# feixue94/sfd2

Hardware: AMD Instinct MI355X
Metric: images/sec extract+match (1600x1200, n4096) (higher is better)
Workload: dtype f16c

## Files before the change

include/sfd2_hip.h:

```cpp
#ifndef SFD2_HIP_H
#define SFD2_HIP_H

#include <stdint.h>

#ifdef __cplusplus
extern "C" {
#endif

typedef struct sfd2_ctx sfd2_ctx;

#define SFD2_DESC_DIM 128
#define SFD2_FLAG_ASYNC 1
#define SFD2_FLAG_NO_STABILITY 2
#define SFD2_FLAG_IMG_NORMALISED 4
#define SFD2_FLAG_IMG_U8_HWC 8
#define SFD2_FLAG_IMG_BGR 16
#define SFD2_FLAG_MATCH_OUT16 64
#define SFD2_FLAG_DESC_STORE64 128
#define SFD2_FLAG_IMG_U8_X 32

typedef struct {
    const char *name;
    const float *data;
    int32_t ndim;
    int64_t shape[4];
} sfd2_tensor;

#define SFD2_MATCH_HLOC 0
#define SFD2_MATCH_ITLOC_NNM 1
#define SFD2_MATCH_ITLOC_NNR 2
#define SFD2_DT_F32 0
#define SFD2_DT_F64 1
#define SFD2_DT_F16 2
#define SFD2_LAYOUT_ND 0
#define SFD2_LAYOUT_DN 1
#define SFD2_SIM_F16 0
#define SFD2_SIM_F16X2 1

typedef struct {
    int32_t flavour;
    int32_t do_mutual_check;
    float ratio_threshold;
    float distance_threshold;
    int32_t sim_mode;
} sfd2_match_conf;

typedef struct {
    float ms_total;
    float ms_backbone;
    float ms_post;
    float ms_match;
    int64_t n_candidates;
} sfd2_timings;

int sfd2_version(void);
const char *sfd2_last_error(void);

int sfd2_ctx_create(int device, sfd2_ctx **out);
int sfd2_device_pci_bus_id(int device, char *out, int len, int *n_devices);
void sfd2_ctx_destroy(sfd2_ctx *ctx);
void *sfd2_get_stream(sfd2_ctx *ctx);

int sfd2_load_weights(sfd2_ctx *ctx, const sfd2_tensor *tensors, int n);

#define SFD2_PREC_F16 0
#define SFD2_PREC_F32 1
#define SFD2_PREC_F16X3 2
#define SFD2_PREC_F16C 3
int sfd2_set_precision(sfd2_ctx *ctx, int mode);

int sfd2_set_option(sfd2_ctx *ctx, const char *key, int value);
int sfd2_get_option(sfd2_ctx *ctx, const char *key, int *value);

int sfd2_det(sfd2_ctx *ctx, const float *x, int x_on_device, int H, int W, int flags,
             float *score, float *stability, float *desc, int out_on_device,
             int *hs, int *ws, int *hc, int *wc);

int sfd2_extract(sfd2_ctx *ctx, const void *img, int img_on_device, int H, int W,
                 float conf_th, int top_k, int flags,
                 float *kpts_xy, float *scores, float *desc, int out_on_device,
                 int64_t cap_out, int *n_out);
int sfd2_extract_multiscale(sfd2_ctx *ctx, const void *img, int img_on_device, int H, int W,
                            const double *scales, int n_scales, float conf_th, int top_k, int flags,
                            float *kpts_xy, float *scores, float *desc, int out_on_device,
                            int64_t cap_out, int *n_out);

int sfd2_preprocess(sfd2_ctx *ctx, const unsigned char *img_hwc, int on_device, int H, int W, int flags,
                    int new_h, int new_w, float *out_chw_dev);

int sfd2_extract_count(sfd2_ctx *ctx, int *n_out);

typedef struct {
    int32_t n;
    int32_t n_candidates;
    uint32_t saturated;
    uint32_t flags;
} sfd2_extract_record;
int sfd2_extract_record_async(sfd2_ctx *ctx, sfd2_extract_record *rec, int rec_on_device);

int sfd2_extract_spp(sfd2_ctx *ctx, const float *x, int x_on_device, int H, int W, float conf_th, int flags,
                     float *kpts_xy, float *scores, float *desc, int64_t cap_out, int *n_out,
                     float *heat_out, float *desc_full_out);
int sfd2_extract_spp_levels(sfd2_ctx *ctx, const float *x, int x_on_device, int H, int W, int n_levels,
                            const int32_t *nh, const int32_t *nw, const int32_t *emit, float conf_th, int flags,
                            float *kpts_xy, float *scores, float *desc, int64_t cap_out, int32_t *level_count);
int sfd2_nms_fast(sfd2_ctx *ctx, const float *heat, int H, int W, float conf_th, int dist, float *kept_out);

int sfd2_simple_nms(sfd2_ctx *ctx, const float *heat, int H, int W, int radius, float *nms_out);
int sfd2_select_keypoints(sfd2_ctx *ctx, const float *heat, int H, int W, float conf_th,
                          int radius, int border, int top_k,
                          float *kpts_xy, float *scores, int64_t cap_out, int *n_out);
int sfd2_sample_descriptors(sfd2_ctx *ctx, const float *desc_map, int hc, int wc, int nh, int nw,
                            const float *kpts_xy, int n, float *desc_out);
int sfd2_heatmap(sfd2_ctx *ctx, const float *score, int hs, int ws, const float *sta, int hc, int wc,
                 int H, int W, float *heat_out);
int sfd2_debug_activation(sfd2_ctx *ctx, const char *name, float *out, int64_t cap, int *c, int *h, int *w);

int sfd2_match(sfd2_ctx *ctx, const void *d0, int n0, const void *d1, int n1, int dim,
               int dtype, int layout, int on_device, const sfd2_match_conf *conf,
               int64_t *matches0, float *scores0, int out_on_device);

int sfd2_match_segments(sfd2_ctx *ctx, const void *d0, int n0, const void *d1, int n1, int dim,
                        int dtype, int layout, int on_device, int n_seg, const int32_t *seg0, const int32_t *seg1,
                        const sfd2_match_conf *conf, int64_t *matches0, float *scores0, int out_on_device);

typedef struct {
    const void *data;
    int32_t n;
    int32_t dtype;
    int32_t layout;
    int32_t on_device;
    const int32_t *rows;
    int32_t n_rows;
    int32_t reserved;
} sfd2_desc_set;

int sfd2_desc_pack(sfd2_ctx *ctx, const sfd2_desc_set *src, int dim, void *dst_f16_dev, int flags);

int sfd2_match_batch(sfd2_ctx *ctx, const sfd2_desc_set *q, const sfd2_desc_set *db, int k, int dim,
                     const sfd2_match_conf *conf, int64_t *matches0, float *scores0, int out_on_device,
                     int flags);

int sfd2_extract_match(sfd2_ctx *ctx, const void *img_dev, int H, int W, float conf_th, int top_k, int flags,
                       float *kpts_xy, float *scores, float *desc, const sfd2_desc_set *db, int k, int dim,
                       const sfd2_match_conf *conf, int64_t *matches0, float *scores0);

int sfd2_get_timings(sfd2_ctx *ctx, sfd2_timings *out);

#define SFD2_RANGE_TENSORS 17
#define SFD2_RANGE_GROUPS 14
typedef struct {
    int32_t n_tensors;
    float max_stored[SFD2_RANGE_TENSORS];
    float max_value[SFD2_RANGE_TENSORS];
    int32_t exponent[SFD2_RANGE_TENSORS];
    uint32_t saturated;
    uint32_t low;
    int32_t fallbacks;
} sfd2_range_status;
int sfd2_get_range_status(sfd2_ctx *ctx, sfd2_range_status *out, int reset);
const char *sfd2_range_tensor_name(int i);
int sfd2_calibrate_range(sfd2_ctx *ctx, const float *img, int img_on_device, int H, int W, int flags);
int sfd2_get_act_exponents(sfd2_ctx *ctx, int32_t *exps, float *maxima, int cap, int *n);
int sfd2_set_act_exponents(sfd2_ctx *ctx, const int32_t *exps, int n );
int sfd2_get_margin_status(sfd2_ctx *ctx, float *errs4, int *choice, float *target);
int sfd2_get_relax_status(sfd2_ctx *ctx, float *err_plain, int *c3b_plain);

int sfd2_sync(sfd2_ctx *ctx);

typedef struct {
    char name[32];
    char kernel[48];
    double flops;
    double bytes;
    double ms_total;
    int32_t launches;
} sfd2_layer_timing;
int sfd2_set_profiling(sfd2_ctx *ctx, int max_steps );
int sfd2_set_profile_filter(sfd2_ctx *ctx, const char *substr);
int sfd2_get_layer_timings(sfd2_ctx *ctx, sfd2_layer_timing *out, int cap, int *n);

#define SFD2_JPEG_OK 0
#define SFD2_JPEG_NOT_JPEG 1
#define SFD2_JPEG_TRUNCATED 2
#define SFD2_JPEG_PROGRESSIVE 3
#define SFD2_JPEG_ARITHMETIC 4
#define SFD2_JPEG_PRECISION 5
#define SFD2_JPEG_COLOUR 6
#define SFD2_JPEG_SAMPLING 7
#define SFD2_JPEG_MULTI_SCAN 8
#define SFD2_JPEG_PROCESS 9
#define SFD2_JPEG_MALFORMED 10
typedef struct {
    int32_t width, height;
    int32_t n_components;
    int32_t h_samp[3], v_samp[3];
    int32_t restart_interval;
    int32_t supported;
    int32_t reason;
    int32_t mcus_x, mcus_y;
    int32_t n_intervals;
    int32_t n_blocks;
    int64_t file_bytes;
    int64_t scan_begin, scan_end;
    int64_t prepared_cap;
    int64_t prepared_bytes;
    int32_t n_lanes;
    int32_t prepared;
} sfd2_jpeg_info;

int sfd2_jpeg_parse(const uint8_t *data, int64_t n, sfd2_jpeg_info *info);

int sfd2_jpeg_prepare(uint8_t *buf, int64_t cap, sfd2_jpeg_info *info);

int sfd2_jpeg_decode(sfd2_ctx *ctx, const uint8_t *data, int64_t n, const sfd2_jpeg_info *info, int flags,
                     uint8_t *out_rgbx_dev, int64_t out_cap, uint32_t *status, int status_on_device);

#define SFD2_CAM_SIMPLE_PINHOLE 0
#define SFD2_CAM_PINHOLE 1
#define SFD2_CAM_SIMPLE_RADIAL 2
#define SFD2_CAM_OPENCV 4
typedef struct {
    int32_t n;
    int32_t model;
    const double *points2D;
    const double *points3D;
    double params[8];
    int32_t width, height;
    double max_error_px;
} sfd2_pose_problem;
typedef struct {
    double min_inlier_ratio;
    int64_t min_num_trials, max_num_trials;
    double confidence;
    uint64_t seed;
} sfd2_pose_conf;
typedef struct {
    int32_t success;
    int32_t num_inliers;
    int32_t num_trials;
    int32_t reserved;
    double qvec[4];
    double tvec[3];
} sfd2_pose_result;

int sfd2_absolute_pose_batch(sfd2_ctx *ctx, const sfd2_pose_problem *problems, int k, const sfd2_pose_conf *conf,
                             sfd2_pose_result *results, uint8_t *inlier_mask_u8, int flags);
int sfd2_pose_refine_batch(sfd2_ctx *ctx, const sfd2_pose_problem *problems, int k, const double *qvec_tvec_in,
                           const uint8_t *inlier_mask_u8, sfd2_pose_result *results, int flags);

#ifdef __cplusplus
}
#endif
#endif
```

sfd2_amd/_lib.py:

```python
import ctypes
import os

import numpy as np

_HERE = os.path.dirname(os.path.abspath(__file__))
LIB_PATH = os.path.join(_HERE, "libsfd2hip.so")


def use_library(path):
    global LIB_PATH, _lib
    if _lib is not None:
        raise RuntimeError("use_library() must be called before the library is first loaded")
    LIB_PATH = os.path.abspath(path)

FLAG_ASYNC = 1
FLAG_NO_STABILITY = 2
FLAG_IMG_NORMALISED = 4
FLAG_IMG_U8_HWC = 8
FLAG_IMG_BGR = 16
FLAG_IMG_U8_X = 32
FLAG_MATCH_OUT16 = 64
FLAG_DESC_STORE64 = 128
MATCH_HLOC, MATCH_ITLOC_NNM, MATCH_ITLOC_NNR = 0, 1, 2
DT_F32, DT_F64, DT_F16 = 0, 1, 2
LAYOUT_ND, LAYOUT_DN = 0, 1
SIM_F16, SIM_F16X2 = 0, 1


class Sfd2Tensor(ctypes.Structure):
    _fields_ = [("name", ctypes.c_char_p), ("data", ctypes.c_void_p), ("ndim", ctypes.c_int32),
                ("shape", ctypes.c_int64 * 4)]


class MatchConf(ctypes.Structure):
    _fields_ = [("flavour", ctypes.c_int32), ("do_mutual_check", ctypes.c_int32),
                ("ratio_threshold", ctypes.c_float), ("distance_threshold", ctypes.c_float),
                ("sim_mode", ctypes.c_int32)]


class Timings(ctypes.Structure):
    _fields_ = [("ms_total", ctypes.c_float), ("ms_backbone", ctypes.c_float), ("ms_post", ctypes.c_float),
                ("ms_match", ctypes.c_float), ("n_candidates", ctypes.c_int64)]


class DescSet(ctypes.Structure):
    _fields_ = [("data", ctypes.c_void_p), ("n", ctypes.c_int32), ("dtype", ctypes.c_int32),
                ("layout", ctypes.c_int32), ("on_device", ctypes.c_int32),
                ("rows", ctypes.c_void_p), ("n_rows", ctypes.c_int32), ("reserved", ctypes.c_int32)]


class LayerTiming(ctypes.Structure):
    _fields_ = [("name", ctypes.c_char * 32), ("kernel", ctypes.c_char * 48), ("flops", ctypes.c_double),
                ("bytes", ctypes.c_double), ("ms_total", ctypes.c_double), ("launches", ctypes.c_int32)]


class ExtractRecord(ctypes.Structure):
    _fields_ = [("n", ctypes.c_int32), ("n_candidates", ctypes.c_int32), ("saturated", ctypes.c_uint32), ("flags", ctypes.c_uint32)]


RANGE_TENSORS, RANGE_GROUPS = 17, 14


class RangeStatus(ctypes.Structure):
    _fields_ = [("n_tensors", ctypes.c_int32), ("max_stored", ctypes.c_float * RANGE_TENSORS),
                ("max_value", ctypes.c_float * RANGE_TENSORS), ("exponent", ctypes.c_int32 * RANGE_TENSORS),
                ("saturated", ctypes.c_uint32), ("low", ctypes.c_uint32), ("fallbacks", ctypes.c_int32)]


class JpegInfo(ctypes.Structure):
    _fields_ = [("width", ctypes.c_int32), ("height", ctypes.c_int32), ("n_components", ctypes.c_int32),
                ("h_samp", ctypes.c_int32 * 3), ("v_samp", ctypes.c_int32 * 3), ("restart_interval", ctypes.c_int32),
                ("supported", ctypes.c_int32), ("reason", ctypes.c_int32), ("mcus_x", ctypes.c_int32), ("mcus_y", ctypes.c_int32),
                ("n_intervals", ctypes.c_int32), ("n_blocks", ctypes.c_int32), ("file_bytes", ctypes.c_int64),
                ("scan_begin", ctypes.c_int64), ("scan_end", ctypes.c_int64), ("prepared_cap", ctypes.c_int64),
                ("prepared_bytes", ctypes.c_int64), ("n_lanes", ctypes.c_int32), ("prepared", ctypes.c_int32)]


class PoseProblem(ctypes.Structure):
    _fields_ = [("n", ctypes.c_int32), ("model", ctypes.c_int32), ("points2D", ctypes.c_void_p), ("points3D", ctypes.c_void_p),
                ("params", ctypes.c_double * 8), ("width", ctypes.c_int32), ("height", ctypes.c_int32), ("max_error_px", ctypes.c_double)]


class PoseConf(ctypes.Structure):
    _fields_ = [("min_inlier_ratio", ctypes.c_double), ("min_num_trials", ctypes.c_int64), ("max_num_trials", ctypes.c_int64),
                ("confidence", ctypes.c_double), ("seed", ctypes.c_uint64)]


class PoseResult(ctypes.Structure):
    _fields_ = [("success", ctypes.c_int32), ("num_inliers", ctypes.c_int32), ("num_trials", ctypes.c_int32), ("reserved", ctypes.c_int32),
                ("qvec", ctypes.c_double * 4), ("tvec", ctypes.c_double * 3)]


EXPORTS = [
    "sfd2_version", "sfd2_last_error", "sfd2_ctx_create", "sfd2_ctx_destroy", "sfd2_get_stream",
    "sfd2_load_weights", "sfd2_det", "sfd2_extract", "sfd2_extract_count", "sfd2_simple_nms",
    "sfd2_select_keypoints", "sfd2_sample_descriptors", "sfd2_heatmap", "sfd2_debug_activation",
    "sfd2_match", "sfd2_match_batch", "sfd2_get_timings", "sfd2_sync", "sfd2_set_profiling",
    "sfd2_get_layer_timings", "sfd2_set_precision", "sfd2_extract_spp", "sfd2_nms_fast",
    "sfd2_set_profile_filter", "sfd2_extract_multiscale", "sfd2_set_option", "sfd2_extract_match", "sfd2_preprocess", "sfd2_extract_spp_levels", "sfd2_match_segments",
    "sfd2_get_range_status", "sfd2_range_tensor_name", "sfd2_calibrate_range", "sfd2_get_act_exponents", "sfd2_set_act_exponents",
    "sfd2_extract_record_async", "sfd2_desc_pack", "sfd2_get_margin_status", "sfd2_get_relax_status", "sfd2_get_option", "sfd2_device_pci_bus_id",
    "sfd2_jpeg_parse", "sfd2_jpeg_prepare", "sfd2_jpeg_decode", "sfd2_absolute_pose_batch", "sfd2_pose_refine_batch",
]

_lib = None


def load():
    global _lib
    if _lib is not None:
        return _lib
    if LIB_PATH == os.path.join(_HERE, "libsfd2hip.so"):
        from . import build as _build
        if _build.needs_build() and _build.have_hipcc():
            import fcntl
            with open(os.path.join(_HERE, ".build.lock"), "w") as lk:
                fcntl.flock(lk, fcntl.LOCK_EX)
                try:
                    if _build.needs_build():
                        _build.build_lib()
                finally:
                    fcntl.flock(lk, fcntl.LOCK_UN)
    if not os.path.exists(LIB_PATH):
        raise RuntimeError(f"{LIB_PATH} is missing and no hipcc was found to build it "
                           "(hipcc --offload-arch=gfx950; `python -c 'import __graft_entry__ as g; g.build()'`). "
                           "There is no CPU fallback.")
    lib = ctypes.CDLL(LIB_PATH)
    vp, ci, cf, i64 = ctypes.c_void_p, ctypes.c_int, ctypes.c_float, ctypes.c_int64
    pi = ctypes.POINTER(ctypes.c_int)
    lib.sfd2_version.restype = ci
    lib.sfd2_last_error.restype = ctypes.c_char_p
    lib.sfd2_ctx_create.argtypes = [ci, ctypes.POINTER(vp)]
    lib.sfd2_ctx_destroy.argtypes = [vp]
    lib.sfd2_ctx_destroy.restype = None
    lib.sfd2_get_stream.argtypes = [vp]
    lib.sfd2_get_stream.restype = vp
    lib.sfd2_load_weights.argtypes = [vp, ctypes.POINTER(Sfd2Tensor), ci]
    lib.sfd2_det.argtypes = [vp, vp, ci, ci, ci, ci, vp, vp, vp, ci, pi, pi, pi, pi]
    lib.sfd2_extract.argtypes = [vp, vp, ci, ci, ci, cf, ci, ci, vp, vp, vp, ci, i64, pi]
    lib.sfd2_extract_count.argtypes = [vp, pi]
    lib.sfd2_extract_multiscale.argtypes = [vp, vp, ci, ci, ci, vp, ci, cf, ci, ci, vp, vp, vp, ci, i64, pi]
    lib.sfd2_extract_spp.argtypes = [vp, vp, ci, ci, ci, cf, ci, vp, vp, vp, i64, pi, vp, vp]
    lib.sfd2_nms_fast.argtypes = [vp, vp, ci, ci, cf, ci, vp]
    lib.sfd2_extract_spp_levels.argtypes = [vp, vp, ci, ci, ci, ci, vp, vp, vp, cf, ci, vp, vp, vp, i64, vp]
    lib.sfd2_simple_nms.argtypes = [vp, vp, ci, ci, ci, vp]
    lib.sfd2_select_keypoints.argtypes = [vp, vp, ci, ci, cf, ci, ci, ci, vp, vp, i64, pi]
    lib.sfd2_sample_descriptors.argtypes = [vp, vp, ci, ci, ci, ci, vp, ci, vp]
    lib.sfd2_heatmap.argtypes = [vp, vp, ci, ci, vp, ci, ci, ci, ci, vp]
    lib.sfd2_debug_activation.argtypes = [vp, ctypes.c_char_p, vp, i64, pi, pi, pi]
    lib.sfd2_match.argtypes = [vp, vp, ci, vp, ci, ci, ci, ci, ci, ctypes.POINTER(MatchConf), vp, vp, ci]
    lib.sfd2_match_segments.argtypes = [vp, vp, ci, vp, ci, ci, ci, ci, ci, ci, vp, vp, ctypes.POINTER(MatchConf), vp, vp, ci]
    lib.sfd2_match_batch.argtypes = [vp, ctypes.POINTER(DescSet), ctypes.POINTER(DescSet), ci, ci,
                                     ctypes.POINTER(MatchConf), vp, vp, ci, ci]
    lib.sfd2_get_timings.argtypes = [vp, ctypes.POINTER(Timings)]
    lib.sfd2_sync.argtypes = [vp]
    lib.sfd2_set_precision.argtypes = [vp, ci]
    lib.sfd2_set_option.argtypes = [vp, ctypes.c_char_p, ci]
    lib.sfd2_get_option.argtypes = [vp, ctypes.c_char_p, pi]
    lib.sfd2_device_pci_bus_id.argtypes = [ci, ctypes.c_char_p, ci, pi]
    lib.sfd2_preprocess.argtypes = [vp, vp, ci, ci, ci, ci, ci, ci, vp]
    lib.sfd2_extract_match.argtypes = [vp, vp, ci, ci, cf, ci, ci, vp, vp, vp, ctypes.POINTER(DescSet), ci, ci,
                                       ctypes.POINTER(MatchConf), vp, vp]
    lib.sfd2_set_profiling.argtypes = [vp, ci]
    lib.sfd2_set_profile_filter.argtypes = [vp, ctypes.c_char_p]
    lib.sfd2_get_layer_timings.argtypes = [vp, ctypes.POINTER(LayerTiming), ci, pi]
    lib.sfd2_get_range_status.argtypes = [vp, ctypes.POINTER(RangeStatus), ci]
    lib.sfd2_range_tensor_name.argtypes = [ci]
    lib.sfd2_range_tensor_name.restype = ctypes.c_char_p
    lib.sfd2_calibrate_range.argtypes = [vp, vp, ci, ci, ci, ci]
    lib.sfd2_get_act_exponents.argtypes = [vp, vp, vp, ci, pi]
    lib.sfd2_get_margin_status.argtypes = [vp, vp, pi, ctypes.POINTER(ctypes.c_float)]
    lib.sfd2_get_relax_status.restype = ci
    lib.sfd2_get_relax_status.argtypes = [vp, ctypes.POINTER(ctypes.c_float), pi]
    lib.sfd2_set_act_exponents.argtypes = [vp, vp, ci]
    lib.sfd2_extract_record_async.argtypes = [vp, vp, ci]
    lib.sfd2_desc_pack.argtypes = [vp, ctypes.POINTER(DescSet), ci, vp, ci]
    lib.sfd2_jpeg_parse.argtypes = [vp, i64, ctypes.POINTER(JpegInfo)]
    lib.sfd2_jpeg_prepare.argtypes = [vp, i64, ctypes.POINTER(JpegInfo)]
    lib.sfd2_jpeg_decode.argtypes = [vp, vp, i64, ctypes.POINTER(JpegInfo), ci, vp, i64, vp, ci]
    lib.sfd2_absolute_pose_batch.argtypes = [vp, ctypes.POINTER(PoseProblem), ci, ctypes.POINTER(PoseConf), ctypes.POINTER(PoseResult), vp, ci]
    lib.sfd2_pose_refine_batch.argtypes = [vp, ctypes.POINTER(PoseProblem), ci, vp, vp, ctypes.POINTER(PoseResult), ci]
    for name in EXPORTS:
        getattr(lib, name)
    if lib.sfd2_version() < 109:
        raise RuntimeError(f"{LIB_PATH} is version {lib.sfd2_version()}, this binding needs >= 109 (rebuild: __graft_entry__.build())")
    _lib = lib
    return lib


def check(rc):
    if rc != 0:
        raise RuntimeError("libsfd2hip: " + load().sfd2_last_error().decode("utf-8", "replace"))


def ptr(a):
    if a is None:
        return None
    if isinstance(a, int):
        return a
    if isinstance(a, np.ndarray):
        return a.ctypes.data
    return a.data_ptr()


class Context:

    def __init__(self, device=0):
        self.lib = load()
        h = ctypes.c_void_p()
        check(self.lib.sfd2_ctx_create(int(device), ctypes.byref(h)))
        self.h = h
        self.device = int(device)
        self.options = {}

    def close(self):
        if getattr(self, "h", None):
            self.lib.sfd2_ctx_destroy(self.h)
            self.h = None

    def __del__(self):
        try:
            self.close()
        except Exception:
            pass

    @property
    def stream(self):
        return self.lib.sfd2_get_stream(self.h)

    def load_weights(self, sd):
        keep, arr = [], (Sfd2Tensor * len(sd))()
        n = 0
        for name, v in sd.items():
            a = v.detach().cpu().numpy() if hasattr(v, "detach") else np.asarray(v)
            if a.dtype.kind != "f":
                continue
            a = np.ascontiguousarray(a, dtype=np.float32)
            if a.ndim > 4:
                continue
            keep.append(a)
            arr[n].name = name.encode()
            arr[n].data = a.ctypes.data
            arr[n].ndim = a.ndim
            for i, s in enumerate(a.shape):
                arr[n].shape[i] = s
            n += 1
        check(self.lib.sfd2_load_weights(self.h, arr, n))

    def timings(self):
        t = Timings()
        check(self.lib.sfd2_get_timings(self.h, ctypes.byref(t)))
        return {"ms_total": t.ms_total, "ms_backbone": t.ms_backbone, "ms_post": t.ms_post,
                "ms_match": t.ms_match, "n_candidates": t.n_candidates}

    def set_precision(self, mode):
        check(self.lib.sfd2_set_precision(self.h, {'f16': 0, 'f32': 1, 'f16x3': 2, 'f16c': 3, 'f16x3d': 2}[mode]))
        check(self.lib.sfd2_set_option(self.h, b"x3_desc16", 1 if mode == 'f16x3d' else 0))

    def set_option(self, key, value):
        check(self.lib.sfd2_set_option(self.h, key.encode(), int(value)))
        self.options.pop(key, None)
        self.options[key] = int(value)

    def get_option(self, key):
        v = ctypes.c_int(0)
        check(self.lib.sfd2_get_option(self.h, key.encode(), ctypes.byref(v)))
        return int(v.value)

    def sync(self):
        check(self.lib.sfd2_sync(self.h))

    def set_profiling(self, max_steps, kernel_filter=None):
        check(self.lib.sfd2_set_profile_filter(self.h, (kernel_filter or "").encode()))
        check(self.lib.sfd2_set_profiling(self.h, int(max_steps)))

    def layer_timings(self):
        n = ctypes.c_int(0)
        arr = (LayerTiming * 64)()
        check(self.lib.sfd2_get_layer_timings(self.h, arr, 64, ctypes.byref(n)))
        return [{"name": arr[i].name.decode(), "kernel": arr[i].kernel.decode(), "flops": arr[i].flops,
                 "bytes": arr[i].bytes, "ms_total": arr[i].ms_total, "launches": arr[i].launches}
                for i in range(min(n.value, 64))]

    def range_status(self, reset=False):
        rs = RangeStatus()
        check(self.lib.sfd2_get_range_status(self.h, ctypes.byref(rs), 1 if reset else 0))
        names = [self.lib.sfd2_range_tensor_name(i).decode() for i in range(rs.n_tensors)]
        return {"tensors": {n: {"max_stored": rs.max_stored[i], "max_value": rs.max_value[i], "exponent": rs.exponent[i]}
                            for i, n in enumerate(names)},
                "saturated": [n for i, n in enumerate(names) if rs.saturated >> i & 1],
                "low": [n for i, n in enumerate(names) if rs.low >> i & 1], "fallbacks": rs.fallbacks}

    def calibrate_range(self, img, normalised=False):
        on_dev = 0 if isinstance(img, np.ndarray) else 1
        if isinstance(img, np.ndarray):
            img = np.ascontiguousarray(img, dtype=np.float32)
        check(self.lib.sfd2_calibrate_range(self.h, ptr(img), on_dev, int(img.shape[-2]), int(img.shape[-1]),
                                            FLAG_IMG_NORMALISED if normalised else 0))

    def act_exponents(self):
        e = np.zeros(RANGE_GROUPS, dtype=np.int32)
        m = np.zeros(RANGE_GROUPS, dtype=np.float32)
        n = ctypes.c_int(0)
        check(self.lib.sfd2_get_act_exponents(self.h, e.ctypes.data, m.ctypes.data, RANGE_GROUPS, ctypes.byref(n)))
        return e, m

    def margin_status(self):
        e = np.zeros(4, dtype=np.float32)
        ch, tg = ctypes.c_int(0), ctypes.c_float(0)
        check(self.lib.sfd2_get_margin_status(self.h, e.ctypes.data, ctypes.byref(ch), ctypes.byref(tg)))
        names = ["as set", "rb_inner=0", "comp_heads=1", "rb_inner=0 comp_heads=1"]
        ep, on = ctypes.c_float(0), ctypes.c_int(0)
        check(self.lib.sfd2_get_relax_status(self.h, ctypes.byref(ep), ctypes.byref(on)))
        return {"errors": {n: float(v) for n, v in zip(names, e)}, "choice": int(ch.value),
                "running": names[ch.value] if ch.value >= 0 else None, "target": float(tg.value),
                "c3b_plain": bool(on.value), "error_with_c3b_plain": float(ep.value)}

    def set_act_exponents(self, exps=None):
        if exps is None:
            check(self.lib.sfd2_set_act_exponents(self.h, None, 0))
        else:
            e = np.ascontiguousarray(exps, dtype=np.int32)
            check(self.lib.sfd2_set_act_exponents(self.h, e.ctypes.data, int(e.size)))

    def debug_activation(self, name):
        c, h, w = ctypes.c_int(), ctypes.c_int(), ctypes.c_int()
        check(self.lib.sfd2_debug_activation(self.h, name.encode(), None, 0, ctypes.byref(c), ctypes.byref(h), ctypes.byref(w)))
        out = np.empty((c.value, h.value, w.value), dtype=np.float32)
        check(self.lib.sfd2_debug_activation(self.h, name.encode(), out.ctypes.data, out.size, ctypes.byref(c),
                                             ctypes.byref(h), ctypes.byref(w)))
        return out


_default_ctx = {}


def default_context(device=0):
    d = int(device)
    if d not in _default_ctx:
        _default_ctx[d] = Context(d)
# ... 2 lines not shown
```

sfd2_amd/csrc/api_core.hip:

```cpp
#include "sfd2_ctx.h"

static thread_local std::string g_err;
int sfd2_fail(const std::string &m)
{
    g_err = m;
    return -1;
}

std::atomic<unsigned long long> g_alloc_gen{0};

thread_local int g_sfd2_cu_limit = 0;

extern "C" int sfd2_version(void) { return 110; }
extern "C" const char *sfd2_last_error(void) { return g_err.c_str(); }

extern "C" int sfd2_ctx_create(int device, sfd2_ctx **out)
{
    if (!out) return fail("sfd2_ctx_create: out is null");
    int ndev = 0;
    hipError_t e = hipGetDeviceCount(&ndev);
    if (e != hipSuccess || ndev <= 0) return fail("sfd2_ctx_create: no HIP device available (libsfd2hip has no CPU fallback)");
    if (device < 0 || device >= ndev) return fail("sfd2_ctx_create: bad device index");
    HIPCHECK(hipSetDevice(device));
    sfd2_ctx *c = new sfd2_ctx();
    c->device = device;
    HIPCHECK(hipStreamCreateWithFlags(&c->stream, hipStreamNonBlocking));
    for (int i = 0; i < 4; ++i) HIPCHECK(hipEventCreate(&c->ev[i]));
    HIPCHECK(hipEventCreateWithFlags(&c->ev_jobs, hipEventDisableTiming));
    HIPCHECK(hipStreamCreateWithFlags(&c->copy_stream, hipStreamNonBlocking));
    HIPCHECK(hipStreamCreateWithFlags(&c->side_stream, hipStreamNonBlocking));
    HIPCHECK(hipEventCreateWithFlags(&c->ev_fork, hipEventDisableTiming));
    HIPCHECK(hipEventCreateWithFlags(&c->ev_join, hipEventDisableTiming));
    c->cur_stream = c->stream;
    for (int i = 0; i < SFD2_IMG_SLOTS; ++i) {
        HIPCHECK(hipEventCreateWithFlags(&c->ev_copied[i], hipEventDisableTiming));
        HIPCHECK(hipEventCreateWithFlags(&c->ev_img_free[i], hipEventDisableTiming));
    }
    c->fuse = sfd2_env("SFD2_NO_FUSE") ? 0 : 1;
    HIPCHECK(c->zero_page.ensure(SFD2_ZERO_PAGE_BYTES + ((size_t)SFD2_RS_COUNT * (SFD2_RANGE_SUB + 1) + 4) * sizeof(unsigned int)));
    HIPCHECK(hipMemset(c->zero_page.p, 0, c->zero_page.cap));
    c->range_stat.p = c->zero_page.as<char>() + SFD2_ZERO_PAGE_BYTES;
    c->range_hist_dev.p = c->range_stat.as<unsigned int>() + SFD2_RS_COUNT * SFD2_RANGE_SUB;
    c->extract_rec.p = c->range_hist_dev.as<unsigned int>() + SFD2_RS_COUNT;
    static_assert(SFD2_RS_COUNT == SFD2_RANGE_TENSORS && AE_COUNT == SFD2_RANGE_GROUPS, "include/sfd2_hip.h and the internal tables agree");

    *out = c;
    return 0;
}

extern "C" int sfd2_device_pci_bus_id(int device, char *out, int len, int *n_devices)
{
    int ndev = 0;
    hipError_t e = hipGetDeviceCount(&ndev);
    if (e != hipSuccess || ndev <= 0) return fail("sfd2_device_pci_bus_id: no HIP device available");
    if (n_devices) *n_devices = ndev;
    if (device < 0 || device >= ndev) return fail("sfd2_device_pci_bus_id: bad device index");
    if (!out || len < 13) return fail("sfd2_device_pci_bus_id: buffer of at least 13 bytes needed");
    HIPCHECK(hipDeviceGetPCIBusId(out, len, device));
    return 0;
}

extern "C" void sfd2_ctx_destroy(sfd2_ctx *c)
{
    if (!c) return;
    (void)hipSetDevice(c->device);
    (void)hipStreamSynchronize(c->stream);
    graphs_release(c);
    for (int i = 0; i < 4; ++i) if (c->ev[i]) (void)hipEventDestroy(c->ev[i]);
    if (c->ev_jobs) (void)hipEventDestroy(c->ev_jobs);
    for (int i = 0; i < SFD2_IMG_SLOTS; ++i) {
        if (c->ev_copied[i]) (void)hipEventDestroy(c->ev_copied[i]);
        if (c->ev_img_free[i]) (void)hipEventDestroy(c->ev_img_free[i]);
    }
    if (c->copy_stream) (void)hipStreamDestroy(c->copy_stream);
    if (c->side_stream) (void)hipStreamDestroy(c->side_stream);
    if (c->ev_fork) (void)hipEventDestroy(c->ev_fork);
    if (c->ev_join) (void)hipEventDestroy(c->ev_join);
    for (hipEvent_t e : c->prof_ev) (void)hipEventDestroy(e);
    if (c->pin_jobs) (void)hipHostFree(c->pin_jobs);
    if (c->stream) (void)hipStreamDestroy(c->stream);
    delete c;
}

extern "C" void *sfd2_get_stream(sfd2_ctx *c) { return c ? (void *)c->stream : nullptr; }

extern "C" int sfd2_set_precision(sfd2_ctx *c, int mode)
{
    if (!c) return fail("sfd2_set_precision: null ctx");
    if (mode != SFD2_PREC_F16 && mode != SFD2_PREC_F32 && mode != SFD2_PREC_F16X3 && mode != SFD2_PREC_F16C)
        return fail("sfd2_set_precision: unknown mode");
    HIPCHECK(hipSetDevice(c->device));
    HIPCHECK(hipStreamSynchronize(c->stream));
    if (mode != c->precision) graphs_release(c);
    c->precision = mode;
    return sfd2_margin_selfcheck_if_pending(c);
}

extern "C" int sfd2_set_option(sfd2_ctx *c, const char *key, int value)
{
    if (!c || !key) return fail("sfd2_set_option: null argument");
    HIPCHECK(hipSetDevice(c->device));
    HIPCHECK(hipStreamSynchronize(c->stream));
    const std::string k(key);
    graphs_release(c);
    if (k == "fuse") c->fuse = value ? 1 : 0;
    else if (k == "fuse_det") c->fuse_det = value ? 1 : 0;
    else if (k == "alias") c->opt_alias = value ? 1 : 0;
    else if (k == "graphs") c->use_graphs = value ? 1 : 0;
    else if (k == "branches") c->opt_branches = value ? 1 : 0;
    else if (k == "sta_side") c->opt_sta_side = value ? 1 : 0;
    else if (k == "fuse_post") c->opt_fuse_post = value ? 1 : 0;
    else if (k == "sparse_desc") c->opt_sparse_desc = value ? 1 : 0;
    else if (k == "sparse_da3") c->opt_sparse_da3 = value ? 1 : 0;
    else if (k == "cu_limit") c->opt_cu_limit = value < 0 ? 0 : value;
    else if (k == "auto_range") c->opt_auto_range = value ? 1 : 0;
    else if (k == "range_fallback") c->opt_range_fallback = value ? 1 : 0;
    else if (k == "x3_pp") c->opt_x3_pp = value ? 1 : 0;
    else if (k == "x3_desc16") c->opt_x3_desc16 = value ? 1 : 0;
    else if (k == "auto_margin") c->opt_auto_margin = value ? 1 : 0;
    else if (k == "fp6_filters") c->opt_fp6_filters = value ? 1 : 0;
    else if (k == "fp6_acts") c->opt_fp6_acts = value ? 1 : 0;
    else if (k == "s2d") c->opt_s2d = value ? 1 : 0;
    else if (k == "trunk_r1") c->opt_trunk_r1 = value ? 1 : 0;
    else if (k == "fuse_pb") c->opt_fuse_pb = value ? 1 : 0;
    else if (k == "generic_c") c->opt_generic_c = value ? 1 : 0;
    else if (k == "comp_rb") c->opt_comp_rb = value ? 1 : 0;
    else if (k == "no_rf_c") c->opt_no_rf_c = value ? 1 : 0;
    else if (k == "comp_heads") { c->opt_comp_heads = c->user_comp_heads = value ? 1 : 0; c->user_set_comp_heads = true; }
    else if (k == "c3b_plain") { c->user_c3b_plain = value < 0 ? -1 : (value ? 1 : 0); c->opt_c3b_plain = value > 0 ? 1 : 0; }
    else if (k == "comp_det") c->opt_comp_det = value ? 1 : 0;
    else if (k == "fuse_rb23") c->opt_fuse_rb23 = value ? 1 : 0;
    else if (k == "rb_inner") { c->opt_rb_inner = c->user_rb_inner = value < 0 ? 0 : (value > 2 ? 2 : value); c->user_set_rb_inner = true; }
    else return fail("sfd2_set_option: unknown key '" + k + "'");
    return 0;
}

extern "C" int sfd2_get_option(sfd2_ctx *c, const char *key, int *value)
{
    if (!c || !key || !value) return fail("sfd2_get_option: null argument");
    const std::string k(key);
    const struct { const char *name; int v; } tab[] = {
        {"fuse", c->fuse}, {"fuse_det", c->fuse_det}, {"alias", c->opt_alias}, {"graphs", c->use_graphs}, {"branches", c->opt_branches}, {"sta_side", c->opt_sta_side},
        {"fuse_post", c->opt_fuse_post}, {"sparse_desc", c->opt_sparse_desc}, {"sparse_da3", c->opt_sparse_da3}, {"cu_limit", c->opt_cu_limit},
        {"auto_range", c->opt_auto_range}, {"range_fallback", c->opt_range_fallback}, {"x3_pp", c->opt_x3_pp}, {"x3_desc16", c->opt_x3_desc16},
        {"auto_margin", c->opt_auto_margin}, {"fp6_filters", c->opt_fp6_filters}, {"fp6_acts", c->opt_fp6_acts}, {"s2d", c->opt_s2d},
        {"trunk_r1", c->opt_trunk_r1}, {"fuse_pb", c->opt_fuse_pb}, {"generic_c", c->opt_generic_c}, {"comp_rb", c->opt_comp_rb},
        {"no_rf_c", c->opt_no_rf_c}, {"comp_heads", c->opt_comp_heads}, {"c3b_plain", c->opt_c3b_plain}, {"comp_det", c->opt_comp_det},
        {"fuse_rb23", c->opt_fuse_rb23}, {"rb_inner", c->opt_rb_inner},
    };
    for (const auto &e : tab)
        if (k == e.name) { *value = e.v; return 0; }
    return fail("sfd2_get_option: unknown key '" + k + "'");
}

extern "C" int sfd2_sync(sfd2_ctx *c)
{
    if (!c) return fail("sfd2_sync: null ctx");
    HIPCHECK(hipSetDevice(c->device));
    HIPCHECK(hipStreamSynchronize(c->stream));
    return 0;
}

extern "C" int sfd2_set_profiling(sfd2_ctx *c, int max_steps)
{
    if (!c) return fail("sfd2_set_profiling: null ctx");
    HIPCHECK(hipSetDevice(c->device));
    HIPCHECK(hipStreamSynchronize(c->stream));
    if (max_steps < 0 || max_steps > 4096) return fail("sfd2_set_profiling: max_steps out of range");
    const size_t need = (size_t)max_steps * PROF_SLOTS * 2;
    while (c->prof_ev.size() < need) {
        hipEvent_t e;
        HIPCHECK(hipEventCreate(&e));
        c->prof_ev.push_back(e);
    }
    c->prof_max_steps = max_steps;
    c->prof_step = 0;
    c->prof_slot = 0;
    c->prof_used.assign(max_steps, 0);
    c->prof_row.assign((size_t)max_steps * PROF_SLOTS, 0);
    c->prof_tab.clear();
    return 0;
}

extern "C" int sfd2_set_profile_filter(sfd2_ctx *c, const char *substr)
{
    if (!c) return fail("sfd2_set_profile_filter: null ctx");
    c->prof_filter = substr ? substr : "";
    return 0;
}

extern "C" int sfd2_get_layer_timings(sfd2_ctx *c, sfd2_layer_timing *out, int cap, int *n)
{
    if (!c || !n) return fail("sfd2_get_layer_timings: null argument");
    HIPCHECK(hipSetDevice(c->device));
    HIPCHECK(hipStreamSynchronize(c->stream));
    for (int st = 0; st < c->prof_step; ++st)
        for (int sl = 0; sl < c->prof_used[st]; ++sl) {
            float ms = 0.0f;
            const size_t e = ((size_t)st * PROF_SLOTS + sl) * 2;
            const int row = c->prof_row[(size_t)st * PROF_SLOTS + sl];
            if (hipEventElapsedTime(&ms, c->prof_ev[e], c->prof_ev[e + 1]) == hipSuccess) {
                c->prof_tab[row].ms_total += ms;
                c->prof_tab[row].launches += 1;
            }
        }
    c->prof_step = 0;
    *n = (int)c->prof_tab.size();
    if (out)
        for (int i = 0; i < *n && i < cap; ++i) out[i] = c->prof_tab[i];
    return 0;
}

extern "C" int sfd2_get_timings(sfd2_ctx *c, sfd2_timings *out)
{
    if (!c || !out) return fail("sfd2_get_timings: null argument");
    *out = c->tim;
    return 0;
}

static const int kRsGroup[SFD2_RS_COUNT] = {AE_CONV1A, AE_CONV1B, AE_CONV2A, AE_CONV2B, AE_CONV3A, AE_TRUNK, AE_T1_0, AE_T1_1, AE_T1_2,
                                            AE_T2_0, AE_T2_1, AE_T2_2, AE_TRUNK, AE_TRUNK, AE_TRUNK, AE_PA0, AE_DA0};
extern "C" const char *sfd2_range_tensor_name(int i)
{
    static const char *names[SFD2_RS_COUNT] = {"conv1a", "conv1b", "conv2a", "conv2b", "conv3a", "conv3b", "conv4.0.t1", "conv4.1.t1", "conv4.2.t1",
                                               "conv4.0.t2", "conv4.1.t2", "conv4.2.t2", "conv4.0", "conv4.1", "conv4.2", "convPa.0", "convDa.0"};
    return (i >= 0 && i < SFD2_RS_COUNT) ? names[i] : "";
}

static int fetch_range_words(sfd2_ctx *c, unsigned int *raw , bool clear)
{
    const size_t bytes = (size_t)SFD2_RS_COUNT * (SFD2_RANGE_SUB + 1) * sizeof(unsigned int);
    HIPCHECK(hipMemcpyAsync(raw, c->range_stat.p, bytes, hipMemcpyDeviceToHost, c->stream));
    if (clear) HIPCHECK(hipMemsetAsync(c->range_stat.p, 0, bytes, c->stream));
    HIPCHECK(hipStreamSynchronize(c->stream));
    return 0;
}

int read_range_status(sfd2_ctx *c, sfd2_range_status *out, int reset)
{
    unsigned int raw[SFD2_RS_COUNT * (SFD2_RANGE_SUB + 1)];
    if (fetch_range_words(c, raw, reset != 0)) return -1;
    std::memset(out, 0, sizeof(*out));
    out->n_tensors = SFD2_RS_COUNT;
    const unsigned int sat_bits = 0x44E00000u;
    for (int t = 0; t < SFD2_RS_COUNT; ++t) {
        unsigned int m = raw[SFD2_RS_COUNT * SFD2_RANGE_SUB + t];
        for (int s = 0; s < SFD2_RANGE_SUB; ++s) m = std::max(m, raw[t * SFD2_RANGE_SUB + s]);
        float f;
        std::memcpy(&f, &m, 4);
        const bool sat = m >= sat_bits || c->range_hist[t] >= SFD2_C_SAT;
        if (!(f >= c->range_hist[t])) f = c->range_hist[t];
        if (reset) c->range_hist[t] = 0.0f;
        const int e = c->act_exp[kRsGroup[t]];
        out->max_stored[t] = f;
        out->max_value[t] = std::ldexp(f, -e);
        out->exponent[t] = e;
        if (sat) out->saturated |= 1u << t;
        if (f > 0.0f && f < 0.03125f) out->low |= 1u << t;
    }
    out->fallbacks = c->range_fallbacks;
    return 0;
}

int reset_range_records(sfd2_ctx *c)
{
    if (!c->range_stat.p) return 0;
    HIPCHECK(hipMemsetAsync(c->range_stat.p, 0, (size_t)SFD2_RS_COUNT * (SFD2_RANGE_SUB + 1) * sizeof(unsigned int), c->stream));
    for (int t = 0; t < SFD2_RS_COUNT; ++t) c->range_hist[t] = 0.0f;
    return 0;
}

int range_fold_before_sync_extract(sfd2_ctx *c)
{
    if (c->precision != SFD2_PREC_F16C || !c->opt_range_fallback || c->in_fallback) return 0;
    launch_extract_record(c->stream, c->range_stat.as<unsigned int>(), c->range_hist_dev.as<unsigned int>(), nullptr, 0, 0, nullptr);
    HIPCHECK(hipGetLastError());
    return 0;
}

extern "C" int sfd2_get_range_status(sfd2_ctx *c, sfd2_range_status *out, int reset)
{
    if (!c || !out) return fail("sfd2_get_range_status: null argument");
    HIPCHECK(hipSetDevice(c->device));
    return read_range_status(c, out, reset);
}

int range_wants_fallback(sfd2_ctx *c)
{
    if (c->precision != SFD2_PREC_F16C || !c->opt_range_fallback || c->in_fallback) return 0;
    unsigned int raw[SFD2_RS_COUNT * SFD2_RANGE_SUB];
    HIPCHECK(hipMemcpyAsync(raw, c->range_stat.p, sizeof(raw), hipMemcpyDeviceToHost, c->stream));
    HIPCHECK(hipStreamSynchronize(c->stream));
    bool sat = false;
    float mx[SFD2_RS_COUNT];
    for (int t = 0; t < SFD2_RS_COUNT; ++t) {
        unsigned int m = 0;
// ... 25 lines not shown
```

sfd2_amd/csrc/api_graph.hip:

```cpp
#include "sfd2_ctx.h"

struct GraphKey {
    int H, W, top_k, flags, k, dim, n0;
    float conf_th;
    sfd2_match_conf conf;
    const void *img, *kp, *sc, *de, *m, *ms;
    unsigned long long db_hash;
    bool operator==(const GraphKey &o) const { return memcmp(this, &o, sizeof(GraphKey)) == 0; }
};
struct GraphEntry {
    GraphKey key;
    hipGraph_t graph = nullptr;
    hipGraphExec_t exec = nullptr;
    unsigned long long gen = 0, last_use = 0;
    int seen = 0;
    void *pin = nullptr;
    size_t pin_cap = 0;
    DevBuf jobs, fins;
};
#define SFD2_MAX_GRAPHS 16

static void graph_entry_release(GraphEntry &e)
{
    if (e.exec) (void)hipGraphExecDestroy(e.exec);
    if (e.graph) (void)hipGraphDestroy(e.graph);
    if (e.pin) (void)hipHostFree(e.pin);
    e.jobs.release();
    e.fins.release();
    e = GraphEntry();
}

void graphs_release(sfd2_ctx *c)
{
    if (!c->graphs) return;
    for (int i = 0; i < c->n_graphs; ++i) graph_entry_release(c->graphs[i]);
    delete[] c->graphs;
    c->graphs = nullptr;
    c->n_graphs = 0;
}

static int extract_match_eager(sfd2_ctx *c, const void *img, int H, int W, float conf_th, int top_k, int flags, float *kp,
                               float *sc, float *de, const sfd2_desc_set *db, int k, int dim, const sfd2_match_conf *conf,
                               int64_t *m, float *ms)
{
    int n_dummy = 0;
    if (sfd2_extract(c, img, 1, H, W, conf_th, top_k, flags | SFD2_FLAG_ASYNC, kp, sc, de, 1, top_k, &n_dummy)) return -1;
    if (k > 0) {
        const sfd2_desc_set q = {de, top_k, SFD2_DT_F32, SFD2_LAYOUT_ND, 1, nullptr, 0, 0};
        if (sfd2_match_batch(c, &q, db, k, dim, conf, m, ms, 1, SFD2_FLAG_ASYNC)) return -1;
    }
    return 0;
}

extern "C" int sfd2_extract_match(sfd2_ctx *c, const void *img_dev, int H, int W, float conf_th, int top_k, int flags,
                                  float *kpts_xy, float *scores, float *desc, const sfd2_desc_set *db, int k, int dim,
                                  const sfd2_match_conf *conf, int64_t *matches0, float *scores0)
{
    if (!c || !img_dev || !kpts_xy || !scores || !desc) return fail("sfd2_extract_match: null argument");
    if (top_k <= 0) return fail("sfd2_extract_match: top_k must be positive (fixed-capacity device outputs)");
    if (flags & SFD2_FLAG_DESC_STORE64) return fail("sfd2_extract_match: SFD2_FLAG_DESC_STORE64 is for stores; the matcher reads the float [n][128] descriptors");
    if (k < 0 || (k > 0 && (!db || !conf || !matches0 || !scores0))) return fail("sfd2_extract_match: null matcher argument");
    for (int i = 0; i < k; ++i)
        if (!db[i].on_device || db[i].rows) return fail("sfd2_extract_match: database sets must be device resident, without row selection");
    HIPCHECK(hipSetDevice(c->device));
    if (!c->use_graphs || c->prof_max_steps > 0)
        return extract_match_eager(c, img_dev, H, W, conf_th, top_k, flags, kpts_xy, scores, desc, db, k, dim, conf, matches0, scores0);

    GraphKey key;
    memset(&key, 0, sizeof(key));
    key.H = H; key.W = W; key.top_k = top_k; key.flags = flags; key.k = k; key.dim = dim; key.n0 = top_k; key.conf_th = conf_th;
    if (conf) key.conf = *conf;
    key.img = img_dev; key.kp = kpts_xy; key.sc = scores; key.de = desc; key.m = matches0; key.ms = scores0;
    unsigned long long h = 1469598103934665603ull;
    for (int i = 0; i < k; ++i) {
        const unsigned long long v[3] = {(unsigned long long)(uintptr_t)db[i].data, (unsigned long long)db[i].n,
                                         ((unsigned long long)db[i].dtype << 8) | (unsigned long long)db[i].layout};
        for (unsigned long long x : v) { h ^= x; h *= 1099511628211ull; }
    }
    key.db_hash = h;
    if (!c->graphs) { c->graphs = new GraphEntry[SFD2_MAX_GRAPHS]; c->n_graphs = SFD2_MAX_GRAPHS; }
    GraphEntry *e = nullptr, *lru = &c->graphs[0];
    for (int i = 0; i < c->n_graphs; ++i) {
        GraphEntry &g = c->graphs[i];
        if (g.seen && g.key == key) { e = &g; break; }
        if (g.last_use < lru->last_use) lru = &g;
    }
    if (!e) {
        graph_entry_release(*lru);
        e = lru;
        e->key = key;
    }
    e->last_use = ++c->graph_clock;
    if (e->exec && e->gen == g_alloc_gen) {
        HIPCHECK(hipGraphLaunch(e->exec, c->stream));
        return 0;
    }
    if (e->exec) {
        (void)hipGraphExecDestroy(e->exec); e->exec = nullptr;
        (void)hipGraphDestroy(e->graph); e->graph = nullptr;
        e->seen = 0;
    }
    if (e->seen == 0) {
        e->seen = 1;
        return extract_match_eager(c, img_dev, H, W, conf_th, top_k, flags, kpts_xy, scores, desc, db, k, dim, conf, matches0, scores0);
    }
    const size_t jb = 2 * (size_t)std::max(k, 1) * sizeof(MatchJob), fb = (size_t)std::max(k, 1) * sizeof(MatchFinal);
    if (!e->pin) {
        HIPCHECK(hipHostMalloc(&e->pin, jb + fb, hipHostMallocDefault));
        e->pin_cap = jb + fb;
        HIPCHECK(e->jobs.ensure(jb + fb));
    }
    HIPCHECK(hipStreamSynchronize(c->stream));
    HIPCHECK(hipEventSynchronize(c->ev_jobs));
    const unsigned long long gen0 = g_alloc_gen.load();
    std::swap(c->pin_jobs, e->pin); std::swap(c->pin_cap, e->pin_cap);
    std::swap(c->m_jobs, e->jobs); std::swap(c->m_fins, e->fins);
    hipError_t be = hipStreamBeginCapture(c->stream, hipStreamCaptureModeThreadLocal);
    int rc = -1;
    hipGraph_t g = nullptr;
    if (be == hipSuccess) {
        rc = extract_match_eager(c, img_dev, H, W, conf_th, top_k, flags, kpts_xy, scores, desc, db, k, dim, conf, matches0, scores0);
        const hipError_t ee = hipStreamEndCapture(c->stream, &g);
        if (ee != hipSuccess) rc = fail(std::string("hipStreamEndCapture: ") + hipGetErrorString(ee));
    } else {
        fail(std::string("hipStreamBeginCapture: ") + hipGetErrorString(be));
    }
    std::swap(c->pin_jobs, e->pin); std::swap(c->pin_cap, e->pin_cap);
    std::swap(c->m_jobs, e->jobs); std::swap(c->m_fins, e->fins);
    if (rc != 0 || g_alloc_gen != gen0) {
        if (g) (void)hipGraphDestroy(g);
        e->seen = 0;
        if (rc == 0) return fail("sfd2_extract_match: workspace changed during capture");
        return -1;
    }
    e->graph = g;
    HIPCHECK(hipGraphInstantiate(&e->exec, g, nullptr, nullptr, 0));
    e->gen = g_alloc_gen;
    HIPCHECK(hipGraphLaunch(e->exec, c->stream));
    return 0;
}
```

sfd2_amd/csrc/api_match.hip:

```cpp
#include "sfd2_ctx.h"

static size_t elt_size(int dtype) { return dtype == SFD2_DT_F64 ? 8 : (dtype == SFD2_DT_F16 ? 2 : 4); }

static int prep_set(sfd2_ctx *c, const void *src, int n_src, const int32_t *rows, int n, int dim, int dtype, int layout,
                    int on_device, int need_lo, DevBuf &stage, size_t &stage_off, half_t *hi_dst, half_t *lo_dst,
                    const half_t **hi, const half_t **lo, const int **rows_dev = nullptr)
{
    if (rows_dev) *rows_dev = nullptr;
    if (!rows && dtype == SFD2_DT_F16 && layout == SFD2_LAYOUT_ND && on_device && dim == 128 && !need_lo) {
        *hi = reinterpret_cast<const half_t *>(src);
        *lo = nullptr;
        return 0;
    }
    const void *dev_src = src;
    if (!on_device) {
        const size_t bytes = (size_t)n_src * dim * elt_size(dtype);
        void *dst = reinterpret_cast<char *>(stage.p) + stage_off;
        HIPCHECK(hipMemcpyAsync(dst, src, bytes, hipMemcpyHostToDevice, c->stream));
        dev_src = dst;
        stage_off += (bytes + 255) & ~(size_t)255;
    }
    const int *rd = nullptr;
    if (rows) {
        void *dst = reinterpret_cast<char *>(stage.p) + stage_off;
        HIPCHECK(hipMemcpyAsync(dst, rows, (size_t)n * sizeof(int32_t), hipMemcpyHostToDevice, c->stream));
        rd = reinterpret_cast<const int *>(dst);
        stage_off += ((size_t)n * sizeof(int32_t) + 255) & ~(size_t)255;
        if (rows_dev) *rows_dev = rd;
    }
    launch_match_prep(c->stream, dev_src, n, n_src, rd, dim, dtype, layout, hi_dst, need_lo ? lo_dst : nullptr);
    *hi = hi_dst;
    *lo = need_lo ? lo_dst : nullptr;
    return 0;
}

extern "C" int sfd2_desc_pack(sfd2_ctx *c, const sfd2_desc_set *src, int dim, void *dst_f16_dev, int flags)
{
    if (!c || !src || !dst_f16_dev) return fail("sfd2_desc_pack: null argument");
    if (dim <= 0 || dim > 128) return fail("descriptor dimension must be in [1,128]");
    if (src->n < 0 || src->n_rows < 0) return fail("negative size");
    if (src->dtype != SFD2_DT_F32 && src->dtype != SFD2_DT_F64 && src->dtype != SFD2_DT_F16) return fail("sfd2_desc_pack: unknown dtype");
    if (src->layout != SFD2_LAYOUT_ND && src->layout != SFD2_LAYOUT_DN) return fail("sfd2_desc_pack: unknown layout");
    const int n = src->rows ? src->n_rows : src->n;
    if (n == 0) return 0;
    if (!src->data) return fail("sfd2_desc_pack: null descriptors");
    if (src->rows)
        for (int r = 0; r < src->n_rows; ++r)
            if (src->rows[r] < 0 || src->rows[r] >= src->n) return fail("sfd2_desc_pack: row index out of range");
    HIPCHECK(hipSetDevice(c->device));
    size_t stage_bytes = 256;
    if (!src->on_device) stage_bytes += (((size_t)src->n * dim * elt_size(src->dtype)) + 255) & ~(size_t)255;
    if (src->rows) stage_bytes += ((size_t)n * sizeof(int32_t) + 255) & ~(size_t)255;
    HIPCHECK(c->m_stage.ensure(stage_bytes));
    size_t off = 0;
    void *dev_src = const_cast<void *>(src->data);
    if (!src->on_device) {
        const size_t bytes = (size_t)src->n * dim * elt_size(src->dtype);
        HIPCHECK(hipMemcpyAsync(c->m_stage.p, src->data, bytes, hipMemcpyHostToDevice, c->stream));
        dev_src = c->m_stage.p;
        off += (bytes + 255) & ~(size_t)255;
    }
    const int *rd = nullptr;
    if (src->rows) {
        void *dst = c->m_stage.as<char>() + off;
        HIPCHECK(hipMemcpyAsync(dst, src->rows, (size_t)n * sizeof(int32_t), hipMemcpyHostToDevice, c->stream));
        rd = reinterpret_cast<const int *>(dst);
    }
    launch_match_prep(c->stream, dev_src, n, src->n, rd, dim, src->dtype, src->layout, reinterpret_cast<half_t *>(dst_f16_dev), nullptr);
    HIPCHECK(hipGetLastError());
    if (!(flags & SFD2_FLAG_ASYNC)) HIPCHECK(hipStreamSynchronize(c->stream));
    return 0;
}

extern "C" int sfd2_match_batch(sfd2_ctx *c, const sfd2_desc_set *q, const sfd2_desc_set *db, int k, int dim,
                                const sfd2_match_conf *conf, int64_t *matches0, float *scores0, int out_on_device,
                                int flags)
{
    if (!c || !conf || !q || (k > 0 && !db)) return fail("sfd2_match_batch: null argument");
    if (dim <= 0 || dim > 128) return fail("descriptor dimension must be in [1,128]");
    const int n0 = q->n;
    if (n0 < 0 || k < 0) return fail("negative size");
    if (k == 0 || n0 == 0) return 0;
    if (!q->data) return fail("sfd2_match_batch: null query descriptors");
    HIPCHECK(hipSetDevice(c->device));
    const int need_lo = conf->sim_mode == SFD2_SIM_F16X2;
    const bool o16 = (flags & SFD2_FLAG_MATCH_OUT16) != 0;
    const size_t msz = o16 ? sizeof(short) : sizeof(long long), ssz = o16 ? sizeof(half_t) : sizeof(float);
    int max_n1 = 0;
    size_t tot_n1 = 0, stage_bytes = 0;
    if (q->rows) return fail("sfd2_match_batch: row selection applies to database sets only");
    std::vector<int> eff_n1(k);
    for (int i = 0; i < k; ++i) {
        if (db[i].n < 0 || db[i].n_rows < 0) return fail("negative n1");
        if (db[i].n > 0 && !db[i].data) return fail("sfd2_match_batch: null database descriptors");
        if (db[i].rows)
            for (int r = 0; r < db[i].n_rows; ++r)
                if (db[i].rows[r] < 0 || db[i].rows[r] >= db[i].n) return fail("sfd2_match_batch: row index out of range");
        eff_n1[i] = db[i].rows ? db[i].n_rows : db[i].n;
        max_n1 = std::max(max_n1, eff_n1[i]);
        tot_n1 += (size_t)eff_n1[i];
        if (!db[i].on_device) stage_bytes += (((size_t)db[i].n * dim * elt_size(db[i].dtype)) + 255) & ~(size_t)255;
        if (db[i].rows) stage_bytes += ((size_t)db[i].n_rows * sizeof(int32_t) + 255) & ~(size_t)255;
    }
    if (!q->on_device) stage_bytes += (((size_t)n0 * dim * elt_size(q->dtype)) + 255) & ~(size_t)255;
    const int max_n = std::max(n0, max_n1);
    const int blocks_per_job = (max_n + 255) / 256;
    int splits = (768 * 6 + 2 * k * blocks_per_job - 1) / (2 * k * blocks_per_job);
    splits = std::max(1, std::min(splits, 8));
    const int min_n = std::max(1, std::min(n0, max_n1 > 0 ? max_n1 : 1));
    splits = std::min(splits, std::max(1, (min_n + 31) / 32));
    if (const char *e = sfd2_env("SFD2_MATCH_SPLITS")) splits = std::max(1, std::min(16, atoi(e)));

    const int need_top2 = (conf->flavour == SFD2_MATCH_ITLOC_NNR) ||
                          (conf->flavour == SFD2_MATCH_HLOC && conf->ratio_threshold > 0.0f);
    const bool single_gemm = !need_lo && !need_top2 && sfd2_env("SFD2_MATCH_TWO_GEMM") == nullptr;
    if (single_gemm) {
        const int qblocks = (n0 + 255) / 256;
        splits = (512 * 6 + k * qblocks - 1) / (k * qblocks);
        splits = std::max(1, std::min(splits, 8));
        splits = std::min(splits, std::max(1, (std::max(1, max_n1) + 31) / 32));
        if (const char *e = sfd2_env("SFD2_MATCH_SPLITS")) splits = std::max(1, std::min(16, atoi(e)));
        splits = std::max(splits, (max_n1 + match_mutual_max_chunk() - 1) / match_mutual_max_chunk());
    }
    const int nstrip = (n0 + match_mutual_strip() - 1) / match_mutual_strip();

    HIPCHECK(c->m_stage.ensure(std::max<size_t>(stage_bytes, 256)));
    HIPCHECK(c->m_hi0.ensure((size_t)n0 * 128 * 2));
    if (need_lo) HIPCHECK(c->m_lo0.ensure((size_t)n0 * 128 * 2));
    HIPCHECK(c->m_hi1.ensure(std::max<size_t>(tot_n1, 1) * 128 * 2));
    if (need_lo) HIPCHECK(c->m_lo1.ensure(std::max<size_t>(tot_n1, 1) * 128 * 2));
    const size_t per_pair_f = (size_t)splits * n0, tot_part = (size_t)k * per_pair_f + (size_t)splits * tot_n1;
    HIPCHECK(c->m_part_f.ensure(std::max<size_t>(tot_part, 1) * 2 * sizeof(float)));
    HIPCHECK(c->m_part_i.ensure(std::max<size_t>(tot_part, 1) * sizeof(int)));
    if (single_gemm) HIPCHECK(c->m_rkeys.ensure(std::max<size_t>((size_t)nstrip * tot_n1, 1) * sizeof(float)));
    HIPCHECK(c->m_red.ensure(((size_t)k * n0 + tot_n1 + 1) * 3 * sizeof(float)));
    HIPCHECK(c->m_jobs.ensure((size_t)2 * k * sizeof(MatchJob) + (size_t)k * sizeof(MatchFinal)));
    HIPCHECK(c->m_out_m.ensure((size_t)k * n0 * sizeof(long long)));
    HIPCHECK(c->m_out_s.ensure((size_t)k * n0 * sizeof(float)));

    HIPCHECK(hipEventRecord(c->ev[0], c->stream));
    prof_step_begin(c);
    size_t stage_off = 0;
    const half_t *q_hi = nullptr, *q_lo = nullptr;
    if (prep_set(c, q->data, n0, nullptr, n0, dim, q->dtype, q->layout, q->on_device, need_lo, c->m_stage, stage_off,
                 c->m_hi0.as<half_t>(), c->m_lo0.as<half_t>(), &q_hi, &q_lo)) return -1;
    static_assert(sizeof(MatchJob2) <= 2 * sizeof(MatchJob), "descriptor buffer sizing");
    const size_t jobs_bytes = 2 * (size_t)k * sizeof(MatchJob), fins_bytes = (size_t)k * sizeof(MatchFinal);
    hipStreamCaptureStatus cap_status = hipStreamCaptureStatusNone;
    (void)hipStreamIsCapturing(c->stream, &cap_status);
    const bool capturing = cap_status != hipStreamCaptureStatusNone;
    if (!capturing) HIPCHECK(hipEventSynchronize(c->ev_jobs));
    if (jobs_bytes + fins_bytes > c->pin_cap) {
        if (c->pin_jobs) (void)hipHostFree(c->pin_jobs);
        c->pin_jobs = nullptr;
        c->pin_cap = 0;
        HIPCHECK(hipHostMalloc(&c->pin_jobs, jobs_bytes + fins_bytes, hipHostMallocDefault));
        c->pin_cap = jobs_bytes + fins_bytes;
    }
    MatchJob *jobs = reinterpret_cast<MatchJob *>(c->pin_jobs);
    MatchJob2 *jobs2 = reinterpret_cast<MatchJob2 *>(c->pin_jobs);
    MatchFinal *fins = reinterpret_cast<MatchFinal *>(reinterpret_cast<char *>(c->pin_jobs) + jobs_bytes);
    float *pf = c->m_part_f.as<float>();
    int *pi = c->m_part_i.as<int>();
    float *red = c->m_red.as<float>();
    size_t off1 = 0, poff = 0, roff = 0;
    for (int i = 0; i < k; ++i) {
        const int n1 = eff_n1[i];
        const half_t *h = nullptr, *l = nullptr;
        const int *remap = nullptr;
        if (n1 > 0) {
            if (prep_set(c, db[i].data, db[i].n, db[i].rows, n1, dim, db[i].dtype, db[i].layout, db[i].on_device, need_lo,
                         c->m_stage, stage_off, c->m_hi1.as<half_t>() + off1 * 128,
                         need_lo ? c->m_lo1.as<half_t>() + off1 * 128 : nullptr, &h, &l, &remap))
                return -1;
        }
        MatchFinal &fn = fins[i];
        fn.remap = remap;
        if (single_gemm) {
            MatchJob2 &j2 = jobs2[i];
            j2.q_hi = q_hi; j2.d_hi = h; j2.n0 = n0; j2.n1 = n1;
            j2.part_v1 = pf + 2 * poff; j2.part_i1 = pi + poff;
            j2.rkeys = c->m_rkeys.as<float>() + (size_t)nstrip * off1;
            poff += (size_t)splits * n0 + (size_t)splits * n1;
            fn.f_v1 = fn.f_v2 = fn.r_v1 = fn.r_v2 = nullptr; fn.f_i1 = fn.r_i1 = nullptr;
        } else {
            MatchJob &f = jobs[2 * i], &r = jobs[2 * i + 1];
            f.a_hi = h; f.a_lo = l; f.b_hi = q_hi; f.b_lo = q_lo; f.na = n1; f.nb = n0;
            f.part_v1 = pf + 2 * poff; f.part_v2 = pf + 2 * poff + (size_t)splits * n0; f.part_i1 = pi + poff;
            poff += (size_t)splits * n0;
            r.a_hi = q_hi; r.a_lo = q_lo; r.b_hi = h; r.b_lo = l; r.na = n0; r.nb = n1;
            r.part_v1 = pf + 2 * poff; r.part_v2 = pf + 2 * poff + (size_t)splits * n1; r.part_i1 = pi + poff;
            poff += (size_t)splits * n1;
            fn.f_v1 = f.part_v1; fn.f_v2 = f.part_v2; fn.f_i1 = f.part_i1;
            fn.r_v1 = r.part_v1; fn.r_v2 = r.part_v2; fn.r_i1 = r.part_i1;
        }
        off1 += (size_t)n1;
        fn.n0 = n0; fn.n1 = n1;
        fn.out16 = o16 ? 1 : 0; fn.pad_ = 0;
        const bool direct_out = out_on_device && matches0 && scores0;
        fn.matches0 = reinterpret_cast<long long *>((direct_out ? reinterpret_cast<char *>(matches0) : c->m_out_m.as<char>()) + (size_t)i * n0 * msz);
        fn.scores0 = reinterpret_cast<float *>((direct_out ? reinterpret_cast<char *>(scores0) : c->m_out_s.as<char>()) + (size_t)i * n0 * ssz);
        fn.red_f = red + 3 * roff; roff += (size_t)n0;
        fn.red_r = red + 3 * roff; roff += (size_t)n1;
    }
    HIPCHECK(hipMemcpyAsync(c->m_jobs.p, jobs, jobs_bytes + fins_bytes, hipMemcpyHostToDevice, c->stream));
    MatchFinal *fins_dev = reinterpret_cast<MatchFinal *>(static_cast<char *>(c->m_jobs.p) + jobs_bytes);
    if (!capturing) HIPCHECK(hipEventRecord(c->ev_jobs, c->stream));
    if (single_gemm) {
        {
            ProfScope ps(c, "match_mutual", "match_mutual_kernel", 2.0 * (double)n0 * (double)tot_n1 * 128.0,
                         2.0 * ((double)k * n0 + (double)tot_n1) * 128.0);
            launch_match_mutual(c->stream, c->m_jobs.as<MatchJob2>(), fins_dev, k, n0, max_n1, splits,
                                conf->flavour == SFD2_MATCH_HLOC && !conf->do_mutual_check);
        }
        {
            ProfScope ps(c, "match_finalize", "match_decide", 0.0, (double)tot_part * 12);
            launch_match_decide(c->stream, fins_dev, k, max_n, conf->flavour, conf->do_mutual_check,
                                conf->ratio_threshold, conf->distance_threshold);
        }
    } else {
        {
            ProfScope ps(c, "match_top2", need_lo ? "match_top2_kernel<x2>" : "match_top2_kernel",
                         2.0 * 2.0 * (double)n0 * (double)tot_n1 * 128.0 * (need_lo ? 3.0 : 1.0),
                         2.0 * 2.0 * ((double)k * n0 + (double)tot_n1) * 128.0);
            launch_match_top2(c->stream, c->m_jobs.as<MatchJob>(), 2 * k, max_n, splits, need_lo, need_top2,
                              c->zero_page.as<half_t>());
        }
        {
            ProfScope ps(c, "match_finalize", "match_reduce+decide", 0.0, (double)tot_part * 12);
            launch_match_finalize(c->stream, fins_dev, k, max_n, splits, conf->flavour,
                                  conf->do_mutual_check, conf->ratio_threshold, conf->distance_threshold);
        }
    }
    prof_step_end(c);
    HIPCHECK(hipGetLastError());
    HIPCHECK(hipEventRecord(c->ev[3], c->stream));
    if (!(out_on_device && matches0 && scores0)) {
        if (copy_out(c, matches0, c->m_out_m.p, (size_t)k * n0 * msz, out_on_device)) return -1;
        if (copy_out(c, scores0, c->m_out_s.p, (size_t)k * n0 * ssz, out_on_device)) return -1;
    }
    if (!(flags & SFD2_FLAG_ASYNC)) {
        HIPCHECK(hipStreamSynchronize(c->stream));
        float ms = 0.0f;
        if (hipEventElapsedTime(&ms, c->ev[0], c->ev[3]) == hipSuccess) c->tim.ms_match = ms;
    }
    return 0;
}

extern "C" int sfd2_match_segments(sfd2_ctx *c, const void *d0, int n0, const void *d1, int n1, int dim, int dtype, int layout,
                                   int on_device, int n_seg, const int32_t *seg0, const int32_t *seg1,
                                   const sfd2_match_conf *conf, int64_t *matches0, float *scores0, int out_on_device)
{
    if (!c || !conf || !seg0 || !seg1 || !matches0 || !scores0) return fail("sfd2_match_segments: null argument");
    if (dim <= 0 || dim > 128) return fail("descriptor dimension must be in [1,128]");
    if (n0 < 0 || n1 < 0 || n_seg < 0) return fail("negative size");
    if (n0 == 0) return 0;
    if (!d0 || (n1 > 0 && !d1)) return fail("sfd2_match_segments: null descriptors");
    if (seg0[0] != 0 || seg1[0] != 0 || seg0[n_seg] != n0 || seg1[n_seg] != n1) return fail("sfd2_match_segments: segment offsets must span [0, n]");
    for (int i = 0; i < n_seg; ++i)
        if (seg0[i + 1] < seg0[i] || seg1[i + 1] < seg1[i]) return fail("sfd2_match_segments: segment offsets must ascend");
    HIPCHECK(hipSetDevice(c->device));
    const int need_lo = conf->sim_mode == SFD2_SIM_F16X2;
    const int need_top2 = (conf->flavour == SFD2_MATCH_ITLOC_NNR) || (conf->flavour == SFD2_MATCH_HLOC && conf->ratio_threshold > 0.0f);
    const bool single_gemm = !need_lo && !need_top2;
    std::vector<int> live;
    int max_a = 0, max_b = 0;
    for (int i = 0; i < n_seg; ++i)
        if (seg0[i + 1] > seg0[i] && seg1[i + 1] > seg1[i]) {
            live.push_back(i);
            max_a = std::max(max_a, seg0[i + 1] - seg0[i]);
            max_b = std::max(max_b, seg1[i + 1] - seg1[i]);
        }
    const int k = (int)live.size();
    HIPCHECK(c->m_out_m.ensure((size_t)n0 * sizeof(long long)));
    HIPCHECK(c->m_out_s.ensure((size_t)n0 * sizeof(float)));
    long long *out_m = out_on_device ? reinterpret_cast<long long *>(matches0) : c->m_out_m.as<long long>();
    float *out_s = out_on_device ? scores0 : c->m_out_s.as<float>();
    HIPCHECK(hipMemsetAsync(out_m, 0xFF, (size_t)n0 * sizeof(long long), c->stream));
    HIPCHECK(hipMemsetAsync(out_s, 0, (size_t)n0 * sizeof(float), c->stream));
    if (k > 0) {
        int splits = std::max(1, (max_b + match_mutual_max_chunk() - 1) / match_mutual_max_chunk());
        const int strip = match_mutual_strip();
        size_t stage_bytes = 256 + (((size_t)n1 * sizeof(int32_t)) + 255);
        if (!on_device) stage_bytes += ((((size_t)n0 + n1) * dim * elt_size(dtype)) + 511);
        HIPCHECK(c->m_stage.ensure(stage_bytes));
        HIPCHECK(c->m_hi0.ensure((size_t)n0 * 128 * 2));
        HIPCHECK(c->m_hi1.ensure((size_t)std::max(n1, 1) * 128 * 2));
        if (need_lo) { HIPCHECK(c->m_lo0.ensure((size_t)n0 * 128 * 2)); HIPCHECK(c->m_lo1.ensure((size_t)std::max(n1, 1) * 128 * 2)); }
        const size_t tot_part = (size_t)splits * ((size_t)n0 + n1);
        HIPCHECK(c->m_part_f.ensure(tot_part * 2 * sizeof(float)));
        HIPCHECK(c->m_part_i.ensure(tot_part * sizeof(int)));
        size_t rk = 0;
        for (int i : live) rk += (size_t)((seg0[i + 1] - seg0[i] + strip - 1) / strip) * (size_t)(seg1[i + 1] - seg1[i]);
        if (single_gemm) HIPCHECK(c->m_rkeys.ensure(std::max<size_t>(rk, 1) * sizeof(float)));
        HIPCHECK(c->m_red.ensure(((size_t)n0 + n1 + 1) * 3 * sizeof(float)));
        HIPCHECK(c->m_jobs.ensure((size_t)2 * k * sizeof(MatchJob) + (size_t)k * sizeof(MatchFinal)));
        prof_step_begin(c);
        size_t stage_off = 0;
        const half_t *h0 = nullptr, *l0 = nullptr, *h1 = nullptr, *l1 = nullptr;
        if (prep_set(c, d0, n0, nullptr, n0, dim, dtype, layout, on_device, need_lo, c->m_stage, stage_off, c->m_hi0.as<half_t>(),
                     c->m_lo0.as<half_t>(), &h0, &l0)) return -1;
        if (prep_set(c, d1, n1, nullptr, n1, dim, dtype, layout, on_device, need_lo, c->m_stage, stage_off, c->m_hi1.as<half_t>(),
                     c->m_lo1.as<half_t>(), &h1, &l1)) return -1;
        std::vector<int32_t> iota((size_t)n1);
        for (int i = 0; i < n1; ++i) iota[i] = i;
        int32_t *iota_dev = reinterpret_cast<int32_t *>(reinterpret_cast<char *>(c->m_stage.p) + ((stage_off + 255) & ~(size_t)255));
        HIPCHECK(hipMemcpyAsync(iota_dev, iota.data(), (size_t)n1 * sizeof(int32_t), hipMemcpyHostToDevice, c->stream));
        HIPCHECK(hipStreamSynchronize(c->stream));
        const size_t jobs_bytes = 2 * (size_t)k * sizeof(MatchJob), fins_bytes = (size_t)k * sizeof(MatchFinal);
        HIPCHECK(hipEventSynchronize(c->ev_jobs));
        if (jobs_bytes + fins_bytes > c->pin_cap) {
            if (c->pin_jobs) (void)hipHostFree(c->pin_jobs);
            c->pin_jobs = nullptr;
            c->pin_cap = 0;
            HIPCHECK(hipHostMalloc(&c->pin_jobs, jobs_bytes + fins_bytes, hipHostMallocDefault));
            c->pin_cap = jobs_bytes + fins_bytes;
        }
        MatchJob *jobs = reinterpret_cast<MatchJob *>(c->pin_jobs);
        MatchJob2 *jobs2 = reinterpret_cast<MatchJob2 *>(c->pin_jobs);
        MatchFinal *fins = reinterpret_cast<MatchFinal *>(reinterpret_cast<char *>(c->pin_jobs) + jobs_bytes);
        float *pf = c->m_part_f.as<float>();
        int *pi = c->m_part_i.as<int>();
        float *red = c->m_red.as<float>();
        size_t poff = 0, roff = 0, rkoff = 0;
        for (int j = 0; j < k; ++j) {
            const int sg = live[j], a0 = seg0[sg], na = seg0[sg + 1] - a0, b0 = seg1[sg], nb = seg1[sg + 1] - b0;
            MatchFinal &fn = fins[j];
            fn.out16 = 0; fn.pad_ = 0;
            fn.remap = iota_dev + b0;
            if (single_gemm) {
                MatchJob2 &j2 = jobs2[j];
                j2.q_hi = h0 + (size_t)a0 * 128; j2.d_hi = h1 + (size_t)b0 * 128; j2.n0 = na; j2.n1 = nb;
                j2.part_v1 = pf + 2 * poff; j2.part_i1 = pi + poff;
                j2.rkeys = c->m_rkeys.as<float>() + rkoff;
                rkoff += (size_t)((na + strip - 1) / strip) * nb;
                poff += (size_t)splits * na + (size_t)splits * nb;
                fn.f_v1 = fn.f_v2 = fn.r_v1 = fn.r_v2 = nullptr; fn.f_i1 = fn.r_i1 = nullptr;
            } else {
                MatchJob &f = jobs[2 * j], &r = jobs[2 * j + 1];
                f.a_hi = h1 + (size_t)b0 * 128; f.a_lo = l1 ? l1 + (size_t)b0 * 128 : nullptr;
                f.b_hi = h0 + (size_t)a0 * 128; f.b_lo = l0 ? l0 + (size_t)a0 * 128 : nullptr; f.na = nb; f.nb = na;
                f.part_v1 = pf + 2 * poff; f.part_v2 = pf + 2 * poff + (size_t)splits * na; f.part_i1 = pi + poff;
                poff += (size_t)splits * na;
                r.a_hi = f.b_hi; r.a_lo = f.b_lo; r.b_hi = f.a_hi; r.b_lo = f.a_lo; r.na = na; r.nb = nb;
                r.part_v1 = pf + 2 * poff; r.part_v2 = pf + 2 * poff + (size_t)splits * nb; r.part_i1 = pi + poff;
                poff += (size_t)splits * nb;
                fn.f_v1 = f.part_v1; fn.f_v2 = f.part_v2; fn.f_i1 = f.part_i1;
                fn.r_v1 = r.part_v1; fn.r_v2 = r.part_v2; fn.r_i1 = r.part_i1;
            }
            fn.n0 = na; fn.n1 = nb;
            fn.matches0 = out_m + a0;
            fn.scores0 = out_s + a0;
            fn.red_f = red + 3 * roff; roff += (size_t)na;
            fn.red_r = red + 3 * roff; roff += (size_t)nb;
        }
        HIPCHECK(hipMemcpyAsync(c->m_jobs.p, jobs, jobs_bytes + fins_bytes, hipMemcpyHostToDevice, c->stream));
        MatchFinal *fins_dev = reinterpret_cast<MatchFinal *>(static_cast<char *>(c->m_jobs.p) + jobs_bytes);
        HIPCHECK(hipEventRecord(c->ev_jobs, c->stream));
        const int max_n = std::max(max_a, max_b);
        if (single_gemm) {
            ProfScope ps(c, "match_segments", "match_mutual_kernel", 0.0, 0.0);
            launch_match_mutual(c->stream, c->m_jobs.as<MatchJob2>(), fins_dev, k, max_a, max_b, splits,
                                conf->flavour == SFD2_MATCH_HLOC && !conf->do_mutual_check);
            launch_match_decide(c->stream, fins_dev, k, max_n, conf->flavour, conf->do_mutual_check,
                                conf->ratio_threshold, conf->distance_threshold);
        } else {
            ProfScope ps(c, "match_segments", "match_top2_kernel", 0.0, 0.0);
            launch_match_top2(c->stream, c->m_jobs.as<MatchJob>(), 2 * k, max_n, splits, need_lo, need_top2, c->zero_page.as<half_t>());
            launch_match_finalize(c->stream, fins_dev, k, max_n, splits, conf->flavour, conf->do_mutual_check,
                                  conf->ratio_threshold, conf->distance_threshold);
        }
        prof_step_end(c);
        HIPCHECK(hipGetLastError());
    }
    if (!out_on_device) {
        if (copy_out(c, matches0, c->m_out_m.p, (size_t)n0 * sizeof(long long), 0)) return -1;
        if (copy_out(c, scores0, c->m_out_s.p, (size_t)n0 * sizeof(float), 0)) return -1;
    }
    HIPCHECK(hipStreamSynchronize(c->stream));
    return 0;
}

extern "C" int sfd2_match(sfd2_ctx *c, const void *d0, int n0, const void *d1, int n1, int dim, int dtype, int layout,
                          int on_device, const sfd2_match_conf *conf, int64_t *matches0, float *scores0, int out_on_device)
{
    const sfd2_desc_set q = {d0, n0, dtype, layout, on_device, nullptr, 0, 0};
    const sfd2_desc_set db = {d1, n1, dtype, layout, on_device, nullptr, 0, 0};
    return sfd2_match_batch(c, &q, &db, 1, dim, conf, matches0, scores0, out_on_device, 0);
}
```

sfd2_amd/csrc/match_kernels.hip:

```cpp
#include "sfd2_internal.h"
#include <math.h>
#include <stdlib.h>

#define NT 256
#define KD 128
#define TA 64
#define APITCH 136

__global__ __launch_bounds__(NT)
void match_prep_kernel(const void *__restrict__ src, int n, int n_src, const int *__restrict__ rows, int dim, int dtype,
                       int layout, half_t *__restrict__ hi, half_t *__restrict__ lo)
{
    const size_t t = (size_t)blockIdx.x * blockDim.x + threadIdx.x;
    if (t >= (size_t)n * KD) return;
    const int i = (int)(t / KD), d = (int)(t % KD);
    double v = 0.0;
    if (d < dim) {
        const int r = rows ? rows[i] : i;
        const size_t off = layout == 0 ? (size_t)r * dim + d : (size_t)d * n_src + r;
        if (dtype == 0) v = (double)reinterpret_cast<const float *>(src)[off];
        else if (dtype == 1) v = reinterpret_cast<const double *>(src)[off];
        else v = (double)(float)reinterpret_cast<const half_t *>(src)[off];
    }
    const half_t h = (half_t)(float)v;
// ... 120 lines not shown
    const float c1 = __shfl_xor(b1, 32), c2 = __shfl_xor(b2, 32);
    const int j1 = __shfl_xor(i1, 32);
    float n1v, n2v;
    int n1i;
    if (c1 > b1 || (c1 == b1 && j1 < i1)) { n1v = c1; n1i = j1; n2v = fmaxf(b1, c2); }
    else { n1v = b1; n1i = i1; n2v = fmaxf(b2, c1); }
    if (lane < 32 && my_i < nb) {
        const size_t o = (size_t)blockIdx.y * nb + my_i;
        job.part_v1[o] = n1v;
        job.part_v2[o] = n2v;
        job.part_i1[o] = n1i;
    }
}

typedef __attribute__((address_space(3))) void lds_void_t;
typedef const __attribute__((address_space(1))) void gbl_void_t;

#define TA2 64
template <bool NEED2, int ABL = 0>
__global__ __launch_bounds__(NT, 2)
void match_top2_v2_kernel(const MatchJob *__restrict__ jobs, int splits, const half_t *__restrict__ zero_page)
{
    extern __shared__ __attribute__((aligned(16))) unsigned char smem[];
    const MatchJob job = jobs[blockIdx.z];
    const int na = job.na, nb = job.nb;
    const int i_base = blockIdx.x * 256;
    if (i_base >= nb) return;
    const int tid = threadIdx.x, lane = tid & 63;
    const int wave = __builtin_amdgcn_readfirstlane(tid >> 6);
    const int lcol = lane & 31, lhi = lane >> 5;

    int chunk = (na + splits - 1) / splits;
    chunk = (chunk + 31) & ~31;
    const int ja0 = blockIdx.y * chunk;
    int ja1 = ja0 + chunk;
    if (ja1 > na) ja1 = na;

    h8_t bq[2][8];
#pragma unroll
    for (int t = 0; t < 2; ++t) {
        const int qi = i_base + wave * 64 + t * 32 + lcol;
#pragma unroll
        for (int ks = 0; ks < 8; ++ks) {
            h8_t z;
#pragma unroll
            for (int e = 0; e < 8; ++e) z[e] = (half_t)0.0f;
            bq[t][ks] = z;
            if (qi < nb) bq[t][ks] = *reinterpret_cast<const h8_t *>(job.b_hi + (size_t)qi * KD + ks * 16 + lhi * 8);
        }
    }
    float b1[2] = {-INFINITY, -INFINITY}, b2[2] = {-INFINITY, -INFINITY};
    int i1[2] = {0, 0};
    f32x16_t zero16;
#pragma unroll
    for (int r = 0; r < 16; ++r) zero16[r] = 0.0f;
    float bp[2] = {-INFINITY, -INFINITY};
    int sid[2] = {0, 0};

    if (ja0 < ja1) {
        const int nst = (ja1 - ja0 + TA2 - 1) / TA2;
        const int srow = lane >> 4;
#define ISSUE_A(stage_, buf_)                                                                            \
    _Pragma("unroll") for (int c = 0; c < TA2 / 16; ++c) {                                               \
        const int row = (wave * (TA2 / 16) + c) * 4 + srow;                                                       \
        const int slot = (lane & 15) ^ (row & 15);                                                       \
        const int ja = ja0 + (stage_)*TA2 + row;                                                          \
        const half_t *src = ja < ja1 ? job.a_hi + (size_t)ja * KD + slot * 8 : zero_page + (lane & 3) * 8; \
        __builtin_amdgcn_global_load_lds((gbl_void_t *)src,                                              \
                                         (lds_void_t *)(smem + (buf_)*TA2 * 256 + (wave * (TA2 / 16) + c) * 1024), 16, 0, 0); \
    }
        ISSUE_A(0, 0)
        SFD2_BARRIER_DRAIN();
        for (int s = 0; s < nst; ++s) {
            const int buf = s & 1;
            if (s + 1 < nst) { ISSUE_A(s + 1, buf ^ 1) }
#pragma unroll
            for (int sub = 0; sub < TA2 / 32; ++sub) {
                f32x16_t acc0 = zero16, acc1 = zero16;
                const int row = sub * 32 + lcol;
                const unsigned char *arow = smem + (buf * TA2 + row) * 256;
                const int sw = row & 15;
#pragma unroll
                for (int ks = 0; ks < 8; ++ks) {
                    const h8_t a = *reinterpret_cast<const h8_t *>(arow + (((ks * 2 + lhi) ^ sw) << 4));
                    acc0 = __builtin_amdgcn_mfma_f32_32x32x16_f16(a, bq[0][ks], acc0, 0, 0, 0);
                    acc1 = __builtin_amdgcn_mfma_f32_32x32x16_f16(a, bq[1][ks], acc1, 0, 0, 0);
                }
                const int jbase = ja0 + s * TA2 + sub * 32 + 4 * lhi;
                const bool full = ja0 + s * TA2 + sub * 32 + 32 <= ja1;
                if (ABL == 1) {
                    bp[0] = fmaxf(bp[0], acc0[0] + acc0[5] + acc0[10] + acc0[15]);
                    bp[1] = fmaxf(bp[1], acc1[0] + acc1[5] + acc1[10] + acc1[15]);
                } else if (!NEED2 && full) {
                    const int sub_id = s * (TA2 / 32) + sub;
                    float m0 = -INFINITY, m1 = -INFINITY;
#pragma unroll
                    for (int r = 0; r < 16; ++r) {
                        const float p0 = __uint_as_float((__float_as_uint(acc0[r]) & 0xFFFFFFF0u) | (unsigned)(15 - r));
                        const float p1 = __uint_as_float((__float_as_uint(acc1[r]) & 0xFFFFFFF0u) | (unsigned)(15 - r));
                        m0 = fmaxf(m0, p0);
                        m1 = fmaxf(m1, p1);
                    }
                    sid[0] = m0 > bp[0] ? sub_id : sid[0]; bp[0] = fmaxf(bp[0], m0);
                    sid[1] = m1 > bp[1] ? sub_id : sid[1]; bp[1] = fmaxf(bp[1], m1);
                } else {
#pragma unroll
                    for (int r = 0; r < 16; ++r) {
                        const int j = jbase + (r & 3) + 8 * (r >> 2);
                        const bool in = j < ja1;
                        const float v0 = in ? acc0[r] : -INFINITY, v1 = in ? acc1[r] : -INFINITY;
                        if (NEED2) {
                            top2_update(v0, j, b1[0], b2[0], i1[0]);
                            top2_update(v1, j, b1[1], b2[1], i1[1]);
                        } else {
                            i1[0] = v0 > b1[0] ? j : i1[0]; b1[0] = fmaxf(b1[0], v0);
                            i1[1] = v1 > b1[1] ? j : i1[1]; b1[1] = fmaxf(b1[1], v1);
                        }
                    }
                }
            }
            SFD2_BARRIER_DRAIN();
        }
#undef ISSUE_A
    }
    if (!NEED2) {
#pragma unroll
        for (int t = 0; t < 2; ++t) {
            const unsigned int bits = __float_as_uint(bp[t]);
            const float v = __uint_as_float(bits & 0xFFFFFFF0u);
            const int r = 15 - (int)(bits & 15u);
            const int j = ja0 + sid[t] * 32 + (r & 3) + 8 * (r >> 2) + 4 * lhi;
            if (bp[t] != -INFINITY && (v > b1[t] || (v == b1[t] && j < i1[t]))) { b1[t] = v; i1[t] = j; }
        }
    }
#pragma unroll
    for (int t = 0; t < 2; ++t) {
        const float c1 = __shfl_xor(b1[t], 32), c2 = __shfl_xor(b2[t], 32);
        const int j1 = __shfl_xor(i1[t], 32);
        float n1v, n2v;
        int n1i;
        if (c1 > b1[t] || (c1 == b1[t] && j1 < i1[t])) { n1v = c1; n1i = j1; n2v = fmaxf(b1[t], c2); }
        else { n1v = b1[t]; n1i = i1[t]; n2v = fmaxf(b2[t], c1); }
        const int qi = i_base + wave * 64 + t * 32 + lcol;
        if (lane < 32 && qi < nb) {
            const size_t o = (size_t)blockIdx.y * nb + qi;
            job.part_v1[o] = n1v;
            job.part_v2[o] = NEED2 ? n2v : -INFINITY;
            job.part_i1[o] = n1i;
        }
    }
}

#define MQ_NEG (-0x1p100f)
void launch_match_mutual_gemm(hipStream_t st, const MatchJob2 *jobs_dev, int npairs, int max_n0, int splits, int fwd_ids);
int match_mutual_strip(void);

__global__ __launch_bounds__(NT)
void match_mutual_reduce_kernel(const MatchJob2 *__restrict__ jobs, const MatchFinal *__restrict__ fins, int splits, int strip, int fwd_ids)
{
    const MatchJob2 job = jobs[blockIdx.y];
    const MatchFinal f = fins[blockIdx.y];
    const int dir = blockIdx.z;
    const int n = dir == 0 ? job.n0 : job.n1;
    const int i = blockIdx.x * blockDim.x + threadIdx.x;
    if (i >= n) return;
    float b1 = -INFINITY;
    int bi = 0;
    if (dir == 0) {
        for (int s = 0; s < splits; ++s) {
            const float c1 = job.part_v1[(size_t)s * n + i];
            if (c1 > b1) { b1 = c1; if (fwd_ids) bi = job.part_i1[(size_t)s * n + i]; }
        }
        if (!fwd_ids) bi = -1;
        f.red_f[i] = b1;
        f.red_f[(size_t)n + i] = -INFINITY;
        reinterpret_cast<int *>(f.red_f)[2 * (size_t)n + i] = bi;
    } else {
        const int nstrip = (job.n0 + strip - 1) / strip;
        float best = MQ_NEG;
        unsigned int bkey = __float_as_uint(MQ_NEG);
        int bs = 0;
        int sidx = 0;
        for (; sidx + 8 <= nstrip; sidx += 8) {
            float k[8];
#pragma unroll
            for (int u = 0; u < 8; ++u) k[u] = job.rkeys[(size_t)(sidx + u) * n + i];
#pragma unroll
            for (int u = 0; u < 8; ++u) {
                const float v = __uint_as_float(__float_as_uint(k[u]) & 0xFFFFFF00u);
                if (v > best) { best = v; bkey = __float_as_uint(k[u]); bs = sidx + u; }
            }
        }
        for (; sidx < nstrip; ++sidx) {
            const float k = job.rkeys[(size_t)sidx * n + i];
            const float v = __uint_as_float(__float_as_uint(k) & 0xFFFFFF00u);
            if (v > best) { best = v; bkey = __float_as_uint(k); bs = sidx; }
        }
        const unsigned int bits = bkey;
        const bool any = best > MQ_NEG;
        f.red_r[i] = any ? __uint_as_float(bits & 0xFFFFFF00u) : -INFINITY;
        f.red_r[(size_t)n + i] = -INFINITY;
        reinterpret_cast<int *>(f.red_r)[2 * (size_t)n + i] = any ? bs * strip + 255 - (int)(bits & 255u) : 0;
    }
}

__global__ __launch_bounds__(NT)
void match_mutual_claim_kernel(const MatchFinal *__restrict__ fins)
{
    const MatchFinal f = fins[blockIdx.y];
    const int j = blockIdx.x * blockDim.x + threadIdx.x;
    if (j >= f.n1) return;
    const float r = f.red_r[j];
    if (!(r > -INFINITY)) return;
    const int i = reinterpret_cast<const int *>(f.red_r)[2 * (size_t)f.n1 + j];
    if ((__float_as_uint(f.red_f[i]) & 0xFFFFFF00u) == __float_as_uint(r))
        atomicMin(reinterpret_cast<unsigned int *>(f.red_f) + 2 * (size_t)f.n0 + i, (unsigned int)j);
}

void launch_match_mutual(hipStream_t st, const MatchJob2 *jobs_dev, const MatchFinal *fins_dev, int npairs, int max_n0,
                         int max_n1, int splits, int fwd_ids)
{
    if (npairs <= 0 || max_n0 <= 0) return;
    launch_match_mutual_gemm(st, jobs_dev, npairs, max_n0, splits, fwd_ids);
    const int max_n = max_n0 > max_n1 ? max_n0 : max_n1;
    hipLaunchKernelGGL(match_mutual_reduce_kernel, dim3((max_n + NT - 1) / NT, npairs, 2), dim3(NT), 0, st, jobs_dev, fins_dev, splits,
                       match_mutual_strip(), fwd_ids);
    if (!fwd_ids && max_n1 > 0)
        hipLaunchKernelGGL(match_mutual_claim_kernel, dim3((max_n1 + NT - 1) / NT, npairs), dim3(NT), 0, st, fins_dev);
}

void launch_match_top2(hipStream_t st, const MatchJob *jobs_dev, int njobs, int max_nb, int splits, int use_lo,
                       int need_top2, const half_t *zero_page)
{
    if (njobs <= 0 || max_nb <= 0) return;
    static bool attr_done = false;
    const size_t lds_hi = (size_t)2 * TA * APITCH * sizeof(half_t);
    if (!attr_done) {
        (void)hipFuncSetAttribute(reinterpret_cast<const void *>(match_top2_kernel<true>),
                                  hipFuncAttributeMaxDynamicSharedMemorySize, (int)(2 * lds_hi));
        attr_done = true;
    }
    if (!use_lo && zero_page && sfd2_env("SFD2_MATCH_V1") == nullptr) {
        const dim3 grid((max_nb + 255) / 256, splits, njobs);
        const size_t lds = (size_t)2 * TA2 * 256;
        static bool attr2 = false;
        if (!attr2) {
            (void)hipFuncSetAttribute(reinterpret_cast<const void *>(match_top2_v2_kernel<true>), hipFuncAttributeMaxDynamicSharedMemorySize, (int)lds);
            (void)hipFuncSetAttribute(reinterpret_cast<const void *>(match_top2_v2_kernel<false>), hipFuncAttributeMaxDynamicSharedMemorySize, (int)lds);
#ifdef SFD2_EXPERIMENTS
            (void)hipFuncSetAttribute(reinterpret_cast<const void *>(match_top2_v2_kernel<false, 1>), hipFuncAttributeMaxDynamicSharedMemorySize, (int)lds);
#endif
            attr2 = true;
        }
        if (need_top2) hipLaunchKernelGGL(match_top2_v2_kernel<true>, grid, dim3(NT), lds, st, jobs_dev, splits, zero_page);
#ifdef SFD2_EXPERIMENTS
        else if (sfd2_env("SFD2_MATCH_ABLATE")) hipLaunchKernelGGL((match_top2_v2_kernel<false, 1>), grid, dim3(NT), lds, st, jobs_dev, splits, zero_page);
#endif
        else hipLaunchKernelGGL(match_top2_v2_kernel<false>, grid, dim3(NT), lds, st, jobs_dev, splits, zero_page);
        return;
    }
    const dim3 grid((max_nb + 127) / 128, splits, njobs);
    if (use_lo) hipLaunchKernelGGL(match_top2_kernel<true>, grid, dim3(NT), 2 * lds_hi, st, jobs_dev, splits);
    else hipLaunchKernelGGL(match_top2_kernel<false>, grid, dim3(NT), lds_hi, st, jobs_dev, splits);
}

__global__ __launch_bounds__(NT)
void match_reduce_kernel(const MatchFinal *__restrict__ fins, int splits)
{
    const MatchFinal f = fins[blockIdx.y];
    const int dir = blockIdx.z;
    const int n = dir == 0 ? f.n0 : f.n1;
    const int i = blockIdx.x * blockDim.x + threadIdx.x;
    if (i >= n) return;
    const float *v1 = dir == 0 ? f.f_v1 : f.r_v1;
    const float *v2 = dir == 0 ? f.f_v2 : f.r_v2;
    const int *i1 = dir == 0 ? f.f_i1 : f.r_i1;
    float *red = dir == 0 ? f.red_f : f.red_r;
    float b1 = -INFINITY, b2 = -INFINITY;
    int bi = 0;
    for (int s = 0; s < splits; ++s) {
        const float c1 = v1[(size_t)s * n + i], c2 = v2[(size_t)s * n + i];
        const int ci = i1[(size_t)s * n + i];
        if (c1 > b1) { b2 = fmaxf(b1, c2); b1 = c1; bi = ci; }
        else { b2 = fmaxf(b2, c1); }
    }
    red[i] = b1;
    red[(size_t)n + i] = b2;
    reinterpret_cast<int *>(red)[2 * (size_t)n + i] = bi;
}

__device__ __forceinline__ bool hloc_pass(float s1, float s2, float ratio, float dist)
{
    const float d0 = 2.0f * (1.0f - s1), d1 = 2.0f * (1.0f - s2);
    bool ok = true;
    if (ratio > 0.0f) ok = ok && (d0 <= (ratio * ratio) * d1);
    if (dist > 0.0f) ok = ok && (d0 <= dist * dist);
    return ok;
}
__device__ __forceinline__ float lowe_ratio(float s1, float s2)
{
    const float d0 = sqrtf(fmaxf(2.0f - 2.0f * s1, 0.0f)), d1 = sqrtf(fmaxf(2.0f - 2.0f * s2, 0.0f));
    return d0 / (d1 + 1e-8f);
}

__global__ __launch_bounds__(NT)
void match_decide_kernel(const MatchFinal *__restrict__ fins, int flavour, int mutual, float ratio, float dist)
{
    const MatchFinal f = fins[blockIdx.y];
    const int i = blockIdx.x * blockDim.x + threadIdx.x;
    if (i >= f.n0) return;
    const float s1 = f.red_f[i], s2 = f.red_f[(size_t)f.n0 + i];
    const int j = reinterpret_cast<const int *>(f.red_f)[2 * (size_t)f.n0 + i];
    long long m = -1;
    float score = 0.0f;
    if (f.n1 > 0 && j < 0) {
        score = flavour == 0 ? (hloc_pass(s1, s2, ratio, dist) ? (s1 + 1.0f) / 2.0f : 0.0f) : s1;
    } else if (f.n1 > 0) {
        const float t1 = f.red_r[j], t2 = f.red_r[(size_t)f.n1 + j];
        const int back = reinterpret_cast<const int *>(f.red_r)[2 * (size_t)f.n1 + j];
        if (flavour == 0) {
            const bool ok = hloc_pass(s1, s2, ratio, dist);
            score = ok ? (s1 + 1.0f) / 2.0f : 0.0f;
            m = ok ? j : -1;
            if (ok && mutual) {
                const bool ok_back = hloc_pass(t1, t2, ratio, dist);
                if (!(ok_back && back == i)) m = -1;
            }
        } else if (flavour == 1) {
            score = s1;
            m = (back == i) ? j : -1;
        } else {
            score = s1;
            const bool ok = (back == i) && lowe_ratio(s1, s2) <= ratio && lowe_ratio(t1, t2) <= ratio;
            m = ok ? j : -1;
        }
    }
    const long long mm = (m >= 0 && f.remap) ? (long long)f.remap[m] : m;
    if (f.out16) {
        reinterpret_cast<short *>(f.matches0)[i] = (short)mm;
        reinterpret_cast<half_t *>(f.scores0)[i] = (half_t)score;
    } else {
        f.matches0[i] = mm;
        f.scores0[i] = score;
    }
}

void launch_match_decide(hipStream_t st, const MatchFinal *fin_dev, int npairs, int max_n, int flavour, int mutual,
                         float ratio, float dist)
{
    if (npairs <= 0 || max_n <= 0) return;
    hipLaunchKernelGGL(match_decide_kernel, dim3((max_n + NT - 1) / NT, npairs), dim3(NT), 0, st, fin_dev, flavour,
                       mutual, ratio, dist);
}

void launch_match_finalize(hipStream_t st, const MatchFinal *fin_dev, int npairs, int max_n, int splits, int flavour,
                           int mutual, float ratio, float dist)
{
    if (npairs <= 0 || max_n <= 0) return;
    hipLaunchKernelGGL(match_reduce_kernel, dim3((max_n + NT - 1) / NT, npairs, 2), dim3(NT), 0, st, fin_dev, splits);
    hipLaunchKernelGGL(match_decide_kernel, dim3((max_n + NT - 1) / NT, npairs), dim3(NT), 0, st, fin_dev, flavour,
                       mutual, ratio, dist);
}
```

sfd2_amd/csrc/match_mutual_kernel.hip:

```cpp
#include "sfd2_internal.h"
#include <math.h>

#define NT 256
#define KD 128
#define TA2 64
typedef __attribute__((address_space(3))) void lds_void_t;
typedef const __attribute__((address_space(1))) void gbl_void_t;

#ifdef SFD2_MQ_NO_TSWZ
#define MQ_TSWZ(q_) 0
#else
#define MQ_TSWZ(q_) (((q_) >> 1) & 7)
#endif
#define MQ_NEG (-0x1p100f)
#define MQ_TILE_BITS 7
#define MQ_MAX_CHUNK (32 << MQ_TILE_BITS)

template <bool FWD_IDS>
__global__ __launch_bounds__(NT, 2)
void match_mutual_kernel(const MatchJob2 *__restrict__ jobs, int splits, int qblocks)
{
    extern __shared__ __attribute__((aligned(16))) unsigned char smem[];
    int swz;
    {
        const int bid = (int)blockIdx.x, nblk = (int)gridDim.x;
        const int q = nblk >> 3, r = nblk & 7, xcd = bid & 7, local = bid >> 3;
        swz = (xcd < r ? xcd * (q + 1) : r * (q + 1) + (xcd - r) * q) + local;
    }
    const int bx = swz % qblocks, by = (swz / qblocks) % splits, bz = swz / (qblocks * splits);
    const MatchJob2 job = jobs[bz];
    const int n1 = job.n1, n0 = job.n0;
    const int i_base = bx * 256;
    if (i_base >= n0) return;
    const int tid = threadIdx.x, lane = tid & 63;
    const int wave = __builtin_amdgcn_readfirstlane(tid >> 6);
    const int lcol = lane & 31, lhi = lane >> 5;

    int chunk = (n1 + splits - 1) / splits;
    chunk = (chunk + 31) & ~31;
    const int ja0 = by * chunk;
    int ja1 = ja0 + chunk;
    if (ja1 > n1) ja1 = n1;

    const int q0 = i_base + wave * 64;
    const bool wave_active = q0 < n0;
    const bool partial_q = q0 + 64 > n0;
    h8_t aq[2][8];
#pragma unroll
    for (int t = 0; t < 2; ++t) {
        const int qi = q0 + t * 32 + lcol;
#pragma unroll
        for (int ks = 0; ks < 8; ++ks) {
            h8_t z;
#pragma unroll
            for (int e = 0; e < 8; ++e) z[e] = (half_t)0.0f;
            aq[t][ks] = z;
            if (qi < n0) aq[t][ks] = *reinterpret_cast<const h8_t *>(job.q_hi + (size_t)qi * KD + ks * 16 + lhi * 8);
        }
    }
    float rm[2][16];
#pragma unroll
    for (int t = 0; t < 2; ++t)
#pragma unroll
        for (int r = 0; r < 16; ++r) rm[t][r] = MQ_NEG;
    f32x16_t zero16;
#pragma unroll
    for (int r = 0; r < 16; ++r) zero16[r] = 0.0f;
    const unsigned int wb = (3u - (unsigned)wave) << 6;
    const unsigned int cb[2] = {wb | 0x20u | ((1u - (unsigned)lhi) << 2), wb | ((1u - (unsigned)lhi) << 2)};
    float *rtab = reinterpret_cast<float *>(smem + 2 * TA2 * 256);
    for (int i = tid; i < ja1 - ja0; i += NT) rtab[i] = MQ_NEG;
    const unsigned rt_lane = (unsigned)(size_t)(const lds_void_t *)rtab + (unsigned)lcol * 4u;
    unsigned int keep = ~((1u << MQ_TILE_BITS) - 1u);
    asm volatile("" : "+v"(keep));

    const unsigned char *brow = smem + lcol * 256;
    const int bsw = lcol & 15;
#define MQ_BFRAG(BUF_, SUB_, KS_) \
    (*reinterpret_cast<const h8_t *>(brow + ((BUF_)*TA2 + (SUB_)*32) * 256 + ((((KS_)*2 + lhi) ^ bsw) << 4)))
#define MQ_TILE_MASK(C0_, C1_, TILE_)                                                                    \
    if (ja0 + (TILE_)*32 + 32 > ja1 || partial_q) {                                                      \
        int qlim_ = n0 - q0 - 4 * lhi;       \
        asm volatile("" : "+v"(qlim_)::"memory");                                                        \
        const bool pad_col_ = ja0 + (TILE_)*32 + lcol >= ja1;                                            \
        _Pragma("unroll") for (int r = 0; r < 16; ++r) {                                                 \
            const int qr_ = (r & 3) + 8 * (r >> 2);                                                      \
            if (pad_col_ || qr_ >= qlim_) C0_[r] = MQ_NEG;                                               \
            if (pad_col_ || qr_ + 32 >= qlim_) C1_[r] = MQ_NEG;                                          \
        }                                                                                                \
    }
#define MQ_TILE_REV(C0_, C1_, TILE_)                                                                     \
    {                                                                                                    \
        float m0_ = MQ_NEG, m1_ = MQ_NEG;                                                                \
        _Pragma("unroll") for (int r = 0; r < 16; ++r) {                                                 \
            m0_ = fmaxf(m0_, __uint_as_float((__float_as_uint(C0_[r]) & 0xFFFFFFE0u) | (unsigned)(((3 - (r >> 2)) << 3) | (3 - (r & 3))))); \
            m1_ = fmaxf(m1_, __uint_as_float((__float_as_uint(C1_[r]) & 0xFFFFFFE0u) | (unsigned)(((3 - (r >> 2)) << 3) | (3 - (r & 3))))); \
        }                                                                                                \
        const float k0_ = __uint_as_float((__float_as_uint(m0_) & 0xFFFFFF1Bu) | cb[0]);                 \
        const float k1_ = __uint_as_float((__float_as_uint(m1_) & 0xFFFFFF1Bu) | cb[1]);                 \
        const unsigned int kb_ = __float_as_uint(fmaxf(k0_, k1_));                                       \
        const auto sw2_ = __builtin_amdgcn_permlane32_swap(kb_, kb_, false, false);                      \
        const float kk_ = fmaxf(__uint_as_float(sw2_[0]), __uint_as_float(sw2_[1]));                     \
        asm volatile("ds_max_f32 %0, %1" ::"v"(rt_lane + (unsigned)(TILE_)*128u), "v"(kk_) : "memory");          \
    }
#ifdef SFD2_MQ_NO_PRIO
#define MQ_PRIO(p_)
#else
#define MQ_PRIO(p_) __builtin_amdgcn_s_setprio(p_);
#endif
#define MQ_STAGE(S_, BUF_)                                                                               \
    {                                                                                                    \
        f32x16_t a0_, a1_, b0_, b1_;                                                                     \
        h8_t fa_ = MQ_BFRAG(BUF_, 0, 0), fb_ = MQ_BFRAG(BUF_, 1, 0), na_ = fa_, nb_ = fb_;               \
        MQ_PRIO(1)                                                                                       \
        _Pragma("unroll") for (int ks = 0; ks < 8; ++ks) {                                               \
                     \
            if (ks + 1 < 8) { na_ = MQ_BFRAG(BUF_, 0, ks + 1); nb_ = MQ_BFRAG(BUF_, 1, ks + 1); }        \
            __builtin_amdgcn_sched_barrier(0);                                                           \
            a0_ = __builtin_amdgcn_mfma_f32_32x32x16_f16(aq[0][ks], fa_, ks == 0 ? zero16 : a0_, 0, 0, 0); \
            a1_ = __builtin_amdgcn_mfma_f32_32x32x16_f16(aq[1][ks], fa_, ks == 0 ? zero16 : a1_, 0, 0, 0); \
            b0_ = __builtin_amdgcn_mfma_f32_32x32x16_f16(aq[0][ks], fb_, ks == 0 ? zero16 : b0_, 0, 0, 0); \
            b1_ = __builtin_amdgcn_mfma_f32_32x32x16_f16(aq[1][ks], fb_, ks == 0 ? zero16 : b1_, 0, 0, 0); \
            __builtin_amdgcn_sched_barrier(0);                                                           \
            fa_ = na_; fb_ = nb_;                                                                        \
        }                                                                                                \
        MQ_PRIO(0)                                                                                       \
        const int ta_ = (S_)*2, tb_ = (S_)*2 + 1;                                                        \
        MQ_TILE_MASK(a0_, a1_, ta_)                                                                      \
        MQ_TILE_MASK(b0_, b1_, tb_)                                                                      \
        if (FWD_IDS) {                                                                                   \
            const unsigned int ca_ = (unsigned)((1 << MQ_TILE_BITS) - 1 - ta_), cb_ = ca_ - 1u;          \
            _Pragma("unroll") for (int r = 0; r < 16; ++r) {                                             \
                rm[0][r] = fmaxf(fmaxf(rm[0][r], __uint_as_float((__float_as_uint(a0_[r]) & keep) | ca_)), \
                                 __uint_as_float((__float_as_uint(b0_[r]) & keep) | cb_));               \
                rm[1][r] = fmaxf(fmaxf(rm[1][r], __uint_as_float((__float_as_uint(a1_[r]) & keep) | ca_)), \
                                 __uint_as_float((__float_as_uint(b1_[r]) & keep) | cb_));               \
            }                                                                                            \
        } else {                                                                                         \
            _Pragma("unroll") for (int r = 0; r < 16; ++r) {                                             \
                rm[0][r] = fmaxf(fmaxf(rm[0][r], a0_[r]), b0_[r]);                                       \
                rm[1][r] = fmaxf(fmaxf(rm[1][r], a1_[r]), b1_[r]);                                       \
            }                                                                                            \
        }                                                                                                \
        MQ_TILE_REV(a0_, a1_, ta_)                                                                       \
        MQ_TILE_REV(b0_, b1_, tb_)                                                                       \
    }

    if (ja0 < ja1) {
        const int nst = (ja1 - ja0 + TA2 - 1) / TA2;
        const __amdgpu_buffer_rsrc_t d_rsrc = __builtin_amdgcn_make_buffer_rsrc(const_cast<half_t *>(job.d_hi), 0, ja1 * (KD * 2), 0x00020000);
        int voff[TA2 / 16];
#pragma unroll
        for (int c = 0; c < TA2 / 16; ++c) {
            const int row = (wave * (TA2 / 16) + c) * 4 + (lane >> 4);
            voff[c] = (ja0 + row) * (KD * 2) + (((lane & 15) ^ (row & 15)) << 4);
        }
#define ISSUE_B(buf_)                                                                                    \
    _Pragma("unroll") for (int c = 0; c < TA2 / 16; ++c) {                                               \
        __builtin_amdgcn_raw_ptr_buffer_load_lds(d_rsrc, (lds_void_t *)(smem + (buf_)*TA2 * 256 + (wave * (TA2 / 16) + c) * 1024), \
                                                 16, voff[c], 0, 0, 0);                                  \
        voff[c] += TA2 * (KD * 2);                                                                       \
    }
        ISSUE_B(0)
        SFD2_BARRIER_DRAIN();
        for (int s = 0; s < nst; s += 2) {
            if (s + 1 < nst) { ISSUE_B(1) }
            if (wave_active) MQ_STAGE(s, 0)
            SFD2_BARRIER_DRAIN();
            if (s + 1 < nst) {
                if (s + 2 < nst) { ISSUE_B(0) }
                if (wave_active) MQ_STAGE(s + 1, 1)
                SFD2_BARRIER_DRAIN();
            }
        }
#undef ISSUE_B
        __syncthreads();
        float *rk = job.rkeys + (size_t)bx * n1 + ja0;
        for (int i = tid; i < ja1 - ja0; i += NT) rk[i] = rtab[i];
    }
#undef MQ_STAGE
#undef MQ_BFRAG
#undef MQ_TILE_MASK
#undef MQ_TILE_REV
    float *T = reinterpret_cast<float *>(smem) + wave * (64 * 32);
    if (wave_active) {
#pragma unroll
        for (int t = 0; t < 2; ++t)
#pragma unroll
            for (int r = 0; r < 16; ++r) {
                const int q = (r & 3) + 8 * (r >> 2) + 4 * lhi;
                T[(t * 32 + q) * 32 + (lcol ^ (MQ_TSWZ(q) << 2))] = rm[t][r];
            }
    }
    __syncthreads();
    if (wave_active && q0 + lane < n0) {
        float best = MQ_NEG;
        int col = 0;
#pragma unroll
        for (int c4 = 0; c4 < 8; ++c4) {
            const float4 v = *reinterpret_cast<const float4 *>(T + lane * 32 + ((c4 ^ MQ_TSWZ(lane)) << 2));
            if (v.x > best) { best = v.x; col = c4 * 4 + 0; }
            if (v.y > best) { best = v.y; col = c4 * 4 + 1; }
            if (v.z > best) { best = v.z; col = c4 * 4 + 2; }
            if (v.w > best) { best = v.w; col = c4 * 4 + 3; }
        }
        const unsigned int bits = __float_as_uint(best);
        const size_t o = (size_t)by * n0 + q0 + lane;
        const bool any = best > MQ_NEG;
        if (FWD_IDS) {
            const int tile = (1 << MQ_TILE_BITS) - 1 - (int)(bits & ((1u << MQ_TILE_BITS) - 1u));
            job.part_v1[o] = any ? __uint_as_float(bits & ~((1u << MQ_TILE_BITS) - 1u)) : -INFINITY;
            job.part_i1[o] = any ? ja0 + tile * 32 + col : 0;
        } else {
            job.part_v1[o] = any ? best : -INFINITY;
        }
    }
}

int match_mutual_strip(void) { return 256; }

void launch_match_mutual_gemm(hipStream_t st, const MatchJob2 *jobs_dev, int npairs, int max_n0, int splits, int fwd_ids)
{
    static bool attr = false;
    const size_t lds = (size_t)2 * TA2 * 256 + (size_t)MQ_MAX_CHUNK * sizeof(float);
    if (!attr) {
        (void)hipFuncSetAttribute(reinterpret_cast<const void *>(match_mutual_kernel<true>), hipFuncAttributeMaxDynamicSharedMemorySize, (int)lds);
        (void)hipFuncSetAttribute(reinterpret_cast<const void *>(match_mutual_kernel<false>), hipFuncAttributeMaxDynamicSharedMemorySize, (int)lds);
        attr = true;
    }
    const int qblocks = (max_n0 + 255) / 256;
    if (fwd_ids) hipLaunchKernelGGL(match_mutual_kernel<true>, dim3(qblocks * splits * npairs), dim3(NT), lds, st, jobs_dev, splits, qblocks);
    else hipLaunchKernelGGL(match_mutual_kernel<false>, dim3(qblocks * splits * npairs), dim3(NT), lds, st, jobs_dev, splits, qblocks);
}

int match_mutual_max_chunk(void) { return MQ_MAX_CHUNK; }
```

sfd2_amd/csrc/sfd2_ctx.h:

```cpp
#pragma once
#include "../../include/sfd2_hip.h"
#include "sfd2_internal.h"

#include <algorithm>
#include <atomic>
#include <cstdlib>
#include <cmath>
#include <cstdio>
#include <cstring>
#include <map>
#include <string>
#include <vector>

int sfd2_fail(const std::string &m);
#define fail sfd2_fail
#define HIPCHECK(expr)                                                                           \
    do {                                                                                          \
        hipError_t e_ = (expr);                                                                   \
        if (e_ != hipSuccess)                                                                     \
            return fail(std::string(#expr) + ": " + hipGetErrorString(e_) + " @" + std::to_string(__LINE__)); \
    } while (0)

extern std::atomic<unsigned long long> g_alloc_gen;

struct DevPtr {
    void *p = nullptr;
    size_t cap = 0;
    template <typename T> T *as() const { return reinterpret_cast<T *>(p); }
};
struct DevBuf : DevPtr {
    DevBuf() = default;
    DevBuf(const DevBuf &) = delete;
    DevBuf &operator=(const DevBuf &) = delete;
    DevBuf(DevBuf &&o) noexcept { p = o.p; cap = o.cap; o.p = nullptr; o.cap = 0; }
    DevBuf &operator=(DevBuf &&o) noexcept
    {
        if (this != &o) { release(); p = o.p; cap = o.cap; o.p = nullptr; o.cap = 0; }
        return *this;
    }
    ~DevBuf() { release(); }
    hipError_t ensure(size_t bytes)
    {
        if (bytes <= cap) return hipSuccess;
        ++g_alloc_gen;
        if (p) (void)hipFree(p);
        p = nullptr;
        cap = 0;
        hipError_t e = hipMalloc(&p, bytes);
        if (e == hipSuccess) cap = bytes;
        return e;
    }
    void release()
    {
        if (p) (void)hipFree(p);
        p = nullptr;
        cap = 0;
    }
};

struct ConvW {
    int cin = 0, cout = 0, cout_pad = 0, ks = 0, stride = 1;
    DevBuf w, scale, shift;
    DevBuf scale_rawin;
    DevBuf wsl;
    DevBuf wrm;
    DevBuf wfh, wfc, wfl;
    DevBuf wlk;
    DevBuf wgc;
    DevBuf wx3;
    DevBuf wx3p;
    DevBuf wc;
    int sbyte = 127;
    DevBuf wf8l;
    DevBuf wfr;
    DevBuf wc6;
    DevBuf sa6;
    size_t w_floats = 0;
    std::vector<float> h_scale, h_shift;
    std::vector<int> h_sa6;
    DevBuf wc66, sa66;
    std::vector<int> h_sa66;
};

enum { AE_CONV1A, AE_CONV1B, AE_CONV2A, AE_CONV2B, AE_CONV3A, AE_TRUNK ,
       AE_T1_0, AE_T1_1, AE_T1_2, AE_T2_0, AE_T2_1, AE_T2_2, AE_PA0, AE_DA0, AE_COUNT };

struct ActInfo { const void *p; int f32; int planar; int c, pitch, h, w; Rec rec = Rec::None;  int exp2 = 0;  bool absent = false;  };

struct JpegBuf {
    void *p = nullptr;
    size_t cap = 0;
    JpegBuf() = default;
    JpegBuf(const JpegBuf &) = delete;
    JpegBuf &operator=(const JpegBuf &) = delete;
    ~JpegBuf() { if (p) (void)hipFree(p); }
    template <typename T> T *as() const { return reinterpret_cast<T *>(p); }
};
struct JpegScratch {
    JpegBuf in[2];
    hipEvent_t ev_copied[2] = {}, ev_free[2] = {};
    int slot = 0;
    JpegBuf lanes, pre, coef, planes;
    JpegBuf words;
    ~JpegScratch()
    {
        for (int i = 0; i < 2; ++i) {
            if (ev_copied[i]) (void)hipEventDestroy(ev_copied[i]);
            if (ev_free[i]) (void)hipEventDestroy(ev_free[i]);
        }
    }
};

struct sfd2_ctx {
    int device = 0;
    hipStream_t stream = nullptr;
    hipEvent_t ev[4] = {nullptr, nullptr, nullptr, nullptr};
    hipEvent_t ev_jobs = nullptr;
    hipStream_t copy_stream = nullptr;
#define SFD2_IMG_SLOTS 4
    hipEvent_t ev_copied[SFD2_IMG_SLOTS] = {}, ev_img_free[SFD2_IMG_SLOTS] = {};
    DevBuf img2[SFD2_IMG_SLOTS];
    int img_slot = 0, img_slot_used = -1;
    void *pin_jobs = nullptr;
    size_t pin_cap = 0;
    bool weights_loaded = false;
    bool counters_clean = false;
    bool has_sta = false;
    int opt_alias = 1;
    int act_exp[AE_COUNT] = {};
    float act_max[AE_COUNT] = {};
    int opt_range_fallback = 1;
    int range_fallbacks = 0;
    int in_fallback = 0;
    int prof_step_entry = 0;
    float range_hist[SFD2_RS_COUNT] = {};
    int opt_auto_range = 1;
    std::vector<float> h_sta_w;
    int opt_cu_limit = 0;
    int fuse_det = 0;
    int use_graphs = 0;
    DevBuf x3_chain[2];
    DevBuf x3_rb_planes[3];
    int opt_fuse_post = 1;
    int opt_sparse_desc = 1;
    const half_t *da0_cur = nullptr;
    DevBuf da3_sparse;
    int opt_fp6_acts = 1;
    int net_error = 0;
    int opt_trunk_r1 = 1;
    int opt_s2d = 1;
    int opt_fp6_filters = 0;
    int opt_x3_pp = 1;
    int opt_auto_margin = 1;
    float margin_err[4] = {-1.0f, -1.0f, -1.0f, -1.0f};
    int margin_choice = -1;
    int opt_c3b_plain = 0;
    int user_c3b_plain = -1;
    bool margin_done = false, margin_pending = false;
    float relax_err = -1.0f;
    bool user_set_rb_inner = false, user_set_comp_heads = false;
    int user_rb_inner = 2, user_comp_heads = 0;
    int opt_x3_desc16 = 0;
    DevBuf x3_planes;
    DevBuf x3_da0_planes;
    DevBuf db_sparse;
    int opt_sparse_da3 = 1;
    int opt_fuse_pb = 1;
    const half_t *pa_cur = nullptr;
    const half_t *da_cur = nullptr;
    int opt_comp_rb = 1;
    int opt_rb_inner = 2;
    int opt_fuse_rb23 = 1;
    int opt_comp_det = 0;
    int opt_comp_heads = 0;
    int opt_no_rf_c = 0;
    int opt_generic_c = 0;
    int opt_branches = 0;
    int opt_sta_side = 0;
    hipStream_t side_stream = nullptr;
    hipStream_t cur_stream = nullptr;
    hipEvent_t ev_fork = nullptr, ev_join = nullptr;
    struct GraphEntry *graphs = nullptr;
    int n_graphs = 0;
    unsigned long long graph_clock = 0;
    ConvW c1a, c1b, c2a, c2b, c3a, c3b, rb1[3], rb2[3], rb3[3], pa0, pa3, da0, da3, pb, db;
    DevBuf sta_w16;
    DevPtr range_stat;
    DevPtr range_hist_dev;
    DevPtr extract_rec;
    DevBuf range_scratch;
    DevBuf sta_w, sta_b, zero_page, w1b_fused;
    DevBuf w1b_stem_c6;
    DevBuf w1b_stem_c;
    DevBuf w1b_stem_x3;
    int fuse = 1;
    int precision = SFD2_PREC_F16;
    ConvW f1a, f1b, f2a, f2b, f3a, f3b, frb1[3], frb2[3], frb3[3], fpa0, fpa3, fda0, fda3, fpb, fdb;
    DevBuf g1a, g1b, g2a, g2b, g3a, g3b, grt1[3], grt2[3], gro[3], gpa0_o, gpa_o, gda0_o, gda_o;
    int H = 0, W = 0, H2 = 0, W2 = 0, H4 = 0, W4 = 0, H8 = 0, W8 = 0;
    DevBuf img, a1a, a1b, a2a, a2b, a3a, a3b, rt1[3], rt2[3], ro[3], pa0_o, pa_o, da0_o, da_o;
    DevBuf logits , draw , sta , score , heat ;
    DevBuf stab , desc_nchw, tmp_f32;
    DevBuf cand, bnd, sel, sorted, counters, kpts, kscores, kdesc;
    DevBuf kdesc64;
    DevBuf g_keys, g_state0, g_state1, g_kept;
    int cand_cap = 0;
    int last_sel_cap = 0;
    float *kpts_cur = nullptr, *kscores_cur = nullptr;
    DevBuf arena;
    DevBuf img_u8_packed;
    JpegScratch jpeg;
    JpegBuf pose_in, pose_ws, pose_out;
    DevBuf img_scaled, ms_kp, ms_sc, ms_de, ms_keys, ms_sorted, ms_cnt;
    unsigned int ms_cand_seen[8] = {};
    int ms_cand_cap[8] = {};
    DevBuf m_stage, m_hi0, m_lo0, m_hi1, m_lo1, m_part_f, m_part_i, m_red, m_jobs, m_fins, m_out_m, m_out_s, m_rkeys;
    sfd2_timings tim = {};
    std::map<std::string, ActInfo> acts;
    int prof_max_steps = 0, prof_step = 0, prof_slot = 0;
    std::vector<hipEvent_t> prof_ev;
    std::vector<sfd2_layer_timing> prof_tab;
    std::vector<int> prof_used;
    std::vector<int> prof_row;
    std::string prof_filter;
};

void graphs_release(sfd2_ctx *c);
#define PROF_SLOTS 48
struct ProfScope {
    sfd2_ctx *c; int slot;
    ProfScope(sfd2_ctx *c_, const char *name, const char *kernel, double flops, double bytes) : c(c_), slot(-1)
    {
        if (c->prof_max_steps <= 0 || c->prof_step >= c->prof_max_steps || c->prof_slot >= PROF_SLOTS) return;
        if (!c->prof_filter.empty() && strstr(kernel, c->prof_filter.c_str()) == nullptr) return;
        slot = c->prof_slot++;
        int row = -1;
        for (size_t i = 0; i < c->prof_tab.size(); ++i)
            if (strncmp(c->prof_tab[i].name, name, sizeof(c->prof_tab[i].name) - 1) == 0) { row = (int)i; break; }
        if (row < 0) {
            c->prof_tab.push_back(sfd2_layer_timing{});
            row = (int)c->prof_tab.size() - 1;
            snprintf(c->prof_tab[row].name, sizeof(c->prof_tab[row].name), "%s", name);
            snprintf(c->prof_tab[row].kernel, sizeof(c->prof_tab[row].kernel), "%s", kernel);
        }
        c->prof_tab[row].flops = flops;
        c->prof_tab[row].bytes = bytes;
        c->prof_row[(size_t)c->prof_step * PROF_SLOTS + slot] = row;
        (void)hipEventRecord(c->prof_ev[((size_t)c->prof_step * PROF_SLOTS + slot) * 2], c->cur_stream);
    }
    void cancel()
    {
        if (slot >= 0 && slot == c->prof_slot - 1) c->prof_slot--;
        slot = -1;
    }
    ~ProfScope()
    {
        if (slot >= 0) (void)hipEventRecord(c->prof_ev[((size_t)c->prof_step * PROF_SLOTS + slot) * 2 + 1], c->cur_stream);
    }
};
static inline void prof_step_begin(sfd2_ctx *c) { c->prof_slot = 0; }
static inline void prof_step_end(sfd2_ctx *c)
{
    if (c->prof_max_steps > 0 && c->prof_step < c->prof_max_steps) {
        c->prof_used[c->prof_step] = c->prof_slot;
        c->prof_step++;
    }
}

int apply_act_exponents(sfd2_ctx *c);
int read_range_status(sfd2_ctx *c, sfd2_range_status *out, int reset);
int range_wants_fallback(sfd2_ctx *c);
int range_fold_before_sync_extract(sfd2_ctx *c);
int sfd2_margin_selfcheck_if_pending(sfd2_ctx *c);
int reset_range_records(sfd2_ctx *c);
struct FallbackScope {
    sfd2_ctx *c; int prec;
    explicit FallbackScope(sfd2_ctx *c_) : c(c_), prec(c_->precision)
    {
        c->precision = SFD2_PREC_F16X3; c->in_fallback = 1; c->range_fallbacks++;
        if (c->prof_step > c->prof_step_entry) c->prof_step = c->prof_step_entry;
    }
    ~FallbackScope() { c->precision = prec; c->in_fallback = 0; }
};
enum PassEntry { PASS_DET , PASS_DENSE , PASS_EXTRACT  };
enum StrictLayer { SL_C1B, SL_C2A, SL_C2B, SL_C3A, SL_C3B, SL_RB1, SL_RB3 = SL_RB1 + 3, SL_PA0 = SL_RB3 + 3, SL_PA3, SL_PB, SL_DA0, SL_DA3, SL_DB, SL_COUNT };
template <class Ctx> auto &strict_layer(Ctx *c, int i)
{
    decltype(&c->f1b) t[] = {&c->f1b, &c->f2a, &c->f2b, &c->f3a, &c->f3b, &c->frb1[0], &c->frb1[1], &c->frb1[2], &c->frb3[0], &c->frb3[1], &c->frb3[2],
                             &c->fpa0, &c->fpa3, &c->fpb, &c->fda0, &c->fda3, &c->fdb};
    static_assert(sizeof(t) == SL_COUNT * sizeof(t[0]), "one entry per StrictLayer");
// ... 34 lines not shown
```

sfd2_amd/csrc/sfd2_internal.h:

```cpp
#pragma once
#include <hip/hip_runtime.h>
#include <hip/hip_fp16.h>
#include <stdint.h>

#ifdef SFD2_EXPERIMENTS
#include <stdlib.h>
static inline const char *sfd2_env(const char *name) { return getenv(name); }
#else
static inline const char *sfd2_env(const char *) { return nullptr; }
#endif

extern thread_local int g_sfd2_cu_limit;
static inline int sfd2_slots(int cus) { return (g_sfd2_cu_limit > 0 && g_sfd2_cu_limit < cus) ? g_sfd2_cu_limit : cus; }

#define SFD2_BARRIER_DRAIN() asm volatile("s_waitcnt vmcnt(0) lgkmcnt(0)\n\ts_barrier" ::: "memory")

typedef _Float16 half_t;
typedef _Float16 h8_t __attribute__((ext_vector_type(8)));
typedef _Float16 h4_t __attribute__((ext_vector_type(4)));
typedef float f32x16_t __attribute__((ext_vector_type(16)));

#ifdef __HIPCC__
__device__ __forceinline__ float4 sfd2_lds_f4(const float *p)
{
    const h8_t raw = *reinterpret_cast<const h8_t *>(reinterpret_cast<const unsigned char *>(p));
    float4 r;
    __builtin_memcpy(&r, &raw, 16);
    return r;
}
#endif
typedef float f32x4_t __attribute__((ext_vector_type(4)));

#define SFD2_C_XL_SHIFT 9
#define SFD2_C_XH_SCALE 0.25f
typedef int v8i_t __attribute__((ext_vector_type(8)));
typedef int v4i_t __attribute__((ext_vector_type(4)));
#ifdef __HIPCC__
__device__ __forceinline__ v8i_t sfd2_cat8(h8_t a, h8_t b)
{
    v4i_t x, y;
    __builtin_memcpy(&x, &a, 16);
    __builtin_memcpy(&y, &b, 16);
    return __builtin_shufflevector(x, y, 0, 1, 2, 3, 4, 5, 6, 7);
}
__device__ __forceinline__ h8_t sfd2_half8(v8i_t v, int kk)
{
    const v4i_t x = kk ? __builtin_shufflevector(v, v, 4, 5, 6, 7) : __builtin_shufflevector(v, v, 0, 1, 2, 3);
    h8_t r;
    __builtin_memcpy(&r, &x, 16);
    return r;
}
__device__ __forceinline__ f32x16_t sfd2_mfma_corr(h8_t a0, h8_t a1, h8_t b0, h8_t b1, f32x16_t acc, int sa)
{
    return __builtin_amdgcn_mfma_scale_f32_32x32x64_f8f6f4(sfd2_cat8(a0, a1), sfd2_cat8(b0, b1), acc, 0, 0, 0, sa, 0, 0x7f7f7f7f);
}
__device__ __forceinline__ void sfd2_mfma_corr_tied(f32x16_t &acc, v8i_t a, v8i_t b, int sa, int sb)
{
    asm volatile("v_mfma_scale_f32_32x32x64_f8f6f4 %0, %1, %2, %0, %3, %4 op_sel_hi:[0,0,0]" : "+v"(acc) : "v"(a), "v"(b), "v"(sa), "v"(sb));
}
__device__ __forceinline__ void sfd2_mfma_unit2(f32x16_t &c0, f32x16_t &c1, h8_t a0, h8_t a1, v8i_t a8, v8i_t b0, v8i_t b1, int sa, int sb, int f8)
{
    const h8_t b00 = sfd2_half8(b0, 0), b01 = sfd2_half8(b0, 1), b10 = sfd2_half8(b1, 0), b11 = sfd2_half8(b1, 1);
    asm volatile("s_cmp_lg_u32 %11, 0\n\t"
                 "s_cbranch_scc1 .Lsfd2_u8_%=\n\t"
                 "v_mfma_f32_32x32x16_f16 %0, %2, %5, %0\n\t"
                 "v_mfma_f32_32x32x16_f16 %1, %2, %7, %1\n\t"
                 "v_mfma_f32_32x32x16_f16 %0, %3, %6, %0\n\t"
                 "v_mfma_f32_32x32x16_f16 %1, %3, %8, %1\n\t"
                 "s_branch .Lsfd2_ue_%=\n"
                 ".Lsfd2_u8_%=:\n\t"
                 "v_mfma_scale_f32_32x32x64_f8f6f4 %0, %4, %12, %0, %9, %10 op_sel_hi:[0,0,0]\n\t"
                 "v_mfma_scale_f32_32x32x64_f8f6f4 %1, %4, %13, %1, %9, %10 op_sel_hi:[0,0,0]\n"
                 ".Lsfd2_ue_%=:"
                 : "+v"(c0), "+v"(c1)
                 : "v"(a0), "v"(a1), "v"(a8), "v"(b00), "v"(b01), "v"(b10), "v"(b11), "v"(sa), "v"(sb), "s"(f8), "v"(b0), "v"(b1)
                 : "scc");
}
__device__ __forceinline__ void sfd2_mfma_settle() { asm volatile("s_nop 15\n\ts_nop 15" ::: "memory"); }
__device__ __forceinline__ unsigned sfd2_corr2(float v0, half_t h0, float v1, half_t h1)
{
    const float l0 = __builtin_amdgcn_fmed3f((v0 - (float)h0) * (float)(1 << SFD2_C_XL_SHIFT), -448.0f, 448.0f);
    const float l1 = __builtin_amdgcn_fmed3f((v1 - (float)h1) * (float)(1 << SFD2_C_XL_SHIFT), -448.0f, 448.0f);
    const float x0 = __builtin_amdgcn_fmed3f(v0 * SFD2_C_XH_SCALE, -448.0f, 448.0f);
    const float x1 = __builtin_amdgcn_fmed3f(v1 * SFD2_C_XH_SCALE, -448.0f, 448.0f);
    int d = __builtin_amdgcn_cvt_pk_fp8_f32(l0, x0, 0, false);
    d = __builtin_amdgcn_cvt_pk_fp8_f32(l1, x1, d, true);
    return (unsigned)d;
}
__device__ __forceinline__ void sfd2_split4(float v0, float v1, float v2, float v3, uint2 &hv, uint2 &cv)
{
    h4_t h;
    h[0] = (half_t)v0; h[1] = (half_t)v1; h[2] = (half_t)v2; h[3] = (half_t)v3;
    __builtin_memcpy(&hv, &h, 8);
    cv.x = sfd2_corr2(v0, h[0], v1, h[1]);
    cv.y = sfd2_corr2(v2, h[2], v3, h[3]);
}
#define SFD2_C_SAT 1792.0f
typedef float f32x2_t __attribute__((ext_vector_type(2)));
typedef _Float16 h2_t __attribute__((ext_vector_type(2)));
__device__ __forceinline__ unsigned sfd2_corr2v(f32x2_t v, h2_t h)
{
    const f32x2_t hf = {(float)h[0], (float)h[1]};
    const f32x2_t l = (v - hf) * (float)(1 << SFD2_C_XL_SHIFT);
    const f32x2_t x = v * SFD2_C_XH_SCALE;
    int d = __builtin_amdgcn_cvt_pk_fp8_f32(l[0], x[0], 0, false);
    d = __builtin_amdgcn_cvt_pk_fp8_f32(l[1], x[1], d, true);
    return (unsigned)d;
}
#define SFD2_RANGE_SUB 16
#define SFD2_ZERO_PAGE_BYTES 1024
enum { SFD2_RS_CONV1A, SFD2_RS_CONV1B, SFD2_RS_CONV2A, SFD2_RS_CONV2B, SFD2_RS_CONV3A, SFD2_RS_CONV3B, SFD2_RS_T1_0, SFD2_RS_T1_1, SFD2_RS_T1_2,
       SFD2_RS_T2_0, SFD2_RS_T2_1, SFD2_RS_T2_2, SFD2_RS_OUT_0, SFD2_RS_OUT_1, SFD2_RS_OUT_2, SFD2_RS_PA0, SFD2_RS_DA0, SFD2_RS_COUNT };
__device__ __forceinline__ float sfd2_max3(float m, float a, float b) { return __builtin_fmaxf(__builtin_fmaxf(m, a), b); }
__device__ __forceinline__ unsigned int sfd2_wave_max_bits(float mx)
{
#ifdef SFD2_NO_RANGE
    return 0u;
#endif
    int v = __float_as_int(__builtin_fmaxf(mx, 0.0f));
#define SFD2_DPP_MAX(ctrl_, rmask_) { const int o_ = __builtin_amdgcn_update_dpp(0, v, ctrl_, rmask_, 0xf, false); v = o_ > v ? o_ : v; }
    SFD2_DPP_MAX(0x111, 0xf)
    SFD2_DPP_MAX(0x112, 0xf)
    SFD2_DPP_MAX(0x114, 0xf)
    SFD2_DPP_MAX(0x118, 0xf)
    SFD2_DPP_MAX(0x142, 0xa)
    SFD2_DPP_MAX(0x143, 0xc)
#undef SFD2_DPP_MAX
    return (unsigned int)__builtin_amdgcn_readlane(v, 63);
}
__device__ __forceinline__ void sfd2_range_commit(unsigned int *slot , unsigned int wave_bits)
{
    if (slot == nullptr || wave_bits == 0u) return;
    unsigned int *w = slot + (blockIdx.x & (SFD2_RANGE_SUB - 1));
    if ((threadIdx.x & 63) == 0) {
        const unsigned int cur = __hip_atomic_load(w, __ATOMIC_RELAXED, __HIP_MEMORY_SCOPE_AGENT);
        if (wave_bits > cur) atomicMax(w, wave_bits);
    }
}

__device__ __forceinline__ void sfd2_track_h4(uint2 hv, unsigned int &mxh)
{
    h2_t a, b, m;
    __builtin_memcpy(&a, &hv.x, 4);
    __builtin_memcpy(&b, &hv.y, 4);
    __builtin_memcpy(&m, &mxh, 4);
    m = __builtin_elementwise_max(__builtin_elementwise_max(m, a), b);
    __builtin_memcpy(&mxh, &m, 4);
}
__device__ __forceinline__ float sfd2_h2_max(unsigned int mxh)
{
    h2_t m;
    __builtin_memcpy(&m, &mxh, 4);
    return __builtin_fmaxf((float)m[0], (float)m[1]);
}

template <bool ADD, bool TRACK = true>
// ... 165 lines not shown
                   const half_t *res, const half_t *res_c, half_t *out, half_t *out_c, const half_t *zero_page,
                   unsigned int *range_t2, unsigned int *range_out, Rec rres, Rec rout ,
                   const half_t *w3l8, int sbyte3 );
void launch_conv1x1_c256_x3(hipStream_t st, const half_t *in, const half_t *in_lo, int npix, const half_t *w, const half_t *wl,
                            const float *scale, const float *shift, int relu, const void *res, const half_t *res_lo, float *out, half_t *out_hi,
                            half_t *out_lo, const half_t *zero_page);
void launch_conv1a_c(hipStream_t st, const float *img, int H, int W, int normalise, const half_t *wpk ,
                     const float *scale, const float *shift, half_t *out, half_t *out_c, unsigned int *range = nullptr);
void launch_gconv_c(hipStream_t st, const half_t *in, const half_t *in_c, int H, int W, const half_t *wpk ,
                    const void *wck , const float *scale, const float *shift, half_t *out, half_t *out_c, int sbyte,
                    int row0, int row1 , unsigned int *range = nullptr);
void launch_nhwc_hc_to_nchw_f(hipStream_t st, const half_t *in, const half_t *in_c, int npix, int pitch, int c, float *out, Rec rec );

void launch_conv_igemm_f32(hipStream_t st, const float *in, int H, int W, int Cin, const float *wpk,
                           const float *scale, const float *shift, int Cout_pad, int ks, int stride, int relu,
                           const float *residual, float *out, int Ho, int Wo);
void launch_x3_split(hipStream_t st, const float *w, size_t n_floats, void *out);
void launch_x3_split_planes(hipStream_t st, const float *in, size_t n_floats, void *hi_out, void *lo_out);
void launch_conv3x3_pp_x3(hipStream_t st, const half_t *in, const half_t *in_lo, int H, int W, int Cin, const half_t *wpk,
                          const float *scale, const float *shift, int CoutP, int relu, half_t *out_hi, half_t *out_lo, float *out_f32,
                          int Ho, int Wo, const half_t *zero_page, int s2d = 0 );
void launch_gconv_x3_pack(hipStream_t st, const float *w , void *out );
void launch_gconv_x3(hipStream_t st, const float *in, int H, int W, const void *wpk, const float *scale, const float *shift, float *out);
void launch_conv_igemm_x3(hipStream_t st, const float *in, int H, int W, int Cin, const float *wpk,
                           const float *scale, const float *shift, int Cout_pad, int ks, int stride, int relu,
                           const float *residual, float *out, int Ho, int Wo);
void launch_conv1a_f32(hipStream_t st, const float *img_chw, int H, int W, int normalise, const float *w ,
                       const float *scale, const float *shift, float *out );
void launch_gconv_f32(hipStream_t st, const float *in, int H, int W, const float *w , const float *scale,
                      const float *shift, float *out);
void launch_convsta_f32(hipStream_t st, const float *in, int npix, const float *w, const float *b, float *out);

void launch_detector_head(hipStream_t st, const float *logits, int pitch, int hc, int wc, float *score);
void launch_heatmap(hipStream_t st, const float *score, int hs, int ws, const float *sta, int hc, int wc,
                    int H, int W, float *heat, float *stab_out );
bool launch_nms_select(hipStream_t st, const float *heat, int H, int W, int radius, float conf_th, int border, int Hb, int Wb,
                       float *nms_dense , unsigned long long *cand_keys, int cand_cap,
                       unsigned int *counters , int fuse_threshold = 0, int top_k = 0);
void launch_heads_heat(hipStream_t st, const float *logits, int pitch, int hc8, int wc8, const float *sta, int hc, int wc,
                       int H, int W, float *heat);
void launch_topk_sort(hipStream_t st, bool threshold_done, const unsigned long long *cand, int cand_cap, int top_k,
                      unsigned long long *sel, unsigned long long *sorted, int sel_cap, unsigned int *counters,
                      unsigned long long *bnd, int W, float *kpts, float *scores);
#define SFD2_HIST_BINS 4096
#define SFD2_COUNTER_BYTES (64 + SFD2_HIST_BINS * 4)
__device__ __forceinline__ unsigned int key_bin(unsigned long long key)
{
    const int b = (int)((unsigned int)(key >> 47) & 0xFFFFu) - ((127 - 12) << 8);
    return (unsigned int)(b < 0 ? 0 : (b > SFD2_HIST_BINS - 1 ? SFD2_HIST_BINS - 1 : b));
}

__device__ __forceinline__ unsigned int sfd2_ld_agent(const unsigned int *p)
{
    return __hip_atomic_load(p, __ATOMIC_RELAXED, __HIP_MEMORY_SCOPE_AGENT);
}

template <bool COHERENT>
__device__ __forceinline__ void sfd2_select_threshold(int cand_cap, int top_k, unsigned int *__restrict__ counters, unsigned int *wsum)
{
    static_assert(SFD2_HIST_BINS == 4096, "one uint4 of bins per thread");
    const unsigned int *hist = counters + 16;
    unsigned int n = COHERENT ? sfd2_ld_agent(counters) : counters[0];
    if (n > (unsigned int)cand_cap) n = cand_cap;
    const unsigned int k = (top_k <= 0 || (unsigned int)top_k > n) ? n : (unsigned int)top_k;
    if (k == n) {
        if (threadIdx.x == 0) { counters[1] = n; counters[2] = 0; counters[3] = 0; counters[4] = 0; counters[5] = 0; counters[6] = 1; }
        return;
    }
    const int t = threadIdx.x, lane = t & 63, wave = t >> 6;
    uint4 hv;
    if (COHERENT) hv = make_uint4(sfd2_ld_agent(hist + 4 * t), sfd2_ld_agent(hist + 4 * t + 1), sfd2_ld_agent(hist + 4 * t + 2), sfd2_ld_agent(hist + 4 * t + 3));
    else hv = reinterpret_cast<const uint4 *>(hist)[t];
    const unsigned int sum = hv.x + hv.y + hv.z + hv.w;
    unsigned int suf = sum;
#pragma unroll
    for (int d = 1; d < 64; d <<= 1) {
        const unsigned int o = __shfl_down(suf, d);
        if (lane + d < 64) suf += o;
    }
    if (lane == 0) wsum[wave] = suf;
    __syncthreads();
    unsigned int higher = 0;
    for (int w = wave + 1; w < 16; ++w) higher += wsum[w];
    const unsigned int above_incl = higher + suf;
    unsigned int above = above_incl - sum;
    if (above < k && above_incl >= k) {
        const unsigned int b[4] = {hv.x, hv.y, hv.z, hv.w};
#pragma unroll
        for (int j = 3; j >= 0; --j) {
            if (above < k && above + b[j] >= k) {
                counters[1] = k; counters[2] = 0; counters[3] = 0;
                counters[4] = 4 * t + j;
                counters[5] = k - above;
                counters[6] = 0;
            }
            above += b[j];
        }
    }
}

void launch_nms4_select(hipStream_t st, const float *heat, int H, int W, float conf_th, int border, int Hb, int Wb, float *nms_dense,
                        unsigned long long *cand, int cand_cap, unsigned int *counters, unsigned int *hist, int fuse_threshold, int top_k);
void launch_greedy_init(hipStream_t st, const float *heat, int n, float conf_th, unsigned long long *keys, unsigned char *state);
void launch_greedy_iter(hipStream_t st, const unsigned long long *keys, const unsigned char *sin, unsigned char *sout,
                        int H, int W, int dist, unsigned int *undecided);
void launch_greedy_final(hipStream_t st, const float *heat, const unsigned char *state, int n, float *kept);
void launch_keys_to_kpts(hipStream_t st, const unsigned long long *sorted_keys, const unsigned int *counters,
                         int W, float *kpts_xy, float *scores, int cap);
void launch_sample_desc(hipStream_t st, const float *desc_nhwc, int hc, int wc, int nh, int nw,
                        const float *kpts_xy, const unsigned int *count , int n_max,
                        float *out, int compact = 0);
void launch_pb_heads_heat(hipStream_t st, const half_t *fmap, int hc8, int wc8, const half_t *wpk, int CoutP, const float *scale,
                          const float *shift, const float *sta, int hc, int wc, int H, int W, float *heat,
                          unsigned int *zero_words , int n_zero);
bool pb_heads_heat_clears(int hc8, int wc8, int n_zero);
void launch_desc_store64(hipStream_t st, const float *in , const unsigned int *count, int n_max, double *out , int pitch);
void launch_desc_head(hipStream_t st, const half_t *fmap, int hc, int wc, int nh, int nw, const half_t *wpk, int CoutP,
                      const float *scale, const float *shift, const float *kpts, const unsigned int *count, int n_max, float *out, int compact = 0);
void launch_desc_normalise_nchw(hipStream_t st, const float *desc_nhwc, int npix, float *out_nchw);
void launch_nhwc_h_to_nchw_f(hipStream_t st, const half_t *in, int npix, int c_pitch, int c, float *out);
void launch_nhwc_f_to_nchw_f(hipStream_t st, const float *in, int npix, int c_pitch, int c, float *out);
void launch_nchw_f_to_nhwc_f(hipStream_t st, const float *in, int npix, int c, float *out);

void launch_scale_inplace(hipStream_t st, float *p, size_t n, float mul);
void launch_absmax_f32(hipStream_t st, const float *in, size_t n, unsigned int *out);

void launch_ingest_u8(hipStream_t st, const unsigned char *src, int H, int W, int bgr, int nh, int nw, float *out);
void launch_unpack_rgbx(hipStream_t st, const unsigned char *src, unsigned char *dst, size_t npix);
void launch_extract_record(hipStream_t st, unsigned int *range_stat, unsigned int *hist, const unsigned int *counters, int sel_cap,
                           int cand_cap, unsigned int *rec );

void launch_match_prep(hipStream_t st, const void *src, int n, int n_src, const int *rows, int dim, int dtype, int layout,
                       half_t *hi, half_t *lo);
struct MatchJob {
    const half_t *a_hi;
    const half_t *a_lo;
    const half_t *b_hi;
    const half_t *b_lo;
    int na, nb;
    float *part_v1;
    float *part_v2;
    int *part_i1;
};
void launch_match_top2(hipStream_t st, const MatchJob *jobs_dev, int njobs, int max_nb, int splits, int use_lo,
                       int need_top2, const half_t *zero_page);
struct MatchJob2 {
    const half_t *q_hi;
    const half_t *d_hi;
    int n0, n1;
    float *part_v1;
    int *part_i1;
    float *rkeys;
};
struct MatchFinal;
void launch_match_mutual(hipStream_t st, const MatchJob2 *jobs_dev, const MatchFinal *fins_dev, int npairs, int max_n0,
                         int max_n1, int splits, int fwd_ids);
int match_mutual_max_chunk(void);
int match_mutual_strip(void);
void launch_match_decide(hipStream_t st, const MatchFinal *fin_dev, int npairs, int max_n, int flavour, int mutual,
                         float ratio, float dist);
struct MatchFinal {
    const float *f_v1, *f_v2; const int *f_i1;
    const float *r_v1, *r_v2; const int *r_i1;
    int n0, n1;
    int out16, pad_;
    long long *matches0; float *scores0;
    float *red_f;
    float *red_r;
    const int *remap;
};
void launch_match_finalize(hipStream_t st, const MatchFinal *fin_dev, int npairs, int max_n, int splits,
                           int flavour, int mutual, float ratio, float dist);

void launch_conv1x1_c256(hipStream_t st, const half_t *in, int npix, const half_t *w_rowmajor, const float *scale,
                         const float *shift, int relu, const half_t *res, half_t *out, const half_t *zero_page);

void launch_resblock(hipStream_t st, const half_t *x, int H, int W, const half_t *w1, const float *sc1, const float *sh1,
                     const half_t *wg, const float *sc2, const float *sh2, const half_t *w3, const float *sc3, const float *sh3,
                     half_t *out, const half_t *zero_page);

void launch_norm_resize(hipStream_t st, const float *img, int mode, int H, int W, int nh, int nw, float *out);
void launch_ms_append(hipStream_t st, const float *kpts, const float *scores, const unsigned int *count, int cap, int W, int nw,
                      int H, int nh, float *kp_out, float *sc_out, unsigned int *level_count);
void launch_ms_merge(hipStream_t st, int n_levels, const int *offsets, const unsigned int *level_count, const float *kp_stage,
                     const float *sc_stage, const float *de_stage, int cap_total, int top_k, unsigned long long *keys,
                     unsigned long long *sorted, unsigned int *ms_counters, int n_max, float *kp_out, float *sc_out, float *de_out);

#define SFD2_JPEG_LANE_BITS 256
#define SFD2_JPEG_SYNC_LAUNCHES 12
#define SFD2_JPEG_BAD_CODE 1u
#define SFD2_JPEG_BAD_COUNT 2u
#define SFD2_JPEG_BAD_END 4u
#define SFD2_JPEG_NO_SYNC 8u
struct JpegHuff {
    uint16_t lut[512];
    int32_t maxcode[18];
    int32_t valoff[18];
    uint8_t vals[256];
};
struct JpegTables {
    JpegHuff huff[3][2];
    uint16_t q[3][64];
};
static inline int64_t jpeg_tail_bytes(int64_t lanes, int64_t intervals)
{
    return (int64_t)sizeof(JpegTables) + 4 * (lanes + 1) + 4 * lanes + 4 * (intervals + 1);
}
struct JpegGeom {
    int ncomp, bpm, mcus_x, total_blocks, ri_blocks , nlanes, nint;
    uint32_t ecs_words;
    int unit_comp[10], unit_dx[10], unit_dy[10];
    int hs[3], vs[3];
    int bw[3], bh[3];
    int blk_base[3];
    int64_t plane_off[3];
    int W, H, mode;
    int cw, ch;
};
struct JpegLane {
    uint32_t spos, epos;
    int32_t su, eu, bad, cnt;
    int32_t dc[3];
    int32_t pad;
};
void launch_jpeg_decode(hipStream_t st, const unsigned char *in, int64_t tab_off, const JpegGeom &g, JpegLane *lanes, int *lane_pre,
                        int *wg_pre, unsigned int *sync_flags, short *coef, unsigned char *planes, unsigned char *out_rgbx,
                        unsigned int *status);

#define SFD2_POSE_WG 256
struct PoseCam {
    double f[2], c[2];
    double k1, k2, p1, p2;
    int32_t distorted, pad;
};
struct PoseProbDev {
    int64_t off;
    int32_t n, pad;
    PoseCam cam;
    double thresh2;
    double qt[7];
};
struct PoseConfDev {
    int64_t max_trials, min_trials;
    double confidence;
    uint64_t seed;
    int32_t refine_only, pad;
};
struct PoseResDev {
    double q[4], t[3];
    int32_t success, num_inliers, num_trials, pad;
};
void launch_pose(hipStream_t st, const PoseProbDev *probs, int k, const PoseConfDev &conf, const double *p2, const double *p3, float4 *xf4,
                 float2 *xf2, double2 *xn, double *hyp, const unsigned char *mask_in, unsigned char *mask_out, PoseResDev *res);
```

Baseline: 729.0.

## Replace fixed split grid in mutual matcher with host-planned balanced segment schedule

The mutual-match GEMM no longer launches a fixed grid of query-block by split by pair. A host planner now divides all (pair, strip, column-tile) work units evenly across a persistent grid of about two blocks per CU, interleaved across XCDs, and emits segment descriptors that are staged to the device with the job buffers. A new finalize path, fused by default, replaces the separate decide kernel. This aims to fix load imbalance and tail effects when pair sizes vary, at the cost of host-side planning work per call, larger descriptor uploads and more LDS per block.

Result: no change. 729.3, median of 3 (+0.0%).

```diff
diff --git a/include/sfd2_hip.h b/include/sfd2_hip.h
--- a/include/sfd2_hip.h
+++ b/include/sfd2_hip.h
@@ -123,6 +123,8 @@
 int sfd2_match_segments(sfd2_ctx *ctx, const void *d0, int n0, const void *d1, int n1, int dim,
                         int dtype, int layout, int on_device, int n_seg, const int32_t *seg0, const int32_t *seg1,
                         const sfd2_match_conf *conf, int64_t *matches0, float *scores0, int out_on_device);
+
+int sfd2_match_plan(const int32_t *n0, const int32_t *n1, int k, int slots, int32_t *segs, int cap_segs, int *n_blocks);
 
 typedef struct {
     const void *data;
diff --git a/sfd2_amd/_lib.py b/sfd2_amd/_lib.py
--- a/sfd2_amd/_lib.py
+++ b/sfd2_amd/_lib.py
@@ -97,7 +97,7 @@
     "sfd2_select_keypoints", "sfd2_sample_descriptors", "sfd2_heatmap", "sfd2_debug_activation",
     "sfd2_match", "sfd2_match_batch", "sfd2_get_timings", "sfd2_sync", "sfd2_set_profiling",
     "sfd2_get_layer_timings", "sfd2_set_precision", "sfd2_extract_spp", "sfd2_nms_fast",
-    "sfd2_set_profile_filter", "sfd2_extract_multiscale", "sfd2_set_option", "sfd2_extract_match", "sfd2_preprocess", "sfd2_extract_spp_levels", "sfd2_match_segments",
+    "sfd2_set_profile_filter", "sfd2_extract_multiscale", "sfd2_set_option", "sfd2_extract_match", "sfd2_preprocess", "sfd2_extract_spp_levels", "sfd2_match_segments", "sfd2_match_plan",
     "sfd2_get_range_status", "sfd2_range_tensor_name", "sfd2_calibrate_range", "sfd2_get_act_exponents", "sfd2_set_act_exponents",
     "sfd2_extract_record_async", "sfd2_desc_pack", "sfd2_get_margin_status", "sfd2_get_relax_status", "sfd2_get_option", "sfd2_device_pci_bus_id",
     "sfd2_jpeg_parse", "sfd2_jpeg_prepare", "sfd2_jpeg_decode", "sfd2_absolute_pose_batch", "sfd2_pose_refine_batch",
@@ -149,6 +149,8 @@
     lib.sfd2_heatmap.argtypes = [vp, vp, ci, ci, vp, ci, ci, ci, ci, vp]
     lib.sfd2_debug_activation.argtypes = [vp, ctypes.c_char_p, vp, i64, pi, pi, pi]
     lib.sfd2_match.argtypes = [vp, vp, ci, vp, ci, ci, ci, ci, ci, ctypes.POINTER(MatchConf), vp, vp, ci]
+    if hasattr(lib, "sfd2_match_plan"):
+        lib.sfd2_match_plan.argtypes = [vp, vp, ci, ci, vp, ci, pi]
     lib.sfd2_match_segments.argtypes = [vp, vp, ci, vp, ci, ci, ci, ci, ci, ci, vp, vp, ctypes.POINTER(MatchConf), vp, vp, ci]
     lib.sfd2_match_batch.argtypes = [vp, ctypes.POINTER(DescSet), ctypes.POINTER(DescSet), ci, ci,
                                      ctypes.POINTER(MatchConf), vp, vp, ci, ci]
@@ -181,11 +183,27 @@
     lib.sfd2_absolute_pose_batch.argtypes = [vp, ctypes.POINTER(PoseProblem), ci, ctypes.POINTER(PoseConf), ctypes.POINTER(PoseResult), vp, ci]
     lib.sfd2_pose_refine_batch.argtypes = [vp, ctypes.POINTER(PoseProblem), ci, vp, vp, ctypes.POINTER(PoseResult), ci]
     for name in EXPORTS:
+        if name == "sfd2_match_plan" and LIB_PATH != os.path.join(_HERE, "libsfd2hip.so"):
+            continue
         getattr(lib, name)
     if lib.sfd2_version() < 109:
         raise RuntimeError(f"{LIB_PATH} is version {lib.sfd2_version()}, this binding needs >= 109 (rebuild: __graft_entry__.build())")
     _lib = lib
     return lib
+
+
+def match_plan(n0, n1, slots=0):
+    lib = load()
+    n0 = np.ascontiguousarray(n0, dtype=np.int32)
+    n1 = np.ascontiguousarray(n1, dtype=np.int32)
+    assert n0.shape == n1.shape and n0.ndim == 1
+    nb = ctypes.c_int()
+    n = lib.sfd2_match_plan(n0.ctypes.data, n1.ctypes.data, len(n0), slots, None, 0, ctypes.byref(nb))
+    if n < 0:
+        raise RuntimeError("sfd2_match_plan failed")
+    segs = np.zeros((n, 6), dtype=np.int32)
+    lib.sfd2_match_plan(n0.ctypes.data, n1.ctypes.data, len(n0), slots, segs.ctypes.data, n, ctypes.byref(nb))
+    return segs, nb.value
 
 
 def check(rc):
diff --git a/sfd2_amd/csrc/api_core.hip b/sfd2_amd/csrc/api_core.hip
--- a/sfd2_amd/csrc/api_core.hip
+++ b/sfd2_amd/csrc/api_core.hip
@@ -113,6 +113,7 @@
     else if (k == "sparse_desc") c->opt_sparse_desc = value ? 1 : 0;
     else if (k == "sparse_da3") c->opt_sparse_da3 = value ? 1 : 0;
     else if (k == "cu_limit") c->opt_cu_limit = value < 0 ? 0 : value;
+    else if (k == "match_fused_finalize") c->opt_match_fused_finalize = value ? 1 : 0;
     else if (k == "auto_range") c->opt_auto_range = value ? 1 : 0;
     else if (k == "range_fallback") c->opt_range_fallback = value ? 1 : 0;
     else if (k == "x3_pp") c->opt_x3_pp = value ? 1 : 0;
@@ -141,7 +142,7 @@
     const std::string k(key);
     const struct { const char *name; int v; } tab[] = {
         {"fuse", c->fuse}, {"fuse_det", c->fuse_det}, {"alias", c->opt_alias}, {"graphs", c->use_graphs}, {"branches", c->opt_branches}, {"sta_side", c->opt_sta_side},
-        {"fuse_post", c->opt_fuse_post}, {"sparse_desc", c->opt_sparse_desc}, {"sparse_da3", c->opt_sparse_da3}, {"cu_limit", c->opt_cu_limit},
+        {"fuse_post", c->opt_fuse_post}, {"sparse_desc", c->opt_sparse_desc}, {"sparse_da3", c->opt_sparse_da3}, {"cu_limit", c->opt_cu_limit}, {"match_fused_finalize", c->opt_match_fused_finalize},
         {"auto_range", c->opt_auto_range}, {"range_fallback", c->opt_range_fallback}, {"x3_pp", c->opt_x3_pp}, {"x3_desc16", c->opt_x3_desc16},
         {"auto_margin", c->opt_auto_margin}, {"fp6_filters", c->opt_fp6_filters}, {"fp6_acts", c->opt_fp6_acts}, {"s2d", c->opt_s2d},
         {"trunk_r1", c->opt_trunk_r1}, {"fuse_pb", c->opt_fuse_pb}, {"generic_c", c->opt_generic_c}, {"comp_rb", c->opt_comp_rb},
diff --git a/sfd2_amd/csrc/api_graph.hip b/sfd2_amd/csrc/api_graph.hip
--- a/sfd2_amd/csrc/api_graph.hip
+++ b/sfd2_amd/csrc/api_graph.hip
@@ -106,9 +106,10 @@
     }
     const size_t jb = 2 * (size_t)std::max(k, 1) * sizeof(MatchJob), fb = (size_t)std::max(k, 1) * sizeof(MatchFinal);
     if (!e->pin) {
-        HIPCHECK(hipHostMalloc(&e->pin, jb + fb, hipHostMallocDefault));
-        e->pin_cap = jb + fb;
-        HIPCHECK(e->jobs.ensure(jb + fb));
+        const size_t need = std::max(std::max(jb + fb, c->pin_cap), c->m_jobs.cap);
+        HIPCHECK(hipHostMalloc(&e->pin, need, hipHostMallocDefault));
+        e->pin_cap = need;
+        HIPCHECK(e->jobs.ensure(need));
     }
     HIPCHECK(hipStreamSynchronize(c->stream));
     HIPCHECK(hipEventSynchronize(c->ev_jobs));
diff --git a/sfd2_amd/csrc/api_match.hip b/sfd2_amd/csrc/api_match.hip
--- a/sfd2_amd/csrc/api_match.hip
+++ b/sfd2_amd/csrc/api_match.hip
@@ -1,6 +1,19 @@
 #include "sfd2_ctx.h"
 
 static size_t elt_size(int dtype) { return dtype == SFD2_DT_F64 ? 8 : (dtype == SFD2_DT_F16 ? 2 : 4); }
+
+static MatchPlanDev plan_stage(const MatchPlan &plan, char *host, char *dev)
+{
+    MatchPlanDev d = {nullptr, nullptr, nullptr, plan.nblk, plan.max_ns};
+    const size_t seg_bytes = (plan.segs.size() * sizeof(MatchSeg) + 15) & ~(size_t)15;
+    if (!plan.segs.empty()) memcpy(host, plan.segs.data(), plan.segs.size() * sizeof(MatchSeg));
+    if (!plan.blk_rng.empty()) memcpy(host + seg_bytes, plan.blk_rng.data(), plan.blk_rng.size() * sizeof(int));
+    if (!plan.fcnt.empty()) memcpy(host + seg_bytes + plan.blk_rng.size() * sizeof(int), plan.fcnt.data(), plan.fcnt.size() * sizeof(int));
+    d.segs = reinterpret_cast<const MatchSeg *>(dev);
+    d.blk_rng = reinterpret_cast<const int *>(dev + seg_bytes);
+    d.fcnt = d.blk_rng + plan.blk_rng.size();
+    return d;
+}
 
 static int prep_set(sfd2_ctx *c, const void *src, int n_src, const int32_t *rows, int n, int dim, int dtype, int layout,
                     int on_device, int need_lo, DevBuf &stage, size_t &stage_off, half_t *hi_dst, half_t *lo_dst,
@@ -114,13 +127,11 @@
     const int need_top2 = (conf->flavour == SFD2_MATCH_ITLOC_NNR) ||
                           (conf->flavour == SFD2_MATCH_HLOC && conf->ratio_threshold > 0.0f);
     const bool single_gemm = !need_lo && !need_top2 && sfd2_env("SFD2_MATCH_TWO_GEMM") == nullptr;
+    MatchPlan plan;
     if (single_gemm) {
-        const int qblocks = (n0 + 255) / 256;
-        splits = (512 * 6 + k * qblocks - 1) / (k * qblocks);
-        splits = std::max(1, std::min(splits, 8));
-        splits = std::min(splits, std::max(1, (std::max(1, max_n1) + 31) / 32));
-        if (const char *e = sfd2_env("SFD2_MATCH_SPLITS")) splits = std::max(1, std::min(16, atoi(e)));
-        splits = std::max(splits, (max_n1 + match_mutual_max_chunk() - 1) / match_mutual_max_chunk());
+        g_sfd2_cu_limit = c->opt_cu_limit;
+        std::vector<int> n0s((size_t)k, n0);
+        match_mutual_plan(n0s.data(), eff_n1.data(), k, match_mutual_slots(), plan);
     }
     const int nstrip = (n0 + match_mutual_strip() - 1) / match_mutual_strip();
 
@@ -129,12 +140,16 @@
     if (need_lo) HIPCHECK(c->m_lo0.ensure((size_t)n0 * 128 * 2));
     HIPCHECK(c->m_hi1.ensure(std::max<size_t>(tot_n1, 1) * 128 * 2));
     if (need_lo) HIPCHECK(c->m_lo1.ensure(std::max<size_t>(tot_n1, 1) * 128 * 2));
-    const size_t per_pair_f = (size_t)splits * n0, tot_part = (size_t)k * per_pair_f + (size_t)splits * tot_n1;
+    size_t tot_part = (size_t)k * splits * n0 + (size_t)splits * tot_n1;
+    if (single_gemm) {
+        tot_part = 0;
+        for (int i = 0; i < k; ++i) tot_part += (size_t)plan.fslots[i] * n0;
+    }
     HIPCHECK(c->m_part_f.ensure(std::max<size_t>(tot_part, 1) * 2 * sizeof(float)));
     HIPCHECK(c->m_part_i.ensure(std::max<size_t>(tot_part, 1) * sizeof(int)));
     if (single_gemm) HIPCHECK(c->m_rkeys.ensure(std::max<size_t>((size_t)nstrip * tot_n1, 1) * sizeof(float)));
     HIPCHECK(c->m_red.ensure(((size_t)k * n0 + tot_n1 + 1) * 3 * sizeof(float)));
-    HIPCHECK(c->m_jobs.ensure((size_t)2 * k * sizeof(MatchJob) + (size_t)k * sizeof(MatchFinal)));
+    HIPCHECK(c->m_jobs.ensure((size_t)2 * k * sizeof(MatchJob) + (size_t)k * sizeof(MatchFinal) + 16 + plan.bytes()));
     HIPCHECK(c->m_out_m.ensure((size_t)k * n0 * sizeof(long long)));
     HIPCHECK(c->m_out_s.ensure((size_t)k * n0 * sizeof(float)));
 
@@ -145,21 +160,24 @@
     if (prep_set(c, q->data, n0, nullptr, n0, dim, q->dtype, q->layout, q->on_device, need_lo, c->m_stage, stage_off,
                  c->m_hi0.as<half_t>(), c->m_lo0.as<half_t>(), &q_hi, &q_lo)) return -1;
     static_assert(sizeof(MatchJob2) <= 2 * sizeof(MatchJob), "descriptor buffer sizing");
-    const size_t jobs_bytes = 2 * (size_t)k * sizeof(MatchJob), fins_bytes = (size_t)k * sizeof(MatchFinal);
+    const size_t jobs_bytes = 2 * (size_t)k * sizeof(MatchJob), fins_bytes = ((size_t)k * sizeof(MatchFinal) + 15) & ~(size_t)15;
+    const size_t plan_bytes = plan.bytes();
     hipStreamCaptureStatus cap_status = hipStreamCaptureStatusNone;
     (void)hipStreamIsCapturing(c->stream, &cap_status);
     const bool capturing = cap_status != hipStreamCaptureStatusNone;
     if (!capturing) HIPCHECK(hipEventSynchronize(c->ev_jobs));
-    if (jobs_bytes + fins_bytes > c->pin_cap) {
+    if (jobs_bytes + fins_bytes + plan_bytes > c->pin_cap) {
         if (c->pin_jobs) (void)hipHostFree(c->pin_jobs);
         c->pin_jobs = nullptr;
         c->pin_cap = 0;
-        HIPCHECK(hipHostMalloc(&c->pin_jobs, jobs_bytes + fins_bytes, hipHostMallocDefault));
-        c->pin_cap = jobs_bytes + fins_bytes;
+        HIPCHECK(hipHostMalloc(&c->pin_jobs, jobs_bytes + fins_bytes + plan_bytes, hipHostMallocDefault));
+        c->pin_cap = jobs_bytes + fins_bytes + plan_bytes;
     }
     MatchJob *jobs = reinterpret_cast<MatchJob *>(c->pin_jobs);
     MatchJob2 *jobs2 = reinterpret_cast<MatchJob2 *>(c->pin_jobs);
     MatchFinal *fins = reinterpret_cast<MatchFinal *>(reinterpret_cast<char *>(c->pin_jobs) + jobs_bytes);
+    const MatchPlanDev plan_dev = plan_stage(plan, reinterpret_cast<char *>(c->pin_jobs) + jobs_bytes + fins_bytes,
+                                             static_cast<char *>(c->m_jobs.p) + jobs_bytes + fins_bytes);
     float *pf = c->m_part_f.as<float>();
     int *pi = c->m_part_i.as<int>();
     float *red = c->m_red.as<float>();
@@ -181,7 +199,7 @@
             j2.q_hi = q_hi; j2.d_hi = h; j2.n0 = n0; j2.n1 = n1;
             j2.part_v1 = pf + 2 * poff; j2.part_i1 = pi + poff;
             j2.rkeys = c->m_rkeys.as<float>() + (size_t)nstrip * off1;
-            poff += (size_t)splits * n0 + (size_t)splits * n1;
+            poff += (size_t)plan.fslots[i] * n0;
             fn.f_v1 = fn.f_v2 = fn.r_v1 = fn.r_v2 = nullptr; fn.f_i1 = fn.r_i1 = nullptr;
         } else {
             MatchJob &f = jobs[2 * i], &r = jobs[2 * i + 1];
@@ -203,20 +221,21 @@
         fn.red_f = red + 3 * roff; roff += (size_t)n0;
         fn.red_r = red + 3 * roff; roff += (size_t)n1;
     }
-    HIPCHECK(hipMemcpyAsync(c->m_jobs.p, jobs, jobs_bytes + fins_bytes, hipMemcpyHostToDevice, c->stream));
+    HIPCHECK(hipMemcpyAsync(c->m_jobs.p, jobs, jobs_bytes + fins_bytes + plan_bytes, hipMemcpyHostToDevice, c->stream));
     MatchFinal *fins_dev = reinterpret_cast<MatchFinal *>(static_cast<char *>(c->m_jobs.p) + jobs_bytes);
     if (!capturing) HIPCHECK(hipEventRecord(c->ev_jobs, c->stream));
     if (single_gemm) {
+        const int fwd_ids = conf->flavour == SFD2_MATCH_HLOC && !conf->do_mutual_check;
         {
             ProfScope ps(c, "match_mutual", "match_mutual_kernel", 2.0 * (double)n0 * (double)tot_n1 * 128.0,
                          2.0 * ((double)k * n0 + (double)tot_n1) * 128.0);
-            launch_match_mutual(c->stream, c->m_jobs.as<MatchJob2>(), fins_dev, k, n0, max_n1, splits,
-                                conf->flavour == SFD2_MATCH_HLOC && !conf->do_mutual_check);
+            launch_match_mutual(c->stream, c->m_jobs.as<MatchJob2>(), plan_dev, fwd_ids);
         }
         {
-            ProfScope ps(c, "match_finalize", "match_decide", 0.0, (double)tot_part * 12);
-            launch_match_decide(c->stream, fins_dev, k, max_n, conf->flavour, conf->do_mutual_check,
-                                conf->ratio_threshold, conf->distance_threshold);
+            ProfScope ps(c, "match_finalize", "match_mutual_finalize", 0.0, (double)tot_part * 12);
+            launch_match_mutual_finalize(c->stream, c->m_jobs.as<MatchJob2>(), fins_dev, k, n0, max_n1, plan_dev, fwd_ids,
+                                         c->opt_match_fused_finalize, conf->flavour, conf->do_mutual_check, conf->ratio_threshold,
+                                         conf->distance_threshold);
         }
     } else {
         {
@@ -279,22 +298,33 @@
     HIPCHECK(hipMemsetAsync(out_m, 0xFF, (size_t)n0 * sizeof(long long), c->stream));
     HIPCHECK(hipMemsetAsync(out_s, 0, (size_t)n0 * sizeof(float), c->stream));
     if (k > 0) {
-        int splits = std::max(1, (max_b + match_mutual_max_chunk() - 1) / match_mutual_max_chunk());
+        const int splits = 1;
         const int strip = match_mutual_strip();
+        MatchPlan plan;
+        if (single_gemm) {
+            g_sfd2_cu_limit = c->opt_cu_limit;
+            std::vector<int> na_l, nb_l;
+            for (int i : live) { na_l.push_back(seg0[i + 1] - seg0[i]); nb_l.push_back(seg1[i + 1] - seg1[i]); }
+            match_mutual_plan(na_l.data(), nb_l.data(), k, match_mutual_slots(), plan);
+        }
         size_t stage_bytes = 256 + (((size_t)n1 * sizeof(int32_t)) + 255);
         if (!on_device) stage_bytes += ((((size_t)n0 + n1) * dim * elt_size(dtype)) + 511);
         HIPCHECK(c->m_stage.ensure(stage_bytes));
         HIPCHECK(c->m_hi0.ensure((size_t)n0 * 128 * 2));
         HIPCHECK(c->m_hi1.ensure((size_t)std::max(n1, 1) * 128 * 2));
         if (need_lo) { HIPCHECK(c->m_lo0.ensure((size_t)n0 * 128 * 2)); HIPCHECK(c->m_lo1.ensure((size_t)std::max(n1, 1) * 128 * 2)); }
-        const size_t tot_part = (size_t)splits * ((size_t)n0 + n1);
+        size_t tot_part = (size_t)splits * ((size_t)n0 + n1);
+        if (single_gemm) {
+            tot_part = 0;
+            for (int j = 0; j < k; ++j) tot_part += (size_t)plan.fslots[j] * (size_t)(seg0[live[j] + 1] - seg0[live[j]]);
+        }
         HIPCHECK(c->m_part_f.ensure(tot_part * 2 * sizeof(float)));
         HIPCHECK(c->m_part_i.ensure(tot_part * sizeof(int)));
         size_t rk = 0;
         for (int i : live) rk += (size_t)((seg0[i + 1] - seg0[i] + strip - 1) / strip) * (size_t)(seg1[i + 1] - seg1[i]);
         if (single_gemm) HIPCHECK(c->m_rkeys.ensure(std::max<size_t>(rk, 1) * sizeof(float)));
         HIPCHECK(c->m_red.ensure(((size_t)n0 + n1 + 1) * 3 * sizeof(float)));
-        HIPCHECK(c->m_jobs.ensure((size_t)2 * k * sizeof(MatchJob) + (size_t)k * sizeof(MatchFinal)));
+        HIPCHECK(c->m_jobs.ensure((size_t)2 * k * sizeof(MatchJob) + (size_t)k * sizeof(MatchFinal) + 16 + plan.bytes()));
         prof_step_begin(c);
         size_t stage_off = 0;
         const half_t *h0 = nullptr, *l0 = nullptr, *h1 = nullptr, *l1 = nullptr;
@@ -307,15 +337,18 @@
         int32_t *iota_dev = reinterpret_cast<int32_t *>(reinterpret_cast<char *>(c->m_stage.p) + ((stage_off + 255) & ~(size_t)255));
         HIPCHECK(hipMemcpyAsync(iota_dev, iota.data(), (size_t)n1 * sizeof(int32_t), hipMemcpyHostToDevice, c->stream));
         HIPCHECK(hipStreamSynchronize(c->stream));
-        const size_t jobs_bytes = 2 * (size_t)k * sizeof(MatchJob), fins_bytes = (size_t)k * sizeof(MatchFinal);
+        const size_t jobs_bytes = 2 * (size_t)k * sizeof(MatchJob), fins_bytes = ((size_t)k * sizeof(MatchFinal) + 15) & ~(size_t)15;
+        const size_t plan_bytes = plan.bytes();
         HIPCHECK(hipEventSynchronize(c->ev_jobs));
-        if (jobs_bytes + fins_bytes > c->pin_cap) {
+        if (jobs_bytes + fins_bytes + plan_bytes > c->pin_cap) {
             if (c->pin_jobs) (void)hipHostFree(c->pin_jobs);
             c->pin_jobs = nullptr;
             c->pin_cap = 0;
-            HIPCHECK(hipHostMalloc(&c->pin_jobs, jobs_bytes + fins_bytes, hipHostMallocDefault));
-            c->pin_cap = jobs_bytes + fins_bytes;
-        }
+            HIPCHECK(hipHostMalloc(&c->pin_jobs, jobs_bytes + fins_bytes + plan_bytes, hipHostMallocDefault));
+            c->pin_cap = jobs_bytes + fins_bytes + plan_bytes;
+        }
+        const MatchPlanDev plan_dev = plan_stage(plan, reinterpret_cast<char *>(c->pin_jobs) + jobs_bytes + fins_bytes,
+                                                 static_cast<char *>(c->m_jobs.p) + jobs_bytes + fins_bytes);
         MatchJob *jobs = reinterpret_cast<MatchJob *>(c->pin_jobs);
         MatchJob2 *jobs2 = reinterpret_cast<MatchJob2 *>(c->pin_jobs);
         MatchFinal *fins = reinterpret_cast<MatchFinal *>(reinterpret_cast<char *>(c->pin_jobs) + jobs_bytes);
@@ -334,7 +367,7 @@
                 j2.part_v1 = pf + 2 * poff; j2.part_i1 = pi + poff;
                 j2.rkeys = c->m_rkeys.as<float>() + rkoff;
                 rkoff += (size_t)((na + strip - 1) / strip) * nb;
-                poff += (size_t)splits * na + (size_t)splits * nb;
+                poff += (size_t)plan.fslots[j] * na;
                 fn.f_v1 = fn.f_v2 = fn.r_v1 = fn.r_v2 = nullptr; fn.f_i1 = fn.r_i1 = nullptr;
             } else {
                 MatchJob &f = jobs[2 * j], &r = jobs[2 * j + 1];
@@ -354,16 +387,17 @@
             fn.red_f = red + 3 * roff; roff += (size_t)na;
             fn.red_r = red + 3 * roff; roff += (size_t)nb;
         }
-        HIPCHECK(hipMemcpyAsync(c->m_jobs.p, jobs, jobs_bytes + fins_bytes, hipMemcpyHostToDevice, c->stream));
+        HIPCHECK(hipMemcpyAsync(c->m_jobs.p, jobs, jobs_bytes + fins_bytes + plan_bytes, hipMemcpyHostToDevice, c->stream));
         MatchFinal *fins_dev = reinterpret_cast<MatchFinal *>(static_cast<char *>(c->m_jobs.p) + jobs_bytes);
         HIPCHECK(hipEventRecord(c->ev_jobs, c->stream));
         const int max_n = std::max(max_a, max_b);
         if (single_gemm) {
             ProfScope ps(c, "match_segments", "match_mutual_kernel", 0.0, 0.0);
-            launch_match_mutual(c->stream, c->m_jobs.as<MatchJob2>(), fins_dev, k, max_a, max_b, splits,
-                                conf->flavour == SFD2_MATCH_HLOC && !conf->do_mutual_check);
-            launch_match_decide(c->stream, fins_dev, k, max_n, conf->flavour, conf->do_mutual_check,
-                                conf->ratio_threshold, conf->distance_threshold);
+            const int fwd_ids = conf->flavour == SFD2_MATCH_HLOC && !conf->do_mutual_check;
+            launch_match_mutual(c->stream, c->m_jobs.as<MatchJob2>(), plan_dev, fwd_ids);
+            launch_match_mutual_finalize(c->stream, c->m_jobs.as<MatchJob2>(), fins_dev, k, max_a, max_b, plan_dev, fwd_ids,
+                                         c->opt_match_fused_finalize, conf->flavour, conf->do_mutual_check, conf->ratio_threshold,
+                                         conf->distance_threshold);
         } else {
             ProfScope ps(c, "match_segments", "match_top2_kernel", 0.0, 0.0);
             launch_match_top2(c->stream, c->m_jobs.as<MatchJob>(), 2 * k, max_n, splits, need_lo, need_top2, c->zero_page.as<half_t>());
@@ -388,3 +422,19 @@
     const sfd2_desc_set db = {d1, n1, dtype, layout, on_device, nullptr, 0, 0};
     return sfd2_match_batch(c, &q, &db, 1, dim, conf, matches0, scores0, out_on_device, 0);
 }
+
+extern "C" int sfd2_match_plan(const int32_t *n0, const int32_t *n1, int k, int slots, int32_t *segs, int cap_segs, int *n_blocks)
+{
+    if (k < 0 || (k > 0 && (!n0 || !n1))) return fail("sfd2_match_plan: bad argument");
+    MatchPlan plan;
+    match_mutual_plan(n0, n1, k, slots > 0 ? slots : match_mutual_slots(), plan);
+    if (n_blocks) *n_blocks = plan.nblk;
+    if (segs)
+        for (int b = 0; b < plan.nblk; ++b)
+            for (int i = plan.blk_rng[2 * b]; i < plan.blk_rng[2 * b + 1] && i < cap_segs; ++i) {
+                const MatchSeg &g = plan.segs[(size_t)i];
+                int32_t *o = segs + 6 * (size_t)i;
+                o[0] = g.pair; o[1] = g.strip; o[2] = g.st0; o[3] = g.nst; o[4] = g.fslot; o[5] = b;
+            }
+    return (int)plan.segs.size();
+}
diff --git a/sfd2_amd/csrc/match_kernels.hip b/sfd2_amd/csrc/match_kernels.hip
--- a/sfd2_amd/csrc/match_kernels.hip
+++ b/sfd2_amd/csrc/match_kernels.hip
@@ -296,11 +296,50 @@
 }
 
 #define MQ_NEG (-0x1p100f)
-void launch_match_mutual_gemm(hipStream_t st, const MatchJob2 *jobs_dev, int npairs, int max_n0, int splits, int fwd_ids);
-int match_mutual_strip(void);
+
+__device__ __forceinline__ void mutual_fold_fwd(const MatchJob2 &job, int i, int nrows, int fwd_ids, float &b1, int &bi)
+{
+    const int n = job.n0;
+    b1 = -INFINITY;
+    bi = 0;
+    for (int s = 0; s < nrows; ++s) {
+        const float c1 = job.part_v1[(size_t)s * n + i];
+        if (c1 > b1) { b1 = c1; if (fwd_ids) bi = job.part_i1[(size_t)s * n + i]; }
+    }
+    if (!fwd_ids) bi = -1;
+}
+
+__device__ __forceinline__ void mutual_fold_rev(const MatchJob2 &job, int j, int strip, float &val, int &idx)
+{
+    const int n = job.n1;
+    const int nstrip = (job.n0 + strip - 1) / strip;
+    float best = MQ_NEG;
+    unsigned int bkey = __float_as_uint(MQ_NEG);
+    int bs = 0;
+    int sidx = 0;
+    for (; sidx + 8 <= nstrip; sidx += 8) {
+        float k[8];
+#pragma unroll
+        for (int u = 0; u < 8; ++u) k[u] = job.rkeys[(size_t)(sidx + u) * n + j];
+#pragma unroll
+        for (int u = 0; u < 8; ++u) {
+            const float v = __uint_as_float(__float_as_uint(k[u]) & 0xFFFFFF00u);
+            if (v > best) { best = v; bkey = __float_as_uint(k[u]); bs = sidx + u; }
+        }
+    }
+    for (; sidx < nstrip; ++sidx) {
+        const float k = job.rkeys[(size_t)sidx * n + j];
+        const float v = __uint_as_float(__float_as_uint(k) & 0xFFFFFF00u);
+        if (v > best) { best = v; bkey = __float_as_uint(k); bs = sidx; }
+    }
+    const bool any = best > MQ_NEG;
+    val = any ? __uint_as_float(bkey & 0xFFFFFF00u) : -INFINITY;
+    idx = any ? bs * strip + 255 - (int)(bkey & 255u) : 0;
+}
 
 __global__ __launch_bounds__(NT)
-void match_mutual_reduce_kernel(const MatchJob2 *__restrict__ jobs, const MatchFinal *__restrict__ fins, int splits, int strip, int fwd_ids)
+void match_mutual_reduce_kernel(const MatchJob2 *__restrict__ jobs, const MatchFinal *__restrict__ fins, const int *__restrict__ fcnt,
+                                int max_ns, int strip, int fwd_ids)
 {
     const MatchJob2 job = jobs[blockIdx.y];
     const MatchFinal f = fins[blockIdx.y];
@@ -308,43 +347,20 @@
     const int n = dir == 0 ? job.n0 : job.n1;
     const int i = blockIdx.x * blockDim.x + threadIdx.x;
     if (i >= n) return;
-    float b1 = -INFINITY;
-    int bi = 0;
     if (dir == 0) {
-        for (int s = 0; s < splits; ++s) {
-            const float c1 = job.part_v1[(size_t)s * n + i];
-            if (c1 > b1) { b1 = c1; if (fwd_ids) bi = job.part_i1[(size_t)s * n + i]; }
-        }
-        if (!fwd_ids) bi = -1;
+        float b1;
+        int bi;
+        mutual_fold_fwd(job, i, fcnt[(size_t)blockIdx.y * max_ns + i / strip], fwd_ids, b1, bi);
         f.red_f[i] = b1;
         f.red_f[(size_t)n + i] = -INFINITY;
         reinterpret_cast<int *>(f.red_f)[2 * (size_t)n + i] = bi;
     } else {
-        const int nstrip = (job.n0 + strip - 1) / strip;
-        float best = MQ_NEG;
-        unsigned int bkey = __float_as_uint(MQ_NEG);
-        int bs = 0;
-        int sidx = 0;
-        for (; sidx + 8 <= nstrip; sidx += 8) {
-            float k[8];
-#pragma unroll
-            for (int u = 0; u < 8; ++u) k[u] = job.rkeys[(size_t)(sidx + u) * n + i];
-#pragma unroll
-            for (int u = 0; u < 8; ++u) {
-                const float v = __uint_as_float(__float_as_uint(k[u]) & 0xFFFFFF00u);
-                if (v > best) { best = v; bkey = __float_as_uint(k[u]); bs = sidx + u; }
-            }
-        }
-        for (; sidx < nstrip; ++sidx) {
-            const float k = job.rkeys[(size_t)sidx * n + i];
-            const float v = __uint_as_float(__float_as_uint(k) & 0xFFFFFF00u);
-            if (v > best) { best = v; bkey = __float_as_uint(k); bs = sidx; }
-        }
-        const unsigned int bits = bkey;
-        const bool any = best > MQ_NEG;
-        f.red_r[i] = any ? __uint_as_float(bits & 0xFFFFFF00u) : -INFINITY;
+        float v;
+        int q;
+        mutual_fold_rev(job, i, strip, v, q);
+        f.red_r[i] = v;
         f.red_r[(size_t)n + i] = -INFINITY;
-        reinterpret_cast<int *>(f.red_r)[2 * (size_t)n + i] = any ? bs * strip + 255 - (int)(bits & 255u) : 0;
+        reinterpret_cast<int *>(f.red_r)[2 * (size_t)n + i] = q;
     }
 }
 
@@ -361,16 +377,117 @@
         atomicMin(reinterpret_cast<unsigned int *>(f.red_f) + 2 * (size_t)f.n0 + i, (unsigned int)j);
 }
 
-void launch_match_mutual(hipStream_t st, const MatchJob2 *jobs_dev, const MatchFinal *fins_dev, int npairs, int max_n0,
-                         int max_n1, int splits, int fwd_ids)
+__device__ __forceinline__ bool hloc_pass(float s1, float s2, float ratio, float dist);
+__device__ __forceinline__ float lowe_ratio(float s1, float s2);
+__device__ __forceinline__ void match_decide_one(const MatchFinal &f, int i, float s1, float s2, int j, float t1, float t2, int back,
+                                                 int flavour, int mutual, float ratio, float dist);
+
+#define MF_NT 1024
+#define MF_MAX_N0 8192
+#define MF_U 4
+#define MF_S 8
+__global__ __launch_bounds__(MF_NT)
+void match_mutual_finalize_kernel(const MatchJob2 *__restrict__ jobs, const MatchFinal *__restrict__ fins, const int *__restrict__ fcnt,
+                                  int max_ns, int strip, int fwd_ids, int flavour, int mutual, float ratio, float dist)
+{
+    extern __shared__ __attribute__((aligned(16))) unsigned char fsm[];
+    const MatchJob2 job = jobs[blockIdx.x];
+    const MatchFinal f = fins[blockIdx.x];
+    const int n0 = job.n0, n1 = job.n1;
+    float *fv = reinterpret_cast<float *>(fsm);
+    unsigned int *fi = reinterpret_cast<unsigned int *>(fsm) + n0;
+    for (int i0 = threadIdx.x; i0 < n0; i0 += MF_NT * MF_U) {
+        float b1[MF_U];
+        int bi[MF_U], nr[MF_U], nrmax = 0;
+#pragma unroll
+        for (int c = 0; c < MF_U; ++c) {
+            const int i = i0 + c * MF_NT;
+            b1[c] = -INFINITY; bi[c] = 0;
+            nr[c] = i < n0 ? fcnt[(size_t)blockIdx.x * max_ns + i / strip] : 0;
+            nrmax = max(nrmax, nr[c]);
+        }
+#pragma unroll 2
+        for (int s = 0; s < nrmax; ++s) {
+            float c1[MF_U];
+            int ci[MF_U];
+#pragma unroll
+            for (int c = 0; c < MF_U; ++c) {
+                const size_t o = (size_t)s * n0 + i0 + c * MF_NT;
+                c1[c] = s < nr[c] ? job.part_v1[o] : -INFINITY;
+                ci[c] = (fwd_ids && s < nr[c]) ? job.part_i1[o] : 0;
+            }
+#pragma unroll
+            for (int c = 0; c < MF_U; ++c)
+                if (c1[c] > b1[c]) { b1[c] = c1[c]; bi[c] = ci[c]; }
+        }
+#pragma unroll
+        for (int c = 0; c < MF_U; ++c) {
+            const int i = i0 + c * MF_NT;
+            if (i < n0) { fv[i] = b1[c]; fi[i] = fwd_ids ? (unsigned int)bi[c] : 0xFFFFFFFFu; }
+        }
+    }
+    __syncthreads();
+    if (!fwd_ids) {
+        const int nstrip = (n0 + strip - 1) / strip;
+        for (int j0 = threadIdx.x; j0 < n1; j0 += MF_NT * MF_U) {
+            float best[MF_U];
+            unsigned int bkey[MF_U];
+            int bs[MF_U];
+#pragma unroll
+            for (int c = 0; c < MF_U; ++c) { best[c] = MQ_NEG; bkey[c] = __float_as_uint(MQ_NEG); bs[c] = 0; }
+            for (int s0 = 0; s0 < nstrip; s0 += MF_S) {
+                float k[MF_U][MF_S];
+#pragma unroll
+                for (int c = 0; c < MF_U; ++c)
+#pragma unroll
+                    for (int u = 0; u < MF_S; ++u)
+                        k[c][u] = (s0 + u < nstrip && j0 + c * MF_NT < n1) ? job.rkeys[(size_t)(s0 + u) * n1 + j0 + c * MF_NT] : MQ_NEG;
+#pragma unroll
+                for (int c = 0; c < MF_U; ++c)
+#pragma unroll
+                    for (int u = 0; u < MF_S; ++u) {
+                        const float v = __uint_as_float(__float_as_uint(k[c][u]) & 0xFFFFFF00u);
+                        if (v > best[c]) { best[c] = v; bkey[c] = __float_as_uint(k[c][u]); bs[c] = s0 + u; }
+                    }
+            }
+#pragma unroll
+            for (int c = 0; c < MF_U; ++c) {
+                const int j = j0 + c * MF_NT;
+                if (j >= n1 || !(best[c] > MQ_NEG)) continue;
+                const unsigned int r = bkey[c] & 0xFFFFFF00u;
+                const int i = bs[c] * strip + 255 - (int)(bkey[c] & 255u);
+                if ((__float_as_uint(fv[i]) & 0xFFFFFF00u) == r) atomicMin(fi + i, (unsigned int)j);
+            }
+        }
+        __syncthreads();
+    }
+    for (int i = threadIdx.x; i < n0; i += MF_NT) {
+        const int j = (int)fi[i];
+        const float s1 = fv[i];
+        match_decide_one(f, i, s1, -INFINITY, j, __uint_as_float(__float_as_uint(s1) & 0xFFFFFF00u), -INFINITY, i, flavour, mutual, ratio, dist);
+    }
+}
+
+int match_fused_max_n0(void) { return MF_MAX_N0; }
+
+void launch_match_decide(hipStream_t st, const MatchFinal *fin_dev, int npairs, int max_n, int flavour, int mutual,
+                         float ratio, float dist);
+void launch_match_mutual_finalize(hipStream_t st, const MatchJob2 *jobs_dev, const MatchFinal *fins_dev, int npairs, int max_n0,
+                                  int max_n1, const MatchPlanDev &plan, int fwd_ids, int fused, int flavour, int mutual,
+                                  float ratio, float dist)
 {
     if (npairs <= 0 || max_n0 <= 0) return;
-    launch_match_mutual_gemm(st, jobs_dev, npairs, max_n0, splits, fwd_ids);
+    if (fused && max_n0 <= MF_MAX_N0) {
+        hipLaunchKernelGGL(match_mutual_finalize_kernel, dim3(npairs), dim3(MF_NT), (size_t)max_n0 * 8, st, jobs_dev, fins_dev, plan.fcnt,
+                           plan.max_ns, match_mutual_strip(), fwd_ids, flavour, mutual, ratio, dist);
+        return;
+    }
     const int max_n = max_n0 > max_n1 ? max_n0 : max_n1;
-    hipLaunchKernelGGL(match_mutual_reduce_kernel, dim3((max_n + NT - 1) / NT, npairs, 2), dim3(NT), 0, st, jobs_dev, fins_dev, splits,
-                       match_mutual_strip(), fwd_ids);
+    hipLaunchKernelGGL(match_mutual_reduce_kernel, dim3((max_n + NT - 1) / NT, npairs, 2), dim3(NT), 0, st, jobs_dev, fins_dev, plan.fcnt,
+                       plan.max_ns, match_mutual_strip(), fwd_ids);
     if (!fwd_ids && max_n1 > 0)
         hipLaunchKernelGGL(match_mutual_claim_kernel, dim3((max_n1 + NT - 1) / NT, npairs), dim3(NT), 0, st, fins_dev);
+    launch_match_decide(st, fins_dev, npairs, max_n, flavour, mutual, ratio, dist);
 }
 
 void launch_match_top2(hipStream_t st, const MatchJob *jobs_dev, int njobs, int max_nb, int splits, int use_lo,
@@ -447,21 +564,14 @@
     return d0 / (d1 + 1e-8f);
 }
 
-__global__ __launch_bounds__(NT)
-void match_decide_kernel(const MatchFinal *__restrict__ fins, int flavour, int mutual, float ratio, float dist)
-{
-    const MatchFinal f = fins[blockIdx.y];
-    const int i = blockIdx.x * blockDim.x + threadIdx.x;
-    if (i >= f.n0) return;
-    const float s1 = f.red_f[i], s2 = f.red_f[(size_t)f.n0 + i];
-    const int j = reinterpret_cast<const int *>(f.red_f)[2 * (size_t)f.n0 + i];
+__device__ __forceinline__ void match_decide_one(const MatchFinal &f, int i, float s1, float s2, int j, float t1, float t2, int back,
+                                                 int flavour, int mutual, float ratio, float dist)
+{
     long long m = -1;
     float score = 0.0f;
     if (f.n1 > 0 && j < 0) {
         score = flavour == 0 ? (hloc_pass(s1, s2, ratio, dist) ? (s1 + 1.0f) / 2.0f : 0.0f) : s1;
     } else if (f.n1 > 0) {
-        const float t1 = f.red_r[j], t2 = f.red_r[(size_t)f.n1 + j];
-        const int back = reinterpret_cast<const int *>(f.red_r)[2 * (size_t)f.n1 + j];
         if (flavour == 0) {
             const bool ok = hloc_pass(s1, s2, ratio, dist);
             score = ok ? (s1 + 1.0f) / 2.0f : 0.0f;
@@ -489,6 +599,23 @@
     }
 }
 
+__global__ __launch_bounds__(NT)
+void match_decide_kernel(const MatchFinal *__restrict__ fins, int flavour, int mutual, float ratio, float dist)
+{
+    const MatchFinal f = fins[blockIdx.y];
+    const int i = blockIdx.x * blockDim.x + threadIdx.x;
+    if (i >= f.n0) return;
+    const float s1 = f.red_f[i], s2 = f.red_f[(size_t)f.n0 + i];
+    const int j = reinterpret_cast<const int *>(f.red_f)[2 * (size_t)f.n0 + i];
+    float t1 = 0.0f, t2 = 0.0f;
+    int back = 0;
+    if (f.n1 > 0 && j >= 0) {
+        t1 = f.red_r[j]; t2 = f.red_r[(size_t)f.n1 + j];
+        back = reinterpret_cast<const int *>(f.red_r)[2 * (size_t)f.n1 + j];
+    }
+    match_decide_one(f, i, s1, s2, j, t1, t2, back, flavour, mutual, ratio, dist);
+}
+
 void launch_match_decide(hipStream_t st, const MatchFinal *fin_dev, int npairs, int max_n, int flavour, int mutual,
                          float ratio, float dist)
 {
diff --git a/sfd2_amd/csrc/match_mutual_kernel.hip b/sfd2_amd/csrc/match_mutual_kernel.hip
--- a/sfd2_amd/csrc/match_mutual_kernel.hip
+++ b/sfd2_amd/csrc/match_mutual_kernel.hip
@@ -1,5 +1,6 @@
 #include "sfd2_internal.h"
 #include <math.h>
+#include <algorithm>
 
 #define NT 256
 #define KD 128
@@ -18,46 +19,24 @@
 
 template <bool FWD_IDS>
 __global__ __launch_bounds__(NT, 2)
-void match_mutual_kernel(const MatchJob2 *__restrict__ jobs, int splits, int qblocks)
+void match_mutual_kernel(const MatchJob2 *__restrict__ jobs, const MatchSeg *__restrict__ segs, const int *__restrict__ blk_rng)
 {
     extern __shared__ __attribute__((aligned(16))) unsigned char smem[];
-    int swz;
-    {
-        const int bid = (int)blockIdx.x, nblk = (int)gridDim.x;
-        const int q = nblk >> 3, r = nblk & 7, xcd = bid & 7, local = bid >> 3;
-        swz = (xcd < r ? xcd * (q + 1) : r * (q + 1) + (xcd - r) * q) + local;
-    }
-    const int bx = swz % qblocks, by = (swz / qblocks) % splits, bz = swz / (qblocks * splits);
-    const MatchJob2 job = jobs[bz];
-    const int n1 = job.n1, n0 = job.n0;
-    const int i_base = bx * 256;
-    if (i_base >= n0) return;
+    int pk_si = blk_rng[2 * blockIdx.x], pk_se = blk_rng[2 * blockIdx.x + 1];
+    if (pk_si >= pk_se) return;
     const int tid = threadIdx.x, lane = tid & 63;
     const int wave = __builtin_amdgcn_readfirstlane(tid >> 6);
     const int lcol = lane & 31, lhi = lane >> 5;
 
-    int chunk = (n1 + splits - 1) / splits;
-    chunk = (chunk + 31) & ~31;
-    const int ja0 = by * chunk;
-    int ja1 = ja0 + chunk;
-    if (ja1 > n1) ja1 = n1;
-
-    const int q0 = i_base + wave * 64;
-    const bool wave_active = q0 < n0;
-    const bool partial_q = q0 + 64 > n0;
+    int nst = 0, n0 = 0, slen = 0, q0 = 0;
+    bool wave_active = false, partial_q = false;
+    int pk_pair = 0, pk_strip = 0, pk_fslot = 0, pk_n1 = 0, pk_ja0 = 0;
+    unsigned long long pk_q = 0;
+#define MQ_PARK(v_) asm volatile("" : "+v"(v_))
+#define MQ_UNPARK(v_) __builtin_amdgcn_readfirstlane(v_)
+    int pk_w64 = (tid >> 6) * 64;
+    MQ_PARK(pk_si); MQ_PARK(pk_se); MQ_PARK(pk_w64);
     h8_t aq[2][8];
-#pragma unroll
-    for (int t = 0; t < 2; ++t) {
-        const int qi = q0 + t * 32 + lcol;
-#pragma unroll
-        for (int ks = 0; ks < 8; ++ks) {
-            h8_t z;
-#pragma unroll
-            for (int e = 0; e < 8; ++e) z[e] = (half_t)0.0f;
-            aq[t][ks] = z;
-            if (qi < n0) aq[t][ks] = *reinterpret_cast<const h8_t *>(job.q_hi + (size_t)qi * KD + ks * 16 + lhi * 8);
-        }
-    }
     float rm[2][16];
 #pragma unroll
     for (int t = 0; t < 2; ++t)
@@ -68,8 +47,7 @@
     for (int r = 0; r < 16; ++r) zero16[r] = 0.0f;
     const unsigned int wb = (3u - (unsigned)wave) << 6;
     const unsigned int cb[2] = {wb | 0x20u | ((1u - (unsigned)lhi) << 2), wb | ((1u - (unsigned)lhi) << 2)};
-    float *rtab = reinterpret_cast<float *>(smem + 2 * TA2 * 256);
-    for (int i = tid; i < ja1 - ja0; i += NT) rtab[i] = MQ_NEG;
+    float *rtab = reinterpret_cast<float *>(smem + 3 * TA2 * 256);
     const unsigned rt_lane = (unsigned)(size_t)(const lds_void_t *)rtab + (unsigned)lcol * 4u;
     unsigned int keep = ~((1u << MQ_TILE_BITS) - 1u);
     asm volatile("" : "+v"(keep));
@@ -79,10 +57,10 @@
 #define MQ_BFRAG(BUF_, SUB_, KS_) \
     (*reinterpret_cast<const h8_t *>(brow + ((BUF_)*TA2 + (SUB_)*32) * 256 + ((((KS_)*2 + lhi) ^ bsw) << 4)))
 #define MQ_TILE_MASK(C0_, C1_, TILE_)                                                                    \
-    if (ja0 + (TILE_)*32 + 32 > ja1 || partial_q) {                                                      \
+    if ((TILE_)*32 + 32 > slen || partial_q) {                                                           \
         int qlim_ = n0 - q0 - 4 * lhi;       \
         asm volatile("" : "+v"(qlim_)::"memory");                                                        \
-        const bool pad_col_ = ja0 + (TILE_)*32 + lcol >= ja1;                                            \
+        const bool pad_col_ = (TILE_)*32 + lcol >= slen;                                                 \
         _Pragma("unroll") for (int r = 0; r < 16; ++r) {                                                 \
             const int qr_ = (r & 3) + 8 * (r >> 2);                                                      \
             if (pad_col_ || qr_ >= qlim_) C0_[r] = MQ_NEG;                                               \
@@ -146,22 +124,55 @@
         MQ_TILE_REV(b0_, b1_, tb_)                                                                       \
     }
 
-    if (ja0 < ja1) {
-        const int nst = (ja1 - ja0 + TA2 - 1) / TA2;
-        const __amdgpu_buffer_rsrc_t d_rsrc = __builtin_amdgcn_make_buffer_rsrc(const_cast<half_t *>(job.d_hi), 0, ja1 * (KD * 2), 0x00020000);
-        int voff[TA2 / 16];
-#pragma unroll
-        for (int c = 0; c < TA2 / 16; ++c) {
-            const int row = (wave * (TA2 / 16) + c) * 4 + (lane >> 4);
-            voff[c] = (ja0 + row) * (KD * 2) + (((lane & 15) ^ (row & 15)) << 4);
-        }
+    __amdgpu_buffer_rsrc_t d_rsrc;
+    int voff[TA2 / 16];
+    const unsigned lds_wave = (unsigned)(size_t)(const lds_void_t *)smem + (unsigned)wave * ((TA2 / 16) * 1024u);
 #define ISSUE_B(buf_)                                                                                    \
     _Pragma("unroll") for (int c = 0; c < TA2 / 16; ++c) {                                               \
-        __builtin_amdgcn_raw_ptr_buffer_load_lds(d_rsrc, (lds_void_t *)(smem + (buf_)*TA2 * 256 + (wave * (TA2 / 16) + c) * 1024), \
+        unsigned lb_ = lds_wave;                                                                         \
+        asm volatile("" : "+s"(lb_));                                                                    \
+        __builtin_amdgcn_raw_ptr_buffer_load_lds(d_rsrc, (lds_void_t *)(size_t)(lb_ + (unsigned)((buf_)*TA2 * 256 + c * 1024)), \
                                                  16, voff[c], 0, 0, 0);                                  \
         voff[c] += TA2 * (KD * 2);                                                                       \
     }
-        ISSUE_B(0)
+#define MQ_SEG_SETUP(FIRST_)                                                                             \
+    {                                                                                                    \
+        const MatchSeg sg_ = segs[MQ_UNPARK(pk_si)];                                                     \
+        const MatchJob2 job_ = jobs[sg_.pair];                                                           \
+        const half_t *q_hi = job_.q_hi;                                                                  \
+        const bool newq_ = (FIRST_) || (unsigned long long)(size_t)q_hi != pk_q || sg_.strip != pk_strip || job_.n0 != n0; \
+        pk_pair = sg_.pair; pk_strip = sg_.strip; pk_fslot = sg_.fslot; pk_n1 = job_.n1;                 \
+        pk_q = (unsigned long long)(size_t)q_hi;                                                         \
+        MQ_PARK(pk_pair); MQ_PARK(pk_strip); MQ_PARK(pk_fslot); MQ_PARK(pk_n1); MQ_PARK(pk_q);           \
+        nst = sg_.nst; n0 = job_.n0;                                                                     \
+        const int ja0 = sg_.st0 * TA2, ja1 = min(job_.n1, ja0 + nst * TA2);                              \
+        slen = ja1 - ja0;                                                                                \
+        pk_ja0 = ja0; MQ_PARK(pk_ja0);                                                                   \
+        q0 = sg_.strip * 256 + MQ_UNPARK(pk_w64);                                                              \
+        wave_active = q0 < n0;                                                                           \
+        partial_q = q0 + 64 > n0;                                                                        \
+        d_rsrc = __builtin_amdgcn_make_buffer_rsrc(const_cast<half_t *>(job_.d_hi), 0, ja1 * (KD * 2), 0x00020000); \
+        _Pragma("unroll") for (int c = 0; c < TA2 / 16; ++c) {                                           \
+            const int row = (wave * (TA2 / 16) + c) * 4 + (lane >> 4);                                   \
+            voff[c] = (ja0 + row) * (KD * 2) + (((lane & 15) ^ (row & 15)) << 4);                        \
+        }                                                                                                \
+        ISSUE_B(0)                                                                                       \
+        if (newq_) {                                                                                     \
+            _Pragma("unroll") for (int t = 0; t < 2; ++t) {                                              \
+                const int qi = q0 + t * 32 + lcol;                                                       \
+                _Pragma("unroll") for (int ks = 0; ks < 8; ++ks) {                                       \
+                    h8_t z;                                                                              \
+                    _Pragma("unroll") for (int e = 0; e < 8; ++e) z[e] = (half_t)0.0f;                   \
+                    aq[t][ks] = z;                                                                       \
+                    if (qi < n0) aq[t][ks] = *reinterpret_cast<const h8_t *>(q_hi + (size_t)qi * KD + ks * 16 + lhi * 8); \
+                }                                                                                        \
+            }                                                                                            \
+        }                                                                                                \
+    }
+    MQ_SEG_SETUP(true)
+    for (int i = tid; i < slen; i += NT) rtab[i] = MQ_NEG;
+    float *T = reinterpret_cast<float *>(smem + TA2 * 256) + wave * (64 * 32);
+    for (;;) {
         SFD2_BARRIER_DRAIN();
         for (int s = 0; s < nst; s += 2) {
             if (s + 1 < nst) { ISSUE_B(1) }
@@ -173,64 +184,158 @@
                 SFD2_BARRIER_DRAIN();
             }
         }
+        __syncthreads();
+        const MatchJob2 fj = jobs[MQ_UNPARK(pk_pair)];
+        const int f_len = slen, f_ja0 = MQ_UNPARK(pk_ja0);
+        float *f_rk = fj.rkeys + (size_t)MQ_UNPARK(pk_strip) * MQ_UNPARK(pk_n1) + f_ja0 + tid;
+        const size_t f_o = (size_t)MQ_UNPARK(pk_fslot) * n0 + q0 + lane;
+        float *f_pv = fj.part_v1 + f_o;
+        int *f_pi = FWD_IDS ? fj.part_i1 + f_o : nullptr;
+        const bool f_active = wave_active, f_row = wave_active && q0 + lane < n0;
+        ++pk_si;
+        const bool more = MQ_UNPARK(pk_si) < MQ_UNPARK(pk_se);
+        int len = 0;
+        if (more) {
+            MQ_SEG_SETUP(false)
+            len = slen;
+        }
+        for (int i = 0; i + tid < max(f_len, len); i += NT) {
+            if (i + tid < f_len) f_rk[i] = rtab[i + tid];
+            if (i + tid < len) rtab[i + tid] = MQ_NEG;
+        }
+        if (f_active) {
+#pragma unroll
+            for (int t = 0; t < 2; ++t)
+#pragma unroll
+                for (int r = 0; r < 16; ++r) {
+                    const int q = (r & 3) + 8 * (r >> 2) + 4 * lhi;
+                    T[(t * 32 + q) * 32 + (lcol ^ (MQ_TSWZ(q) << 2))] = rm[t][r];
+                    rm[t][r] = MQ_NEG;
+                }
+        }
+        __syncthreads();
+        if (f_row) {
+            float best = MQ_NEG;
+            int col = 0;
+#pragma unroll
+            for (int c4 = 0; c4 < 8; ++c4) {
+                const float4 v = *reinterpret_cast<const float4 *>(T + lane * 32 + ((c4 ^ MQ_TSWZ(lane)) << 2));
+                if (v.x > best) { best = v.x; col = c4 * 4 + 0; }
+                if (v.y > best) { best = v.y; col = c4 * 4 + 1; }
+                if (v.z > best) { best = v.z; col = c4 * 4 + 2; }
+                if (v.w > best) { best = v.w; col = c4 * 4 + 3; }
+            }
+            const unsigned int bits = __float_as_uint(best);
+            const bool any = best > MQ_NEG;
+            if (FWD_IDS) {
+                const int tile = (1 << MQ_TILE_BITS) - 1 - (int)(bits & ((1u << MQ_TILE_BITS) - 1u));
+                *f_pv = any ? __uint_as_float(bits & ~((1u << MQ_TILE_BITS) - 1u)) : -INFINITY;
+                *f_pi = any ? f_ja0 + tile * 32 + col : 0;
+            } else {
+                *f_pv = any ? best : -INFINITY;
+            }
+        }
+        if (!more) break;
+    }
 #undef ISSUE_B
-        __syncthreads();
-        float *rk = job.rkeys + (size_t)bx * n1 + ja0;
-        for (int i = tid; i < ja1 - ja0; i += NT) rk[i] = rtab[i];
-    }
+#undef MQ_SEG_SETUP
+#undef MQ_PARK
+#undef MQ_UNPARK
 #undef MQ_STAGE
 #undef MQ_BFRAG
 #undef MQ_TILE_MASK
 #undef MQ_TILE_REV
-    float *T = reinterpret_cast<float *>(smem) + wave * (64 * 32);
-    if (wave_active) {
-#pragma unroll
-        for (int t = 0; t < 2; ++t)
-#pragma unroll
-            for (int r = 0; r < 16; ++r) {
-                const int q = (r & 3) + 8 * (r >> 2) + 4 * lhi;
-                T[(t * 32 + q) * 32 + (lcol ^ (MQ_TSWZ(q) << 2))] = rm[t][r];
+}
+
+int match_mutual_strip(void) { return 256; }
+
+#define MQ_XCDS 8
+#define MQ_SEG_UNITS (MQ_MAX_CHUNK / (2 * TA2))
+
+int match_mutual_slots(void)
+{
+    static int cus = 0;
+    if (cus == 0) {
+        int dev = 0, n = 0;
+        cus = (hipGetDevice(&dev) == hipSuccess && hipDeviceGetAttribute(&n, hipDeviceAttributeMultiprocessorCount, dev) == hipSuccess && n > 0) ? n : 256;
+    }
+    return 2 * sfd2_slots(cus);
+}
+
+void match_mutual_plan(const int *n0, const int *n1, int npairs, int slots, MatchPlan &plan)
+{
+    plan.segs.clear(); plan.blk_rng.clear(); plan.fcnt.clear();
+    plan.fslots.assign((size_t)(npairs > 0 ? npairs : 0), 0);
+    plan.nblk = 0; plan.max_ns = 0;
+    std::vector<long long> W((size_t)npairs + 1, 0);
+    std::vector<int> units((size_t)npairs, 0), ns((size_t)npairs, 0);
+    for (int p = 0; p < npairs; ++p) {
+        const int nst = n1[p] > 0 ? (n1[p] + TA2 - 1) / TA2 : 0;
+        ns[p] = (n0[p] > 0 && nst > 0) ? (n0[p] + 255) / 256 : 0;
+        units[p] = ns[p] > 0 ? (nst + 1) / 2 : 0;
+        W[p + 1] = W[p] + (long long)units[p] * ns[p];
+        if (ns[p] > plan.max_ns) plan.max_ns = ns[p];
+    }
+    for (int p = 0; p < npairs; ++p) plan.max_ns = std::max(plan.max_ns, n0[p] > 0 ? (n0[p] + 255) / 256 : 0);
+    plan.fcnt.assign((size_t)npairs * plan.max_ns, 0);
+    const long long total = W[npairs];
+    if (total == 0 || slots <= 0) return;
+    const int nblk = (int)std::min<long long>(slots, total);
+    plan.nblk = nblk;
+    plan.blk_rng.assign((size_t)2 * nblk, 0);
+    const long long base = total / nblk, rem = total % nblk;
+    long long i0 = 0;
+    for (int x = 0; x < MQ_XCDS && x < nblk; ++x) {
+        long long share = 0;
+        for (int b = x; b < nblk; b += MQ_XCDS) share += base + (b < rem ? 1 : 0);
+        const long long i1 = i0 + share;
+        int b = x;
+        long long room = base + (b < rem ? 1 : 0);
+        plan.blk_rng[2 * b] = plan.blk_rng[2 * b + 1] = (int)plan.segs.size();
+        int p_lo = 0;
+        while (p_lo < npairs && W[p_lo + 1] <= i0) ++p_lo;
+        for (int s = 0; s < plan.max_ns; ++s)
+            for (int p = p_lo; p < npairs && W[p] < i1; ++p) {
+                if (s >= ns[p]) continue;
+                const long long a = std::max(i0, W[p]) - W[p], e = std::min(i1, W[p + 1]) - W[p];
+                long long c = a > s ? (a - s + ns[p] - 1) / ns[p] : 0;
+                const long long c_end = e > s ? (e - s + ns[p] - 1) / ns[p] : 0;
+                const int nst_p = (n1[p] + TA2 - 1) / TA2;
+                while (c < c_end) {
+                    if (room == 0) {
+                        b += MQ_XCDS;
+                        room = base + (b < rem ? 1 : 0);
+                        plan.blk_rng[2 * b] = plan.blk_rng[2 * b + 1] = (int)plan.segs.size();
+                    }
+                    const long long take = std::min<long long>(std::min<long long>(c_end - c, room), MQ_SEG_UNITS);
+                    MatchSeg g;
+                    g.pair = p; g.strip = s; g.st0 = (int)(2 * c);
+                    g.nst = std::min(nst_p - g.st0, (int)(2 * take));
+                    g.fslot = plan.fcnt[(size_t)p * plan.max_ns + s]++;
+                    g.pad_ = 0;
+                    plan.segs.push_back(g);
+                    plan.blk_rng[2 * b + 1] = (int)plan.segs.size();
+                    c += take; room -= take;
+                }
             }
-    }
-    __syncthreads();
-    if (wave_active && q0 + lane < n0) {
-        float best = MQ_NEG;
-        int col = 0;
-#pragma unroll
-        for (int c4 = 0; c4 < 8; ++c4) {
-            const float4 v = *reinterpret_cast<const float4 *>(T + lane * 32 + ((c4 ^ MQ_TSWZ(lane)) << 2));
-            if (v.x > best) { best = v.x; col = c4 * 4 + 0; }
-            if (v.y > best) { best = v.y; col = c4 * 4 + 1; }
-            if (v.z > best) { best = v.z; col = c4 * 4 + 2; }
-            if (v.w > best) { best = v.w; col = c4 * 4 + 3; }
-        }
-        const unsigned int bits = __float_as_uint(best);
-        const size_t o = (size_t)by * n0 + q0 + lane;
-        const bool any = best > MQ_NEG;
-        if (FWD_IDS) {
-            const int tile = (1 << MQ_TILE_BITS) - 1 - (int)(bits & ((1u << MQ_TILE_BITS) - 1u));
-            job.part_v1[o] = any ? __uint_as_float(bits & ~((1u << MQ_TILE_BITS) - 1u)) : -INFINITY;
-            job.part_i1[o] = any ? ja0 + tile * 32 + col : 0;
-        } else {
-            job.part_v1[o] = any ? best : -INFINITY;
-        }
-    }
+        i0 = i1;
+    }
+    for (int p = 0; p < npairs; ++p)
+        for (int s = 0; s < plan.max_ns; ++s) plan.fslots[p] = std::max(plan.fslots[p], plan.fcnt[(size_t)p * plan.max_ns + s]);
 }
 
-int match_mutual_strip(void) { return 256; }
-
-void launch_match_mutual_gemm(hipStream_t st, const MatchJob2 *jobs_dev, int npairs, int max_n0, int splits, int fwd_ids)
+void launch_match_mutual(hipStream_t st, const MatchJob2 *jobs_dev, const MatchPlanDev &plan, int fwd_ids)
 {
     static bool attr = false;
-    const size_t lds = (size_t)2 * TA2 * 256 + (size_t)MQ_MAX_CHUNK * sizeof(float);
+    const size_t lds = (size_t)3 * TA2 * 256 + (size_t)MQ_MAX_CHUNK * sizeof(float);
     if (!attr) {
         (void)hipFuncSetAttribute(reinterpret_cast<const void *>(match_mutual_kernel<true>), hipFuncAttributeMaxDynamicSharedMemorySize, (int)lds);
         (void)hipFuncSetAttribute(reinterpret_cast<const void *>(match_mutual_kernel<false>), hipFuncAttributeMaxDynamicSharedMemorySize, (int)lds);
         attr = true;
     }
-    const int qblocks = (max_n0 + 255) / 256;
-    if (fwd_ids) hipLaunchKernelGGL(match_mutual_kernel<true>, dim3(qblocks * splits * npairs), dim3(NT), lds, st, jobs_dev, splits, qblocks);
-    else hipLaunchKernelGGL(match_mutual_kernel<false>, dim3(qblocks * splits * npairs), dim3(NT), lds, st, jobs_dev, splits, qblocks);
+    if (plan.nblk <= 0) return;
+    if (fwd_ids) hipLaunchKernelGGL(match_mutual_kernel<true>, dim3(plan.nblk), dim3(NT), lds, st, jobs_dev, plan.segs, plan.blk_rng);
+    else hipLaunchKernelGGL(match_mutual_kernel<false>, dim3(plan.nblk), dim3(NT), lds, st, jobs_dev, plan.segs, plan.blk_rng);
 }
 
 int match_mutual_max_chunk(void) { return MQ_MAX_CHUNK; }
diff --git a/sfd2_amd/csrc/sfd2_ctx.h b/sfd2_amd/csrc/sfd2_ctx.h
--- a/sfd2_amd/csrc/sfd2_ctx.h
+++ b/sfd2_amd/csrc/sfd2_ctx.h
@@ -136,6 +136,7 @@
     float range_hist[SFD2_RS_COUNT] = {};
     int opt_auto_range = 1;
     std::vector<float> h_sta_w;
+    int opt_match_fused_finalize = 1;
     int opt_cu_limit = 0;
     int fuse_det = 0;
     int use_graphs = 0;
diff --git a/sfd2_amd/csrc/sfd2_internal.h b/sfd2_amd/csrc/sfd2_internal.h
--- a/sfd2_amd/csrc/sfd2_internal.h
+++ b/sfd2_amd/csrc/sfd2_internal.h
@@ -2,6 +2,7 @@
 #include <hip/hip_runtime.h>
 #include <hip/hip_fp16.h>
 #include <stdint.h>
+#include <vector>
 
 #ifdef SFD2_EXPERIMENTS
 #include <stdlib.h>
@@ -473,9 +474,33 @@
     int *part_i1;
     float *rkeys;
 };
+struct MatchSeg {
+    int pair, strip;
+    int st0, nst;
+    int fslot;
+    int pad_;
+};
+struct MatchPlan {
+    int nblk = 0;
+    int max_ns = 0;
+    std::vector<MatchSeg> segs;
+    std::vector<int> blk_rng;
+    std::vector<int> fcnt;
+    std::vector<int> fslots;
+    size_t bytes() const { return ((segs.size() * sizeof(MatchSeg) + 15) & ~(size_t)15) + (blk_rng.size() + fcnt.size()) * sizeof(int); }
+};
+void match_mutual_plan(const int *n0, const int *n1, int npairs, int slots, MatchPlan &plan);
+struct MatchPlanDev {
+    const MatchSeg *segs; const int *blk_rng; const int *fcnt;
+    int nblk, max_ns;
+};
+int match_mutual_slots(void);
 struct MatchFinal;
-void launch_match_mutual(hipStream_t st, const MatchJob2 *jobs_dev, const MatchFinal *fins_dev, int npairs, int max_n0,
-                         int max_n1, int splits, int fwd_ids);
+void launch_match_mutual(hipStream_t st, const MatchJob2 *jobs_dev, const MatchPlanDev &plan, int fwd_ids);
+void launch_match_mutual_finalize(hipStream_t st, const MatchJob2 *jobs_dev, const MatchFinal *fins_dev, int npairs, int max_n0,
+                                  int max_n1, const MatchPlanDev &plan, int fwd_ids, int fused, int flavour, int mutual,
+                                  float ratio, float dist);
+int match_fused_max_n0(void);
 int match_mutual_max_chunk(void);
 int match_mutual_strip(void);
 void launch_match_decide(hipStream_t st, const MatchFinal *fin_dev, int npairs, int max_n, int flavour, int mutual,
```
